# NeRF-3DTalker/NeRF-3DTalker-code

Measured on AMD Instinct MI355X. Metric: rendered frames/sec @512^2 x 64 samples/ray, higher is better.
Workload: dtype bf16; 1 GPU; cfg2-R: 16 heads/GPU/step, 64x64 rays x 64 samples -> fused MLP+composite -> neural renderer -> 512x512 RGB (+ background image); rays_per_frame=4096, samples_per_ray=64, parallelism=frames sharded over 1 rank(s), no data-path collective, ranks_seen_by_backend=1

## Files before the change

### include/n3dt.h

```cpp
#ifndef N3DT_API_H_
#define N3DT_API_H_

#include <stddef.h>
#include <stdint.h>

#ifdef __cplusplus
extern "C" {
#endif

#define N3DT_ABI_VERSION 5

#define N3DT_F32 0
#define N3DT_BF16 1
#define N3DT_F16 2
#define N3DT_BF16X3 3

#define N3DT_OK 0
#define N3DT_EINVAL (-1)
#define N3DT_EWORKSPACE (-2)
#define N3DT_EHIP (-3)

#define N3DT_PE_DIM 63
#define N3DT_MLP_LAYERS 12

typedef struct N3dtGeom {
    int32_t batch;
    int32_t n_rays;
    int32_t n_samples;
    int32_t hidden;
    int32_t feat_nc;
    int32_t shape_dim;
    int32_t appea_dim;
    int32_t audio_dim;
    int32_t featmap_size;
    int32_t n_blocks;
    float world_z1;
    float world_z2;
    int64_t xy_stride_b, xy_stride_c, xy_stride_r;
    int32_t z_planes_given;
    int32_t bg_is_hwc;
    int32_t vd_dim;
} N3dtGeom;

typedef struct N3dtMlpParams {
    const float* weight[N3DT_MLP_LAYERS];
    const float* bias[N3DT_MLP_LAYERS];
} N3dtMlpParams;

#define N3DT_MAX_BLOCKS 8
typedef struct N3dtRenderParams {
    const float* to_rgb_w[N3DT_MAX_BLOCKS + 1];
    const float* to_rgb_b[N3DT_MAX_BLOCKS + 1];
    const float* psu1_w[N3DT_MAX_BLOCKS];
    const float* psu1_b[N3DT_MAX_BLOCKS];
    const float* psu2_w[N3DT_MAX_BLOCKS];
    const float* psu2_b[N3DT_MAX_BLOCKS];
    const float* feat_w[N3DT_MAX_BLOCKS];
    const float* feat_b[N3DT_MAX_BLOCKS];
} N3dtRenderParams;

typedef struct N3dtMlpGrads {
    float* weight[N3DT_MLP_LAYERS];
    float* bias[N3DT_MLP_LAYERS];
} N3dtMlpGrads;

typedef struct N3dtRenderGrads {
    float* to_rgb_w[N3DT_MAX_BLOCKS + 1];
    float* to_rgb_b[N3DT_MAX_BLOCKS + 1];
    float* psu1_w[N3DT_MAX_BLOCKS];
    float* psu1_b[N3DT_MAX_BLOCKS];
    float* psu2_w[N3DT_MAX_BLOCKS];
    float* psu2_b[N3DT_MAX_BLOCKS];
    float* feat_w[N3DT_MAX_BLOCKS];
    float* feat_b[N3DT_MAX_BLOCKS];
} N3dtRenderGrads;

int n3dt_abi_version(void);
const char* n3dt_last_error(void);

size_t n3dt_mlp_packed_bytes(const N3dtGeom* g, int precision);
int n3dt_mlp_pack(const N3dtGeom* g, int precision, const N3dtMlpParams* p, void* packed, void* stream);

size_t n3dt_render_workspace_bytes(const N3dtGeom* g, int precision);
int n3dt_render_fwd(const N3dtGeom* g, int precision, const void* packed_mlp, const N3dtMlpParams* p,
                    const float* xy, const float* R, const float* T, const float* Kinv,
                    const float* shape, const float* appea, const float* audio, const float* t_rand,
                    const float* bg_featmap, const float* ray_bias,
                    float* fg_feat, float* bg_alpha, float* depth, float* weight, float* merge_feat,
                    void* workspace, size_t workspace_bytes, void* stream);

int n3dt_render_fwd16(const N3dtGeom* g, int precision, const void* packed_mlp, const N3dtMlpParams* p,
                      const float* xy, const float* R, const float* T, const float* Kinv,
                      const float* shape, const float* appea, const float* audio, const float* t_rand,
                      const float* bg_featmap, const float* ray_bias,
                      float* fg_feat, float* bg_alpha, float* depth, float* weight, float* merge_feat,
                      void* merge_feat16, float* rgb0, const float* rgb0_w, const float* rgb0_b,
                      void* workspace, size_t workspace_bytes, void* stream);

int n3dt_ray_vd_bias(const N3dtGeom* g, const float* w_vd, int64_t ld_w, const float* xy, const float* R, const float* Kinv,
                     float* ray_bias, void* stream);

int n3dt_fine_sample(const N3dtGeom* g, int n_fine, const float* weight, const float* T, const float* t_rand, const float* u,
                     float* z_planes, void* stream);

int n3dt_sample_points(const N3dtGeom* g, const float* xy, const float* R, const float* T, const float* Kinv, const float* t_rand,
                       float* pts, float* zvals, float* z_dists, float* ray_d, float* ray_l, void* stream);
int n3dt_embed(int batch, size_t m, const float* pts, float* pe, void* stream);
int n3dt_embed_freqs(int batch, size_t m, int n_freqs, const float* pts, float* pe, void* stream);
size_t n3dt_mlp_points_workspace_bytes(const N3dtGeom* g, size_t m);
int n3dt_mlp_points(const N3dtGeom* g, size_t m, const N3dtMlpParams* p, const float* audio, const float* embed_vps,
                    const float* embed_vds, float* rgb, float* density, void* workspace, size_t workspace_bytes, void* stream);
int n3dt_composite(int batch, int n_rays, int n_samples, int channels, const float* rgb, const float* density, const float* z_dists,
                   const float* zvals, float* feat, float* bg_alpha, float* depth, float* weight, void* stream);
int n3dt_x16_pack_probe(int precision, int form, size_t n, const float* in, uint16_t* out, void* stream);
int n3dt_x16_pe_probe(int precision, int form, size_t n, const float* points, uint16_t* out, void* stream);

size_t n3dt_neural_render_workspace_bytes(const N3dtGeom* g, int nb);
int n3dt_neural_render_fwd(const N3dtGeom* g, int nb, int precision, const N3dtRenderParams* p, const float* featmap,
                           float* img, void* workspace, size_t workspace_bytes, void* stream);

int n3dt_neural_render_pack(const N3dtGeom* g, int nb, int precision, const N3dtRenderParams* p, void* workspace,
                            size_t workspace_bytes, void* stream);
int n3dt_neural_render_fwd_reuse(const N3dtGeom* g, int nb, int precision, const N3dtRenderParams* p, const float* featmap,
                                 float* img, void* workspace, size_t workspace_bytes, void* stream);
int n3dt_feat_to_rgb0(int nb, int n_pix, const float* featmap, const float* w, const float* b, float* rgb0, void* stream);
int n3dt_neural_render_fwd16_reuse(const N3dtGeom* g, int nb, int precision, const N3dtRenderParams* p, const void* featmap16,
                                   const float* rgb0, float* img, void* workspace, size_t workspace_bytes, void* stream);

size_t n3dt_render_train_saved_bytes(const N3dtGeom* g);
size_t n3dt_render_train_workspace_bytes(const N3dtGeom* g);
int n3dt_render_train_fwd(const N3dtGeom* g, int precision, const void* packed_mlp, const N3dtMlpParams* p,
                          const float* xy, const float* R, const float* T, const float* Kinv,
                          const float* shape, const float* appea, const float* audio, const float* t_rand,
                          const float* bg_featmap, const float* ray_bias, float* fg_feat, float* bg_alpha, float* depth, float* merge_feat,
                          void* saved, size_t saved_bytes, void* workspace, size_t workspace_bytes, void* stream);
int n3dt_render_bwd(const N3dtGeom* g, int precision, const N3dtMlpParams* p, const N3dtMlpGrads* grads,
                    const float* shape, const float* appea, const float* audio, const float* bg_featmap,
                    const float* d_merge_feat, const float* d_fg_feat, const float* d_bg_alpha,
                    const void* saved, size_t saved_bytes,
                    float* d_bg_featmap, float* d_shape, float* d_appea, float* d_audio, float* d_ray_bias,
                    const float* xy, const float* R, const float* T, const float* Kinv, const float* t_rand,
                    float* d_R, float* d_T,
                    void* workspace, size_t workspace_bytes, void* stream);
int n3dt_render_bwd_cam(const N3dtGeom* g, int precision, const N3dtMlpParams* p, const N3dtMlpGrads* grads,
                        const float* shape, const float* appea, const float* audio, const float* bg_featmap,
                        const float* d_merge_feat, const float* d_fg_feat, const float* d_bg_alpha,
                        const void* saved, size_t saved_bytes,
                        float* d_bg_featmap, float* d_shape, float* d_appea, float* d_audio, float* d_ray_bias,
                        const float* xy, const float* R, const float* T, const float* Kinv, const float* t_rand,
                        float* d_R, float* d_T, float* d_Kinv, float* d_xy,
                        void* workspace, size_t workspace_bytes, void* stream);

size_t n3dt_neural_render_train_saved_bytes(const N3dtGeom* g, int nb);
size_t n3dt_neural_render_train_workspace_bytes(const N3dtGeom* g, int nb);
int n3dt_neural_render_train_fwd(const N3dtGeom* g, int nb, int precision, const N3dtRenderParams* p, const float* featmap, float* img,
                                 void* saved, size_t saved_bytes, void* workspace, size_t workspace_bytes, void* stream);
int n3dt_neural_render_bwd(const N3dtGeom* g, int nb, int precision, const N3dtRenderParams* p, const N3dtRenderGrads* grads,
                           const float* featmap, const float* d_img, const void* saved, size_t saved_bytes,
                           float* d_featmap, void* workspace, size_t workspace_bytes, void* stream);

int n3dt_img_to_uint8(int n_images, int pixels, const float* img, unsigned char* out, void* stream);

size_t n3dt_eval_metrics_workspace_bytes(int n_images, int height, int width);
int n3dt_eval_metrics(int n_images, int height, int width, const float* pred, const float* gt, double* ssim, double* psnr,
                      void* workspace, size_t workspace_bytes, void* stream);

#define N3DT_LPIPS_LAYERS 5
#define N3DT_LPIPS_REFERENCE 0
#define N3DT_LPIPS_STANDARD 1
typedef struct N3dtLpipsParams {
    const float* weight[N3DT_LPIPS_LAYERS];
    const float* bias[N3DT_LPIPS_LAYERS];
    const float* lin[N3DT_LPIPS_LAYERS];
} N3dtLpipsParams;
size_t n3dt_lpips_packed_bytes(void);
int n3dt_lpips_pack(const N3dtLpipsParams* p, void* packed, void* stream);
size_t n3dt_lpips_workspace_bytes(int batch, int height, int width);
int n3dt_lpips(int batch, int height, int width, int input_mode, const void* packed, const float* pred, const float* gt, double* out,
               double* layers, void* workspace, size_t workspace_bytes, void* stream);

size_t n3dt_mel_workspace_bytes(void);
int n3dt_mel_spectrogram(int64_t n_samples, const float* wav, int64_t wav_offset, const float* prev_sample, int64_t total_samples,
                         int64_t first_frame, int n_frames, const float* basis, const double* table, void* out, int64_t out_ld,
                         int out_is_f64, void* workspace, size_t workspace_bytes, void* stream);
int n3dt_mel_windows(int64_t T, const void* mel, int64_t mel_ld, int mel_is_f64, int n_windows, const int32_t* start, float* out,
                     void* stream);

#define N3DT_SYNCNET_BLOCKS 31
typedef struct N3dtSyncnetParams {
    const float* weight[N3DT_SYNCNET_BLOCKS];
    const float* bias[N3DT_SYNCNET_BLOCKS];
    const float* bn_weight[N3DT_SYNCNET_BLOCKS];
    const float* bn_bias[N3DT_SYNCNET_BLOCKS];
    const float* bn_mean[N3DT_SYNCNET_BLOCKS];
    const float* bn_var[N3DT_SYNCNET_BLOCKS];
} N3dtSyncnetParams;
size_t n3dt_syncnet_packed_bytes(void);
int n3dt_syncnet_pack(const N3dtSyncnetParams* p, void* packed, void* stream);
size_t n3dt_syncnet_workspace_bytes(int n);
int n3dt_syncnet_face_windows(int n, int height, int width, const float* frames, const int32_t* boxes, int n_boxes, float* face_windows,
                              void* stream);
int n3dt_syncnet_fwd(int n, const void* packed, const float* mel_windows, const float* face_windows, const float* frames,
                     const int32_t* boxes, int n_boxes, int height, int width, float* audio_emb, float* face_emb, double* cos,
                     void* workspace, size_t workspace_bytes, void* stream);
int n3dt_syncnet_block(int block, int n, const void* packed, const float* in, float* out, void* workspace, size_t workspace_bytes,
                       void* stream);

int n3dt_loss_fwd(int batch, int pixels, const float* merge_img, const float* bg_img, const float* gt, const float* mask,
                  float bg_value, float* acc, float* terms, void* stream);
int n3dt_loss_bwd(int batch, int pixels, const float* merge_img, const float* bg_img, const float* gt, const float* mask,
                  float bg_value, const float* acc, const float* g, const float* g_total, float* d_merge, float* d_bg, void* stream);

#define N3DT_VGG_CONVS 10
typedef struct N3dtVggParams {
    const float* weight[N3DT_VGG_CONVS];
    const float* bias[N3DT_VGG_CONVS];
} N3dtVggParams;
size_t n3dt_vgg_packed_bytes(int precision);
int n3dt_vgg_pack(int precision, const N3dtVggParams* p, void* packed, void* stream);
size_t n3dt_vgg_saved_bytes(int batch, int precision);
size_t n3dt_vgg_workspace_bytes(int batch, int img_size, int precision);
int n3dt_vgg_loss_fwd(int batch, int img_size, int precision, const void* packed, const float* merge_img, const float* gt,
                      const float* mask, float bg_value, float* terms, void* saved, size_t saved_bytes, void* ws, size_t ws_bytes,
                      void* stream);
int n3dt_vgg_loss_bwd(int batch, int img_size, int precision, const void* packed, const float* merge_img, const float* g_total,
                      const void* saved, size_t saved_bytes, float* d_merge, void* ws, size_t ws_bytes, void* stream);

#define N3DT_A2S_IN 1280
#define N3DT_A2S_HIDDEN 640
#define N3DT_A2S_OUT 64
#define N3DT_A2S_MAX_T 256
#define N3DT_A2S_GRAD_FLOATS 20726784
typedef struct N3dtA2sParams {
    const float* w_ih[4];
    const float* w_hh[4];
    const float* b_ih[4];
    const float* b_hh[4];
    const float* lin_w[3];
    const float* lin_b[3];
} N3dtA2sParams;
size_t n3dt_a2s_saved_bytes(int T);
size_t n3dt_a2s_workspace_bytes(int T);
int n3dt_a2s_fwd(int T, const N3dtA2sParams* p, const float* mel, const float* mask1, const float* mask2, const float* mask3,
                 float* out, void* saved, size_t saved_bytes, void* ws, size_t ws_bytes, void* stream);
int n3dt_a2s_bwd(int T, const N3dtA2sParams* p, const float* g_out, const void* saved, size_t saved_bytes, float* grad_arena,
                 void* ws, size_t ws_bytes, void* stream);

#define N3DT_ADAM_MAX_GROUPS 64
#define N3DT_ADAM_MAX_GRID 1024
#define N3DT_ADAM_COUNTER_INTS 4
typedef struct N3dtAdamTensor {
    float* param;
    const float* grad;
    float* exp_avg;
    float* exp_avg_sq;
    int64_t numel;
    int32_t group;
    int32_t active;
} N3dtAdamTensor;
typedef struct N3dtAdamChunk {
    int64_t start;
    int32_t tensor;
    int32_t length;
} N3dtAdamChunk;
typedef struct N3dtAdamGroup {
    double lr, beta1, beta2, eps, weight_decay;
    int32_t maximize;
    int32_t reserved;
} N3dtAdamGroup;
size_t n3dt_flat_adam_record_bytes(int which);
int n3dt_flat_adam_step(const void* tensor_table, const void* chunk_table, int n_chunks, const void* group_table, int n_groups,
                        void* step_counter, void* stream);
#include "n3dt_flat_adam_guard.h"

int n3dt_chw_to_hwc(int C, int n, const float* src, float* dst, void* stream);

#define N3DT_STAGE_MAX 12
typedef struct N3dtStageCopy {
    const float* src[N3DT_STAGE_MAX];
    float* dst[N3DT_STAGE_MAX];
    int64_t count[N3DT_STAGE_MAX];
    int64_t view_dims[3], view_strides[3];
    int32_t n;
} N3dtStageCopy;
int n3dt_stage_inputs(const N3dtStageCopy* st, void* stream);

int n3dt_graph_begin(void* stream);
int n3dt_graph_end(void* stream, void** graph_out);
int n3dt_graph_launch(void* graph, void* stream);
int n3dt_graph_destroy(void* graph);

int n3dt_prof_enable(int max_records);
int n3dt_prof_collect(float* ms_out, int capacity, int* n_out);

#ifdef __cplusplus
}
#endif
#endif
```

### nerf-3dtalker-code_amd/csrc/n3dt_api.hip

```cpp
#include <hip/hip_runtime.h>
#include <stdio.h>
#include <stdlib.h>
#include <string.h>

#include <mutex>

#include "../../include/n3dt.h"
#include "n3dt_layout.h"
#include "eval_metrics_core.h"
#include "lpips_core.h"
#include "mel_core.h"
#include "syncnet_core.h"

extern "C" {
void n3dt_launch_pack(const N3dtGeom*, int, const N3dtMlpParams*, void*, hipStream_t);
void n3dt_launch_fold(const N3dtGeom*, const N3dtMlpParams*, const float*, const float*, const float*, float*, int, hipStream_t);
void n3dt_launch_ray_head(const N3dtGeom*, int, int, const float*, const float*, const float*, const float*, int, float*, float*,
                          float*, float*, float*, hipStream_t);
void n3dt_launch_ray_head_mfma(const N3dtGeom*, int, int, const float*, const float*, const float*, const float*, int, float*, float*,
                               float*, float*, float*, float*, hipStream_t);
void n3dt_launch_ray_head_mfma16(const N3dtGeom*, int, int, const float*, const float*, const float*, const float*, int, float*, float*,
                                 float*, float*, float*, void*, int, float*, const float*, const float*, hipStream_t);
void n3dt_launch_chw_to_hwc(int, int, const float*, float*, hipStream_t);
void n3dt_launch_rayfold(const N3dtGeom*, const float*, const float*, hipStream_t);
void n3dt_launch_ray_vd_bias(const N3dtGeom*, const float*, long, const float*, const float*, const float*, float*, hipStream_t);
void n3dt_launch_embed_freqs(int, size_t, int, const float*, float*, hipStream_t);
void n3dt_launch_sample_points(const N3dtGeom*, const float*, const float*, const float*, const float*, const float*, float*, float*,
                               float*, float*, float*, hipStream_t);
void n3dt_launch_embed(int, size_t, const float*, float*, hipStream_t);
size_t n3dt_seam_mlp_ws_floats(const N3dtGeom*, size_t);
void n3dt_launch_mlp_points(const N3dtGeom*, size_t, const N3dtMlpParams*, const float*, const float*, const float*, float*, float*, float*,
                            hipStream_t);
void n3dt_launch_composite(int, int, int, int, const float*, const float*, const float*, const float*, float*, float*, float*, float*,
                           hipStream_t);
void n3dt_launch_x16_pack_probe(int, int, size_t, const float*, unsigned short*, hipStream_t);
void n3dt_launch_x16_pe_probe(int, int, size_t, const float*, unsigned short*, hipStream_t);
void n3dt_launch_fine_sample(const N3dtGeom*, int, const float*, const float*, const float*, const float*, float*, hipStream_t);
void n3dt_launch_nerf_fwd_f32(const N3dtGeom*, const N3dtMlpParams*, const void*, const float*, const float*, const float*,
                              const float*, const float*, const float*, float*, float*, hipStream_t);
void n3dt_launch_nerf_fwd_x16(const N3dtGeom*, int, const void*, const float*, const float*, const float*, const float*,
                              const float*, const float*, float*, float*, hipStream_t);
void n3dt_launch_nerf_fwd_x16s(const N3dtGeom*, const void*, const float*, const float*, const float*, const float*, const float*,
                               const float*, float*, float*, hipStream_t);
size_t n3dt_nr_workspace_floats(const N3dtGeom*, int);
size_t n3dt_train_saved_floats(const N3dtGeom*);
size_t n3dt_train_ws_floats(const N3dtGeom*);
void n3dt_launch_train_fwd(const N3dtGeom*, const N3dtMlpParams*, const float*, const float*, const float*, const float*, const float*,
                           const float*, const float*, const float*, const float*, const float*, float*, float*, float*, float*, float*,
                           float*, const float* , hipStream_t);
void n3dt_launch_train_bwd(const N3dtGeom*, const N3dtMlpParams*, const N3dtMlpGrads*, const float*, const float*, const float*,
                           const float*, const float*, const float*, const float*, const float*, float*, float*, float*, float*,
                           const float*, const float*, const float*, const float*, const float*, float*, float*, float* ,
                           float* , float*, float* , hipStream_t);
size_t n3dt_train16_saved_bytes(const N3dtGeom*);
size_t n3dt_train16_ws_bytes(const N3dtGeom*);
void n3dt_launch_train16_fwd(const N3dtGeom*, const N3dtMlpParams*, const void*, const float*, const float*, const float*, const float*,
                             const float*, const float*, const float*, const float*, const float*, const float*, float*, float*, float*,
                             float*, void*, void*, const float* , hipStream_t);
void n3dt_launch_train16_bwd(const N3dtGeom*, const N3dtMlpParams*, const N3dtMlpGrads*, const float*, const float*, const float*,
                             const float*, const float*, const float*, const float*, const void*, float*, float*, float*, float*,
                             const float*, const float*, const float*, const float*, const float*, float*, float*, float* ,
                             float* , void*, float* , hipStream_t);
void n3dt_launch_img_to_uint8(int, int, const float*, unsigned char*, hipStream_t);
void n3dt_launch_loss_fwd(int, int, const float*, const float*, const float*, const float*, float, float*, float*, hipStream_t);
void n3dt_launch_loss_bwd(int, int, const float*, const float*, const float*, const float*, float, const float*, const float*, const float*, float*,
                          float*, hipStream_t);
size_t n3dt_nr_train_saved_floats(const N3dtGeom*, int);
size_t n3dt_nr_train_ws_floats(const N3dtGeom*, int);
void n3dt_launch_nr_train_fwd(const N3dtGeom*, int, const N3dtRenderParams*, const float*, float*, float*, float*, int, hipStream_t);
void n3dt_launch_nr_bwd(const N3dtGeom*, int, const N3dtRenderParams*, const N3dtRenderGrads*, const float*, const float*, const float*,
                        float*, float*, int, hipStream_t);
void n3dt_launch_neural_render(const N3dtGeom*, int, int, const N3dtRenderParams*, const float*, float*, float*, int, hipStream_t);
void n3dt_launch_feat_to_rgb0(int, int, const float*, const float*, const float*, float*, hipStream_t);
void n3dt_launch_neural_render16(const N3dtGeom*, int, int, const N3dtRenderParams*, const void*, const float*, float*, float*, hipStream_t);
void n3dt_launch_stage(const N3dtStageCopy*, hipStream_t);
size_t n3dt_vgg_packed_layout_bytes(int);
size_t n3dt_vgg_saved_floats(int);
size_t n3dt_vgg_ws_floats(int);
void n3dt_launch_vgg_pack(int, const N3dtVggParams*, void*, hipStream_t);
void n3dt_launch_vgg_fwd(int, int, int, const void*, const float*, const float*, const float*, float, float*, void*, void*, hipStream_t);
void n3dt_launch_vgg_bwd(int, int, int, const void*, const float*, const float*, const void*, float*, void*, hipStream_t);
size_t n3dt_a2s_saved_floats(int);
size_t n3dt_a2s_ws_floats(int);
void n3dt_launch_a2s_fwd(int, const N3dtA2sParams*, const float*, const float* const[3], float*, void*, void*, hipStream_t);
void n3dt_launch_a2s_bwd(int, const N3dtA2sParams*, const float*, const void*, float*, void*, hipStream_t);
void n3dt_launch_flat_adam(const void*, const void*, int, const void*, int, void*, hipStream_t);
void n3dt_launch_flat_adam_guarded(const void*, const void*, int, const void*, int, void*, void*, void*, hipStream_t);
size_t n3dt_eval_metrics_ws_bytes(int, int, int);
void n3dt_launch_eval_metrics(int, int, int, const float*, const float*, double*, double*, void*, hipStream_t);
size_t n3dt_lpips_packed_layout_bytes(void);
size_t n3dt_lpips_ws_bytes(int, int, int);
void n3dt_launch_lpips_pack(const N3dtLpipsParams*, void*, hipStream_t);
void n3dt_launch_lpips(int, int, int, int, const void*, const float*, const float*, double*, double*, void*, hipStream_t);
size_t n3dt_mel_ws_bytes(void);
void n3dt_launch_mel_spectrogram(const MelSignal*, long long, int, const float*, const double*, void*, long long, int, void*, hipStream_t);
void n3dt_launch_mel_windows(const void*, long long, long long, int, const int*, int, float*, hipStream_t);
size_t n3dt_syncnet_packed_layout_bytes(void);
size_t n3dt_syncnet_ws_bytes(int);
float* n3dt_syncnet_ws_faces(int, void*);
void n3dt_launch_syncnet_pack(const N3dtSyncnetParams*, void*, hipStream_t);
void n3dt_launch_syncnet_faces(int, int, int, const float*, const int*, int, float*, hipStream_t);
void n3dt_launch_syncnet_fwd(int, const void*, const float*, const float*, float*, float*, double*, void*, hipStream_t);
void n3dt_launch_syncnet_block(int, int, const void*, const float*, float*, void*, hipStream_t);
}

static thread_local char g_err[256] = "";

static int fail(int code, const char* msg) {
    snprintf(g_err, sizeof(g_err), "%s", msg);
    return code;
}

static int check_hip(const char* where) {
    hipError_t e = hipGetLastError();
    if (e != hipSuccess) {
        snprintf(g_err, sizeof(g_err), "%s: %s", where, hipGetErrorString(e));
        return N3DT_EHIP;
    }
    return N3DT_OK;
}

static int check_geom(const N3dtGeom* g, int precision) {
    if (!g) return fail(N3DT_EINVAL, "geometry is NULL");
    if (precision != N3DT_F32 && precision != N3DT_BF16 && precision != N3DT_F16 && precision != N3DT_BF16X3)
        return fail(N3DT_EINVAL, "unknown precision");
    if (g->batch < 1 || g->n_rays < 1 || g->n_samples < 1) return fail(N3DT_EINVAL, "batch, n_rays and n_samples must be >= 1");
    if (g->n_samples > 1024) return fail(N3DT_EINVAL, "n_samples > 1024 is not supported");
    if (g->hidden != 384) return fail(N3DT_EINVAL, "only mlp_hidden_nchannels == 384 is built");
    if (g->feat_nc != 256) return fail(N3DT_EINVAL, "only featmap_nc == 256 is built");
    if (g->shape_dim < 1 || g->appea_dim < 1 || g->audio_dim < 0) return fail(N3DT_EINVAL, "bad latent widths");
    if (g->shape_dim + g->audio_dim > 512 || g->appea_dim > 512) return fail(N3DT_EINVAL, "latent width > 512");
    if (g->vd_dim != 0 && g->vd_dim != 27) return fail(N3DT_EINVAL, "vd_dim must be 0 or 27 (include_vd: 3 + 6 * 4 channels)");
    return N3DT_OK;
}
static int check_ray_bias(const N3dtGeom* g, const void* ray_bias, const char* who) {
    if ((g->vd_dim > 0) != (ray_bias != nullptr)) {
        snprintf(g_err, sizeof(g_err), "%s: the per-ray bias must be given iff vd_dim > 0", who);
        return N3DT_EINVAL;
    }
    return N3DT_OK;
}

static inline int block_samples(int precision) { return precision == N3DT_F32 ? 16 : 32; }
static inline size_t align256(size_t b) { return (b + 255) & ~(size_t)255; }

struct RenderCarve {
    size_t fold, part, wlocal, bghwc, total;
    int bpr, bs;
};

static RenderCarve render_carve(const N3dtGeom* g, int precision) {
    RenderCarve c;
    c.bs = block_samples(precision);
    c.bpr = (g->n_samples + c.bs - 1) / c.bs;
    const size_t blocks = (size_t)g->batch * g->n_rays * c.bpr;
    c.fold = 0;
    c.part = align256(n3dt_fold_region_floats(g->batch, g->n_rays, g->vd_dim) * sizeof(float));
    c.wlocal = c.part + align256(blocks * (192 + 4) * sizeof(float));
    c.bghwc = c.wlocal + align256(blocks * c.bs * sizeof(float));
    c.total = c.bghwc + align256((size_t)g->n_rays * g->feat_nc * sizeof(float));
    return c;
}

static std::mutex g_prof_mu;
static hipEvent_t* g_prof_ev = nullptr;
static int g_prof_cap = 0, g_prof_n = 0;

static void prof_free_locked(int created) {
    for (int i = 0; i < created; ++i) (void)hipEventDestroy(g_prof_ev[i]);
    delete[] g_prof_ev;
    g_prof_ev = nullptr;
    g_prof_cap = g_prof_n = 0;
}

extern "C" int n3dt_prof_enable(int max_records) {
    std::lock_guard<std::mutex> lock(g_prof_mu);
    prof_free_locked(2 * g_prof_cap);
    if (max_records <= 0) return N3DT_OK;
    g_prof_ev = new hipEvent_t[2 * (size_t)max_records];
    for (int i = 0; i < 2 * max_records; ++i)
        if (hipEventCreate(&g_prof_ev[i]) != hipSuccess) {
            prof_free_locked(i);
            return fail(N3DT_EHIP, "n3dt_prof_enable: hipEventCreate failed");
        }
    g_prof_cap = max_records;
    return N3DT_OK;
}

extern "C" int n3dt_prof_span_begin(hipStream_t s) {
    if (g_prof_cap <= 0) return -1;
    std::lock_guard<std::mutex> lock(g_prof_mu);
    if (g_prof_n >= g_prof_cap) return -1;
    const int slot = g_prof_n++;
    (void)hipEventRecord(g_prof_ev[2 * slot], s);
    return slot;
}
extern "C" void n3dt_prof_span_end(int slot, hipStream_t s) {
    if (slot < 0) return;
    std::lock_guard<std::mutex> lock(g_prof_mu);
    if (slot < g_prof_cap) (void)hipEventRecord(g_prof_ev[2 * slot + 1], s);
}

extern "C" int n3dt_prof_collect(float* ms_out, int capacity, int* n_out) {
    if (!ms_out || !n_out) return fail(N3DT_EINVAL, "n3dt_prof_collect: NULL argument");
    std::lock_guard<std::mutex> lock(g_prof_mu);
    int n = g_prof_n < capacity ? g_prof_n : capacity;
    for (int i = 0; i < n; ++i) {
        if (hipEventSynchronize(g_prof_ev[2 * i + 1]) != hipSuccess) return fail(N3DT_EHIP, "n3dt_prof_collect: sync failed");
        if (hipEventElapsedTime(&ms_out[i], g_prof_ev[2 * i], g_prof_ev[2 * i + 1]) != hipSuccess)
            return fail(N3DT_EHIP, "n3dt_prof_collect: elapsed failed");
    }
    *n_out = n;
    g_prof_n = 0;
    return N3DT_OK;
}

extern "C" int n3dt_abi_version(void) { return N3DT_ABI_VERSION; }
extern "C" const char* n3dt_last_error(void) { return g_err; }

extern "C" size_t n3dt_mlp_packed_bytes(const N3dtGeom* g, int precision) {
    if (check_geom(g, precision) != N3DT_OK) return 0;
    return n3dt_packed_tail_offset(precision) + n3dt_packed_tail_floats() * sizeof(float);
}

extern "C" int n3dt_mlp_pack(const N3dtGeom* g, int precision, const N3dtMlpParams* p, void* packed, void* stream) {
    int rc = check_geom(g, precision);
    if (rc) return rc;
    if (!p || !packed) return fail(N3DT_EINVAL, "n3dt_mlp_pack: NULL argument");
    for (int l = 0; l < N3DT_MLP_LAYERS; ++l)
        if (!p->weight[l] || !p->bias[l]) return fail(N3DT_EINVAL, "n3dt_mlp_pack: NULL parameter pointer");
    n3dt_launch_pack(g, precision, p, packed, (hipStream_t)stream);
    return check_hip("n3dt_mlp_pack");
}

extern "C" size_t n3dt_render_workspace_bytes(const N3dtGeom* g, int precision) {
    if (check_geom(g, precision) != N3DT_OK) return 0;
    return render_carve(g, precision).total;
}

static int render_fwd_common(const N3dtGeom* g, int precision, const void* packed_mlp, const N3dtMlpParams* p, const float* xy,
                             const float* R, const float* T, const float* Kinv, const float* shape, const float* appea,
                             const float* audio, const float* t_rand, const float* bg_featmap, const float* ray_bias, float* fg_feat,
                             float* bg_alpha, float* depth, float* weight, float* merge_feat, void* merge_feat16, float* rgb0,
                             const float* rgb0_w, const float* rgb0_b, void* workspace, size_t workspace_bytes, void* stream) {
    int rc = check_geom(g, precision);
    if (rc) return rc;
    if ((rc = check_ray_bias(g, ray_bias, "n3dt_render_fwd")) != N3DT_OK) return rc;
    if (!packed_mlp || !p || !xy || !R || !T || !Kinv || !shape || !appea || !workspace)
        return fail(N3DT_EINVAL, "n3dt_render_fwd: NULL argument");
    if (!fg_feat && !merge_feat && !merge_feat16) return fail(N3DT_EINVAL, "n3dt_render_fwd: neither fg_feat nor merge_feat requested");
    if (g->audio_dim > 0 && !audio) return fail(N3DT_EINVAL, "n3dt_render_fwd: audio is NULL but audio_dim > 0");
    if ((merge_feat || merge_feat16 || rgb0) && !bg_featmap) return fail(N3DT_EINVAL, "n3dt_render_fwd: merge_feat needs bg_featmap");
    if ((merge_feat16 || rgb0) && precision == N3DT_F32)
        return fail(N3DT_EINVAL, "n3dt_render_fwd16: the 16-bit map and rgb0 are outputs of the 16-bit precisions");
    if (rgb0 && (!rgb0_w || !rgb0_b)) return fail(N3DT_EINVAL, "n3dt_render_fwd16: rgb0 needs rgb0_w and rgb0_b");
    if (g->z_planes_given && !t_rand) return fail(N3DT_EINVAL, "n3dt_render_fwd: z_planes_given but no planes passed as t_rand");
    const RenderCarve c = render_carve(g, precision);
    if (workspace_bytes < c.total) return fail(N3DT_EWORKSPACE, "n3dt_render_fwd: workspace too small");
    hipStream_t s = (hipStream_t)stream;
    unsigned char* ws = (unsigned char*)workspace;
    float* fold = (float*)(ws + c.fold);
    float* part = (float*)(ws + c.part);
    float* wlocal = (float*)(ws + c.wlocal);
    n3dt_launch_fold(g, p, shape, appea, audio, fold, precision != N3DT_F32, s);
    if (ray_bias) n3dt_launch_rayfold(g, fold, ray_bias, s);
    const int span = n3dt_prof_span_begin(s);
    if (precision == N3DT_F32)
        n3dt_launch_nerf_fwd_f32(g, p, packed_mlp, fold, xy, R, T, Kinv, t_rand, part, weight ? wlocal : nullptr, s);
    else if (precision == N3DT_BF16X3)
        n3dt_launch_nerf_fwd_x16s(g, packed_mlp, fold, xy, R, T, Kinv, t_rand, part, weight ? wlocal : nullptr, s);
    else
        n3dt_launch_nerf_fwd_x16(g, precision, packed_mlp, fold, xy, R, T, Kinv, t_rand, part, weight ? wlocal : nullptr, s);
    n3dt_prof_span_end(span, s);
    const float* tail = (const float*)((const unsigned char*)packed_mlp + n3dt_packed_tail_offset(precision));
    const float* bghwc = bg_featmap;
    const bool merged = merge_feat || merge_feat16 || rgb0;
    if (merged && !g->bg_is_hwc) {
        n3dt_launch_chw_to_hwc(g->feat_nc, g->n_rays, bg_featmap, (float*)(ws + c.bghwc), s);
        bghwc = (const float*)(ws + c.bghwc);
    }
    if (precision == N3DT_F32)
        n3dt_launch_ray_head(g, c.bpr, c.bs, part, wlocal, tail, bghwc, 1, fg_feat, bg_alpha, depth, weight, merge_feat, s);
    else if (merge_feat16 || rgb0)
        n3dt_launch_ray_head_mfma16(g, c.bpr, c.bs, part, wlocal, tail, bghwc, 1, fg_feat, bg_alpha, depth, weight, merge_feat, merge_feat16,
                                    precision == N3DT_BF16 ? N3DT_BF16 : N3DT_F16, rgb0, rgb0_w, rgb0_b, s);
    else
        n3dt_launch_ray_head_mfma(g, c.bpr, c.bs, part, wlocal, tail, bghwc, 1, fg_feat, bg_alpha, depth, weight, merge_feat, nullptr, s);
    return check_hip("n3dt_render_fwd");
}

extern "C" int n3dt_render_fwd(const N3dtGeom* g, int precision, const void* packed_mlp, const N3dtMlpParams* p, const float* xy,
                               const float* R, const float* T, const float* Kinv, const float* shape, const float* appea,
                               const float* audio, const float* t_rand, const float* bg_featmap, const float* ray_bias, float* fg_feat,
                               float* bg_alpha, float* depth, float* weight, float* merge_feat, void* workspace,
                               size_t workspace_bytes, void* stream) {
    return render_fwd_common(g, precision, packed_mlp, p, xy, R, T, Kinv, shape, appea, audio, t_rand, bg_featmap, ray_bias, fg_feat, bg_alpha,
                             depth, weight, merge_feat, nullptr, nullptr, nullptr, nullptr, workspace, workspace_bytes, stream);
}

extern "C" int n3dt_render_fwd16(const N3dtGeom* g, int precision, const void* packed_mlp, const N3dtMlpParams* p, const float* xy,
                                 const float* R, const float* T, const float* Kinv, const float* shape, const float* appea,
                                 const float* audio, const float* t_rand, const float* bg_featmap, const float* ray_bias, float* fg_feat,
                                 float* bg_alpha, float* depth, float* weight, float* merge_feat, void* merge_feat16, float* rgb0,
                                 const float* rgb0_w, const float* rgb0_b, void* workspace, size_t workspace_bytes, void* stream) {
    return render_fwd_common(g, precision, packed_mlp, p, xy, R, T, Kinv, shape, appea, audio, t_rand, bg_featmap, ray_bias, fg_feat, bg_alpha,
                             depth, weight, merge_feat, merge_feat16, rgb0, rgb0_w, rgb0_b, workspace, workspace_bytes, stream);
}

extern "C" int n3dt_sample_points(const N3dtGeom* g, const float* xy, const float* R, const float* T, const float* Kinv,
                                  const float* t_rand, float* pts, float* zvals, float* z_dists, float* ray_d, float* ray_l, void* stream) {
    int rc = check_geom(g, N3DT_F32);
    if (rc) return rc;
    if (!xy || !R || !T || !Kinv) return fail(N3DT_EINVAL, "n3dt_sample_points: NULL argument");
    if (g->z_planes_given && !t_rand) return fail(N3DT_EINVAL, "n3dt_sample_points: z_planes_given but no planes passed as t_rand");
    n3dt_launch_sample_points(g, xy, R, T, Kinv, t_rand, pts, zvals, z_dists, ray_d, ray_l, (hipStream_t)stream);
    return check_hip("n3dt_sample_points");
}

extern "C" int n3dt_embed(int batch, size_t m, const float* pts, float* pe, void* stream) {
    if (batch < 1 || m < 1 || !pts || !pe) return fail(N3DT_EINVAL, "n3dt_embed: bad argument");
    n3dt_launch_embed(batch, m, pts, pe, (hipStream_t)stream);
    return check_hip("n3dt_embed");
}

extern "C" int n3dt_embed_freqs(int batch, size_t m, int n_freqs, const float* pts, float* pe, void* stream) {
    if (batch < 1 || m < 1 || n_freqs < 1 || n_freqs > 16 || !pts || !pe) return fail(N3DT_EINVAL, "n3dt_embed_freqs: bad argument");
    n3dt_launch_embed_freqs(batch, m, n_freqs, pts, pe, (hipStream_t)stream);
    return check_hip("n3dt_embed_freqs");
}

extern "C" int n3dt_ray_vd_bias(const N3dtGeom* g, const float* w_vd, int64_t ld_w, const float* xy, const float* R, const float* Kinv,
                                float* ray_bias, void* stream) {
    int rc = check_geom(g, N3DT_F32);
    if (rc) return rc;
    if (g->vd_dim != 27) return fail(N3DT_EINVAL, "n3dt_ray_vd_bias: vd_dim must be 27");
    if (!w_vd || ld_w < 27 || !xy || !R || !Kinv || !ray_bias) return fail(N3DT_EINVAL, "n3dt_ray_vd_bias: bad argument");
    n3dt_launch_ray_vd_bias(g, w_vd, (long)ld_w, xy, R, Kinv, ray_bias, (hipStream_t)stream);
    return check_hip("n3dt_ray_vd_bias");
}

extern "C" size_t n3dt_mlp_points_workspace_bytes(const N3dtGeom* g, size_t m) {
    if (check_geom(g, N3DT_F32) != N3DT_OK || m < 1) return 0;
    return n3dt_seam_mlp_ws_floats(g, m) * sizeof(float);
}

extern "C" int n3dt_mlp_points(const N3dtGeom* g, size_t m, const N3dtMlpParams* p, const float* audio, const float* embed_vps,
                               const float* embed_vds, float* rgb, float* density, void* workspace, size_t workspace_bytes, void* stream) {
    int rc = check_geom(g, N3DT_F32);
    if (rc) return rc;
    if (m < 1 || !p || !embed_vps || !embed_vds || !rgb || !density || !workspace) return fail(N3DT_EINVAL, "n3dt_mlp_points: NULL argument");
    if (g->audio_dim > 0 && !audio) return fail(N3DT_EINVAL, "n3dt_mlp_points: audio is NULL but audio_dim > 0");
    if ((size_t)g->batch * m > (size_t)1 << 30) return fail(N3DT_EINVAL, "n3dt_mlp_points: more than 2^30 points");
    if (workspace_bytes < n3dt_mlp_points_workspace_bytes(g, m)) return fail(N3DT_EWORKSPACE, "n3dt_mlp_points: workspace too small");
    for (int l = 0; l < N3DT_MLP_LAYERS; ++l)
        if (!p->weight[l] || !p->bias[l]) return fail(N3DT_EINVAL, "n3dt_mlp_points: NULL parameter pointer");
    n3dt_launch_mlp_points(g, m, p, audio, embed_vps, embed_vds, rgb, density, (float*)workspace, (hipStream_t)stream);
    return check_hip("n3dt_mlp_points");
}

extern "C" int n3dt_composite(int batch, int n_rays, int n_samples, int channels, const float* rgb, const float* density,
                              const float* z_dists, const float* zvals, float* feat, float* bg_alpha, float* depth, float* weight,
                              void* stream) {
    if (batch < 1 || n_rays < 1 || n_samples < 1 || channels < 1 || !rgb || !density || !z_dists || !zvals || !feat)
        return fail(N3DT_EINVAL, "n3dt_composite: bad argument");
    if (n_samples > 4096) return fail(N3DT_EINVAL, "n3dt_composite: more than 4096 samples per ray");
    n3dt_launch_composite(batch, n_rays, n_samples, channels, rgb, density, z_dists, zvals, feat, bg_alpha, depth, weight,
                          (hipStream_t)stream);
    return check_hip("n3dt_composite");
}

extern "C" int n3dt_x16_pack_probe(int precision, int form, size_t n, const float* in, uint16_t* out, void* stream) {
    if (precision != N3DT_BF16 && precision != N3DT_F16) return fail(N3DT_EINVAL, "n3dt_x16_pack_probe: precision must be N3DT_BF16 or N3DT_F16");
    if (form != 0 && form != 1) return fail(N3DT_EINVAL, "n3dt_x16_pack_probe: form must be 0 (pack) or 1 (element-wise cast)");
    if (n < 512 || n % 512 != 0 || n / 512 > 0x7fffffffu) return fail(N3DT_EINVAL, "n3dt_x16_pack_probe: n must be a multiple of 512, at most 2^40");
    if (!in || !out) return fail(N3DT_EINVAL, "n3dt_x16_pack_probe: NULL argument");
    n3dt_launch_x16_pack_probe(precision, form, n, in, out, (hipStream_t)stream);
    return check_hip("n3dt_x16_pack_probe");
}

extern "C" int n3dt_x16_pe_probe(int precision, int form, size_t n, const float* points, uint16_t* out, void* stream) {
    if (precision != N3DT_BF16 && precision != N3DT_F16) return fail(N3DT_EINVAL, "n3dt_x16_pe_probe: precision must be N3DT_BF16 or N3DT_F16");
    if (form != 0 && form != 1) return fail(N3DT_EINVAL, "n3dt_x16_pe_probe: form must be 0 (by octave half) or 1 (per channel)");
    if (n < 32 || n % 32 != 0 || n / 32 > 0x7fffffffu) return fail(N3DT_EINVAL, "n3dt_x16_pe_probe: n must be a multiple of 32, at most 2^36");
    if (!points || !out) return fail(N3DT_EINVAL, "n3dt_x16_pe_probe: NULL argument");
    n3dt_launch_x16_pe_probe(precision, form, n, points, out, (hipStream_t)stream);
    return check_hip("n3dt_x16_pe_probe");
}

extern "C" int n3dt_fine_sample(const N3dtGeom* g, int n_fine, const float* weight, const float* T, const float* t_rand, const float* u,
                                float* z_planes, void* stream) {
    int rc = check_geom(g, N3DT_F32);
    if (rc) return rc;
    if (!weight || !T || !z_planes) return fail(N3DT_EINVAL, "n3dt_fine_sample: NULL argument");
    if (g->z_planes_given && !t_rand) return fail(N3DT_EINVAL, "n3dt_fine_sample: z_planes_given but no coarse planes passed as t_rand");
    if (g->n_samples < 3) return fail(N3DT_EINVAL, "n3dt_fine_sample: needs at least 3 coarse samples");
    if (n_fine < 0 || g->n_samples + n_fine + 1 > 2048) return fail(N3DT_EINVAL, "n3dt_fine_sample: more than 2048 planes per ray");
    n3dt_launch_fine_sample(g, n_fine, weight, T, t_rand, u, z_planes, (hipStream_t)stream);
    return check_hip("n3dt_fine_sample");
}

extern "C" size_t n3dt_neural_render_workspace_bytes(const N3dtGeom* g, int nb) {
    if (!g || nb < 1 || g->n_blocks < 1 || g->n_blocks > N3DT_MAX_BLOCKS || g->featmap_size < 2) return 0;
    return n3dt_nr_workspace_floats(g, nb) * sizeof(float);
}

static int neural_render_common(const N3dtGeom* g, int nb, int precision, const N3dtRenderParams* p, const float* featmap, float* img,
                                void* workspace, size_t workspace_bytes, int pack_mode, void* stream, const char* who,
                                const void* featmap16 = nullptr, const float* rgb0 = nullptr) {
    if (!g || !p || !workspace || (pack_mode != 2 && ((!featmap && !featmap16) || !img))) return fail(N3DT_EINVAL, "neural render: NULL argument");
    if (featmap16 && (!rgb0 || precision == N3DT_F32)) return fail(N3DT_EINVAL, "neural render: a 16-bit map needs rgb0 and a 16-bit precision");
    if (precision == N3DT_BF16X3) precision = N3DT_F16;
    if (precision != N3DT_F32 && precision != N3DT_BF16 && precision != N3DT_F16) return fail(N3DT_EINVAL, "unknown precision");
    if (nb < 1) return fail(N3DT_EINVAL, "neural render: nb < 1");
    if (g->n_blocks < 1 || g->n_blocks > N3DT_MAX_BLOCKS) return fail(N3DT_EINVAL, "n_blocks must be in 1..8");
    if (g->feat_nc != 256) return fail(N3DT_EINVAL, "only featmap_nc == 256 is built");
    if (g->featmap_size < 2) return fail(N3DT_EINVAL, "featmap_size < 2 (reflect border needs 2 pixels)");
    {
        const size_t side = (size_t)g->featmap_size << g->n_blocks, elems = (size_t)nb * side * side * 32;
        if (elems >= ((size_t)1 << 31)) return fail(N3DT_EINVAL, "neural render: nb x output pixels x 32 channels must stay below 2^31 (split the batch)");
    }
    if (workspace_bytes < n3dt_neural_render_workspace_bytes(g, nb)) return fail(N3DT_EWORKSPACE, "neural render workspace too small");
    for (int i = 0; i <= g->n_blocks; ++i)
        if (!p->to_rgb_w[i] || !p->to_rgb_b[i]) return fail(N3DT_EINVAL, "NULL feat_2_rgb parameter");
    for (int i = 0; i < g->n_blocks; ++i)
        if (!p->psu1_w[i] || !p->psu1_b[i] || !p->psu2_w[i] || !p->psu2_b[i] || !p->feat_w[i] || !p->feat_b[i])
            return fail(N3DT_EINVAL, "NULL neural-render block parameter");
    if (featmap16)
        n3dt_launch_neural_render16(g, nb, precision, p, featmap16, rgb0, img, (float*)workspace, (hipStream_t)stream);
    else
        n3dt_launch_neural_render(g, nb, precision, p, featmap, img, (float*)workspace, pack_mode, (hipStream_t)stream);
    return check_hip(who);
}

extern "C" int n3dt_neural_render_fwd(const N3dtGeom* g, int nb, int precision, const N3dtRenderParams* p, const float* featmap,
                                      float* img, void* workspace, size_t workspace_bytes, void* stream) {
    return neural_render_common(g, nb, precision, p, featmap, img, workspace, workspace_bytes, 0, stream, "n3dt_neural_render_fwd");
}

extern "C" int n3dt_neural_render_pack(const N3dtGeom* g, int nb, int precision, const N3dtRenderParams* p, void* workspace,
                                       size_t workspace_bytes, void* stream) {
    return neural_render_common(g, nb, precision, p, nullptr, nullptr, workspace, workspace_bytes, 2, stream, "n3dt_neural_render_pack");
}

extern "C" int n3dt_neural_render_fwd_reuse(const N3dtGeom* g, int nb, int precision, const N3dtRenderParams* p, const float* featmap,
                                            float* img, void* workspace, size_t workspace_bytes, void* stream) {
    return neural_render_common(g, nb, precision, p, featmap, img, workspace, workspace_bytes, 1, stream, "n3dt_neural_render_fwd_reuse");
}

extern "C" int n3dt_feat_to_rgb0(int nb, int n_pix, const float* featmap, const float* w, const float* b, float* rgb0, void* stream) {
    if (nb < 1 || n_pix < 1 || !featmap || !w || !b || !rgb0) return fail(N3DT_EINVAL, "n3dt_feat_to_rgb0: bad argument");
    if ((size_t)nb * n_pix >= ((size_t)1 << 27)) return fail(N3DT_EINVAL, "n3dt_feat_to_rgb0: more than 2^27 pixels");
    n3dt_launch_feat_to_rgb0(nb, n_pix, featmap, w, b, rgb0, (hipStream_t)stream);
    return check_hip("n3dt_feat_to_rgb0");
}

extern "C" int n3dt_neural_render_fwd16_reuse(const N3dtGeom* g, int nb, int precision, const N3dtRenderParams* p, const void* featmap16,
                                              const float* rgb0, float* img, void* workspace, size_t workspace_bytes, void* stream) {
    if (!featmap16) return fail(N3DT_EINVAL, "n3dt_neural_render_fwd16_reuse: NULL argument");
    return neural_render_common(g, nb, precision, p, nullptr, img, workspace, workspace_bytes, 1, stream, "n3dt_neural_render_fwd16_reuse",
                                featmap16, rgb0);
}

static int check_vgg(const char* who, int batch, int img_size, int precision) {
    char m[160];
    if (precision != N3DT_F32 && precision != N3DT_BF16) {
        snprintf(m, sizeof(m), "%s: unsupported precision %d (N3DT_F32 or N3DT_BF16)", who, precision);
        return fail(N3DT_EINVAL, m);
    }
    if (batch < 1 || batch > 64) {
        snprintf(m, sizeof(m), "%s: batch %d outside 1..64", who, batch);
        return fail(N3DT_EINVAL, m);
    }
    if (img_size < 16 || img_size > 2048) {
        snprintf(m, sizeof(m), "%s: img_size %d outside 16..2048", who, img_size);
        return fail(N3DT_EINVAL, m);
    }
    return N3DT_OK;
}

extern "C" size_t n3dt_vgg_packed_bytes(int precision) {
    if (check_vgg("n3dt_vgg_packed_bytes", 1, 224, precision)) return 0;
    return n3dt_vgg_packed_layout_bytes(precision);
}

extern "C" size_t n3dt_vgg_saved_bytes(int batch, int precision) {
    if (check_vgg("n3dt_vgg_saved_bytes", batch, 224, precision)) return 0;
    return n3dt_vgg_saved_floats(batch) * sizeof(float);
}

extern "C" size_t n3dt_vgg_workspace_bytes(int batch, int img_size, int precision) {
    if (check_vgg("n3dt_vgg_workspace_bytes", batch, img_size, precision)) return 0;
    return n3dt_vgg_ws_floats(batch) * sizeof(float);
}

extern "C" int n3dt_vgg_pack(int precision, const N3dtVggParams* p, void* packed, void* stream) {
    int rc = check_vgg("n3dt_vgg_pack", 1, 224, precision);
    if (rc) return rc;
    if (!p || !packed) return fail(N3DT_EINVAL, "n3dt_vgg_pack: NULL argument");
    for (int l = 0; l < N3DT_VGG_CONVS; ++l)
        if (!p->weight[l] || !p->bias[l]) return fail(N3DT_EINVAL, "n3dt_vgg_pack: NULL parameter pointer");
    n3dt_launch_vgg_pack(precision, p, packed, (hipStream_t)stream);
    return check_hip("n3dt_vgg_pack");
}

extern "C" int n3dt_vgg_loss_fwd(int batch, int img_size, int precision, const void* packed, const float* merge_img, const float* gt,
                                 const float* mask, float bg_value, float* terms, void* saved, size_t saved_bytes, void* ws, size_t ws_bytes,
                                 void* stream) {
    int rc = check_vgg("n3dt_vgg_loss_fwd", batch, img_size, precision);
    if (rc) return rc;
    if (!packed || !merge_img || !gt || !terms || !saved || !ws) return fail(N3DT_EINVAL, "n3dt_vgg_loss_fwd: NULL argument");
    if (saved_bytes < n3dt_vgg_saved_floats(batch) * sizeof(float)) return fail(N3DT_EWORKSPACE, "n3dt_vgg_loss_fwd: saved buffer too small");
    if (ws_bytes < n3dt_vgg_ws_floats(batch) * sizeof(float)) return fail(N3DT_EWORKSPACE, "n3dt_vgg_loss_fwd: workspace too small");
    n3dt_launch_vgg_fwd(batch, img_size, precision, packed, merge_img, gt, mask, bg_value, terms, saved, ws, (hipStream_t)stream);
    return check_hip("n3dt_vgg_loss_fwd");
}

extern "C" int n3dt_vgg_loss_bwd(int batch, int img_size, int precision, const void* packed, const float* merge_img, const float* g_total,
                                 const void* saved, size_t saved_bytes, float* d_merge, void* ws, size_t ws_bytes, void* stream) {
    int rc = check_vgg("n3dt_vgg_loss_bwd", batch, img_size, precision);
    if (rc) return rc;
    if (!packed || !merge_img || !g_total || !saved || !d_merge || !ws) return fail(N3DT_EINVAL, "n3dt_vgg_loss_bwd: NULL argument");
    if (saved_bytes < n3dt_vgg_saved_floats(batch) * sizeof(float)) return fail(N3DT_EWORKSPACE, "n3dt_vgg_loss_bwd: saved buffer too small");
    if (ws_bytes < n3dt_vgg_ws_floats(batch) * sizeof(float)) return fail(N3DT_EWORKSPACE, "n3dt_vgg_loss_bwd: workspace too small");
    n3dt_launch_vgg_bwd(batch, img_size, precision, packed, merge_img, g_total, saved, d_merge, ws, (hipStream_t)stream);
    return check_hip("n3dt_vgg_loss_bwd");
}

static int a2s_fail(const char* who, const char* what) {
    char m[200];
    snprintf(m, sizeof(m), "%s: %s", who, what);
    return fail(N3DT_EINVAL, m);
}

static int check_a2s_T(const char* who, int T) {
    if (T < 1 || T > N3DT_A2S_MAX_T) {
        char m[160];
        snprintf(m, sizeof(m), "%s: T = %d outside 1..%d", who, T, N3DT_A2S_MAX_T);
        return fail(N3DT_EINVAL, m);
    }
    return N3DT_OK;
}

static bool a2s_aligned(const void* q) { return (((size_t)q) & 15) == 0; }

static int check_a2s_params(const char* who, const N3dtA2sParams* p) {
    if (!p) return a2s_fail(who, "params is NULL");
    static const char* names[4] = {"w_ih", "w_hh", "b_ih", "b_hh"};
    const float* const* lstm[4] = {p->w_ih, p->w_hh, p->b_ih, p->b_hh};
    char m[96];
    for (int a = 0; a < 4; ++a)
        for (int k = 0; k < 4; ++k) {
            if (!lstm[a][k] || !a2s_aligned(lstm[a][k])) {
                snprintf(m, sizeof(m), "params->%s[%d] is NULL or not 16-byte aligned", names[a], k);
                return a2s_fail(who, m);
            }
        }
    for (int k = 0; k < 3; ++k) {
        if (!p->lin_w[k] || !a2s_aligned(p->lin_w[k])) {
            snprintf(m, sizeof(m), "params->lin_w[%d] is NULL or not 16-byte aligned", k);
            return a2s_fail(who, m);
        }
        if (!p->lin_b[k] || !a2s_aligned(p->lin_b[k])) {
            snprintf(m, sizeof(m), "params->lin_b[%d] is NULL or not 16-byte aligned", k);
            return a2s_fail(who, m);
        }
    }
    return N3DT_OK;
}

static int check_a2s_buf(const char* who, const char* name, const void* q, size_t have, size_t need) {
    char m[160];
    if (!q || !a2s_aligned(q)) {
        snprintf(m, sizeof(m), "%s is NULL or not 16-byte aligned", name);
        return a2s_fail(who, m);
    }
    if (have < need) {
        snprintf(m, sizeof(m), "%s_bytes = %zu, %zu needed", name, have, need);
        return a2s_fail(who, m);
    }
    return N3DT_OK;
}

extern "C" size_t n3dt_a2s_saved_bytes(int T) {
    if (check_a2s_T("n3dt_a2s_saved_bytes", T)) return 0;
    return n3dt_a2s_saved_floats(T) * sizeof(float);
}

extern "C" size_t n3dt_a2s_workspace_bytes(int T) {
    if (check_a2s_T("n3dt_a2s_workspace_bytes", T)) return 0;
    return n3dt_a2s_ws_floats(T) * sizeof(float);
}

extern "C" int n3dt_a2s_fwd(int T, const N3dtA2sParams* p, const float* mel, const float* mask1, const float* mask2, const float* mask3,
                            float* out, void* saved, size_t saved_bytes, void* ws, size_t ws_bytes, void* stream) {
    static const char* who = "n3dt_a2s_fwd";
    int rc = check_a2s_T(who, T);
    if (!rc) rc = check_a2s_params(who, p);
    if (rc) return rc;
    if (!mel || !a2s_aligned(mel)) return a2s_fail(who, "mel is NULL or not 16-byte aligned");
    if (!out) return a2s_fail(who, "out is NULL");
    const float* masks[3] = {mask1, mask2, mask3};
    if ((mask1 != nullptr) != (mask2 != nullptr) || (mask1 != nullptr) != (mask3 != nullptr))
        return a2s_fail(who, "mask1, mask2 and mask3 must be all given or all NULL");
    if ((rc = check_a2s_buf(who, "saved", saved, saved_bytes, n3dt_a2s_saved_floats(T) * sizeof(float)))) return rc;
    if ((rc = check_a2s_buf(who, "ws", ws, ws_bytes, n3dt_a2s_ws_floats(T) * sizeof(float)))) return rc;
    n3dt_launch_a2s_fwd(T, p, mel, masks, out, saved, ws, (hipStream_t)stream);
    return check_hip(who);
}

extern "C" int n3dt_a2s_bwd(int T, const N3dtA2sParams* p, const float* g_out, const void* saved, size_t saved_bytes, float* grad_arena,
                            void* ws, size_t ws_bytes, void* stream) {
    static const char* who = "n3dt_a2s_bwd";
    int rc = check_a2s_T(who, T);
    if (!rc) rc = check_a2s_params(who, p);
    if (rc) return rc;
    if (!g_out) return a2s_fail(who, "g_out is NULL");
    if (!grad_arena || !a2s_aligned(grad_arena)) return a2s_fail(who, "grad_arena is NULL or not 16-byte aligned");
    if ((rc = check_a2s_buf(who, "saved", saved, saved_bytes, n3dt_a2s_saved_floats(T) * sizeof(float)))) return rc;
    if ((rc = check_a2s_buf(who, "ws", ws, ws_bytes, n3dt_a2s_ws_floats(T) * sizeof(float)))) return rc;
    n3dt_launch_a2s_bwd(T, p, g_out, saved, grad_arena, ws, (hipStream_t)stream);
    return check_hip(who);
}

extern "C" size_t n3dt_flat_adam_record_bytes(int which) {
    return which == 0 ? sizeof(N3dtAdamTensor) : which == 1 ? sizeof(N3dtAdamChunk) : which == 2 ? sizeof(N3dtAdamGroup) : 0;
}

extern "C" int n3dt_flat_adam_step(const void* tensor_table, const void* chunk_table, int n_chunks, const void* group_table,
                                   int n_groups, void* step_counter, void* stream) {
    if (!tensor_table || !chunk_table || !group_table || !step_counter) return fail(N3DT_EINVAL, "n3dt_flat_adam_step: NULL table");
    if (n_chunks <= 0) return fail(N3DT_EINVAL, "n3dt_flat_adam_step: n_chunks must be >= 1");
    if (n_groups < 1 || n_groups > N3DT_ADAM_MAX_GROUPS) return fail(N3DT_EINVAL, "n3dt_flat_adam_step: n_groups outside 1..64");
    if ((((size_t)tensor_table) | ((size_t)chunk_table) | ((size_t)group_table)) & 7 || ((size_t)step_counter) & 3)
        return fail(N3DT_EINVAL, "n3dt_flat_adam_step: tables must be 8-byte aligned, the step counter 4-byte aligned");
    n3dt_launch_flat_adam(tensor_table, chunk_table, n_chunks, group_table, n_groups, step_counter, (hipStream_t)stream);
    return check_hip("n3dt_flat_adam_step");
}

extern "C" size_t n3dt_flat_adam_guard_bytes(void) { return sizeof(N3dtAdamGuard); }

extern "C" int n3dt_flat_adam_guarded_step(const void* tensor_table, const void* chunk_table, int n_chunks, const void* group_table,
                                           int n_groups, void* step_counter, void* partials, void* guard, void* stream) {
    static const char* who = "n3dt_flat_adam_guarded_step";
    char msg[160];
    const char* what = nullptr;
    if (!tensor_table || !chunk_table || !group_table || !step_counter) what = "NULL table";
    else if (!partials || !guard) what = "NULL partials or guard record";
    else if (n_chunks <= 0) what = "n_chunks must be >= 1";
    else if (n_groups < 1 || n_groups > N3DT_ADAM_MAX_GROUPS) what = "n_groups outside 1..64";
    else if ((((size_t)tensor_table) | ((size_t)chunk_table) | ((size_t)group_table)) & 7 || ((size_t)step_counter) & 3)
        what = "tables must be 8-byte aligned, the step counter 4-byte aligned";
    else if (((size_t)partials) & 7 || ((size_t)guard) & 3) what = "partials must be 8-byte aligned, the guard record 4-byte aligned";
    if (what) {
        snprintf(msg, sizeof(msg), "%s: %s", who, what);
        return fail(N3DT_EINVAL, msg);
    }
    n3dt_launch_flat_adam_guarded(tensor_table, chunk_table, n_chunks, group_table, n_groups, step_counter, partials, guard,
                                  (hipStream_t)stream);
    return check_hip(who);
}

static const char* eval_metrics_geometry(int n_images, int height, int width) {
    if (n_images < 1) return "n_images must be >= 1";
    if (height < EVM_WIN || width < EVM_WIN) return "height and width must be >= 7 (one 7x7 window)";
    if ((long long)height * (long long)width >= EVM_MAX_HW) return "height * width must stay below 2^31";
    return nullptr;
}

extern "C" size_t n3dt_eval_metrics_workspace_bytes(int n_images, int height, int width) {
    const char* what = eval_metrics_geometry(n_images, height, width);
    if (what) {
        snprintf(g_err, sizeof(g_err), "n3dt_eval_metrics_workspace_bytes: %s", what);
        return 0;
    }
    return n3dt_eval_metrics_ws_bytes(n_images, height, width);
}

extern "C" int n3dt_eval_metrics(int n_images, int height, int width, const float* pred, const float* gt, double* ssim, double* psnr,
                                 void* workspace, size_t workspace_bytes, void* stream) {
    static const char* who = "n3dt_eval_metrics";
    char msg[160];
    const char* what = eval_metrics_geometry(n_images, height, width);
    if (!what) {
        if (!pred || !gt || !ssim || !psnr || !workspace) what = "NULL pointer";
        else if ((((size_t)ssim) | ((size_t)psnr) | ((size_t)workspace)) & 7) what = "ssim, psnr and the workspace must be 8-byte aligned";
        else if ((((size_t)pred) | ((size_t)gt)) & 3) what = "pred and gt must be 4-byte aligned";
        else if (workspace_bytes < n3dt_eval_metrics_ws_bytes(n_images, height, width)) what = "workspace too small";
    }
    if (what) {
// ... 425 lines not shown
```

### nerf-3dtalker-code_amd/csrc/n3dt_device.h

```cpp
#pragma once
#include <hip/hip_runtime.h>
#include <stdint.h>

#include "../../include/n3dt.h"

#define N3DT_HID 384
#define N3DT_C 256
#define N3DT_G 192
#define N3DT_PE_ROWS 64
#define N3DT_PART_STRIDE (N3DT_G + 4)

typedef float f32x4 __attribute__((ext_vector_type(4)));
typedef float f32x16 __attribute__((ext_vector_type(16)));
typedef short s16x8 __attribute__((ext_vector_type(8)));
typedef _Float16 f16x8 __attribute__((ext_vector_type(8)));

struct N3dtFrameCam {
    float R[9], K[9], T[3];
};

__device__ __forceinline__ float n3dt_linspace01(int i, int steps) {
    float step = 1.0f / (float)(steps - 1);
    int half = steps / 2;
    return (i < half) ? step * (float)i : 1.0f - step * (float)(steps - 1 - i);
}

__device__ __forceinline__ void n3dt_ray_setup(const float* __restrict__ R, const float* __restrict__ K, float x, float y,
                                               float d[3], float& l) {
    float c[3], w[3];
#pragma unroll
    for (int i = 0; i < 3; ++i) c[i] = K[i * 3 + 0] * x + K[i * 3 + 1] * y + K[i * 3 + 2] * 1.0f;
#pragma unroll
    for (int i = 0; i < 3; ++i) w[i] = R[i * 3 + 0] * c[0] + R[i * 3 + 1] * c[1] + R[i * 3 + 2] * c[2];
    float n = sqrtf(w[0] * w[0] + w[1] * w[1] + w[2] * w[2]);
    d[0] = w[0] / n;
    d[1] = w[1] / n;
    d[2] = w[2] / n;
    l = -1.0f / d[2];
}

__device__ __forceinline__ float n3dt_edge_z(float rz1, float rz2, int j, int Ns, const float* __restrict__ tr) {
    float t = n3dt_linspace01(j, Ns + 1);
    float zv = rz1 * (1.0f - t) + rz2 * t;
    if (!tr) return zv;
    float lower, upper;
    if (j == 0) {
        lower = zv;
    } else {
        float tp = n3dt_linspace01(j - 1, Ns + 1);
        float zp = rz1 * (1.0f - tp) + rz2 * tp;
        lower = 0.5f * (zv + zp);
    }
    if (j == Ns) {
        upper = zv;
    } else {
        float tn = n3dt_linspace01(j + 1, Ns + 1);
        float zn = rz1 * (1.0f - tn) + rz2 * tn;
        upper = 0.5f * (zn + zv);
    }
    return lower + (upper - lower) * tr[j];
}

__device__ __forceinline__ void n3dt_sample_point(const N3dtGeom& g, const float* __restrict__ xy, const float* __restrict__ R,
                                                  const float* __restrict__ T, const float* __restrict__ Kinv,
                                                  const float* __restrict__ t_rand, int b, int ray, int s, float p[3],
                                                  float& dist, float& zval) {
    const float* Rb = R + b * 9;
    const float* Kb = Kinv + b * 9;
    const float* Tb = T + b * 3;
    float x = xy[(int64_t)b * g.xy_stride_b + 0 * g.xy_stride_c + (int64_t)ray * g.xy_stride_r];
    float y = xy[(int64_t)b * g.xy_stride_b + 1 * g.xy_stride_c + (int64_t)ray * g.xy_stride_r];
    float d[3], l;
    n3dt_ray_setup(Rb, Kb, x, y, d, l);
    float rz1 = Tb[2] - g.world_z1, rz2 = Tb[2] - g.world_z2;
    const int Ns = g.n_samples;
    if (s < Ns) {
        const float* tr = t_rand ? t_rand + ((int64_t)b * g.n_rays + ray) * (Ns + 1) : nullptr;
        float z_lo, z_hi;
        if (g.z_planes_given) {
            z_lo = tr[s];
            z_hi = tr[s + 1];
        } else {
            z_lo = n3dt_edge_z(rz1, rz2, s, Ns, tr);
            z_hi = n3dt_edge_z(rz1, rz2, s + 1, Ns, tr);
        }
        dist = (z_hi - z_lo) * l;
        zval = z_lo;
#pragma unroll
        for (int i = 0; i < 3; ++i) p[i] = Tb[i] + (d[i] * l) * z_lo;
    } else {
        dist = 0.0f;
        zval = 0.0f;
        p[0] = p[1] = p[2] = 0.0f;
    }
}

__device__ __forceinline__ float n3dt_pe_row_accurate(const float p[3], int row) {
    if (row < 3) return row == 0 ? p[0] : (row == 1 ? p[1] : p[2]);
    if (row >= N3DT_PE_DIM) return 0.0f;
    int k = (row - 3) / 6, w = (row - 3) % 6;
    int dim = w % 3;
    float v = dim == 0 ? p[0] : (dim == 1 ? p[1] : p[2]);
    float a = v * (float)(1 << k);
    return w < 3 ? sinf(a) : cosf(a);
}

struct N3dtDiv {
    unsigned d;
    int sh;
};
__device__ __forceinline__ N3dtDiv n3dt_div(const unsigned d) {
    N3dtDiv v;
    v.d = d;
    v.sh = (d != 0 && (d & (d - 1)) == 0) ? 31 - __builtin_clz(d) : -1;
    return v;
}
__device__ __forceinline__ size_t n3dt_quot(const size_t x, const N3dtDiv v) { return v.sh >= 0 ? x >> v.sh : x / v.d; }
__device__ __forceinline__ int n3dt_rem(const size_t x, const N3dtDiv v) { return v.sh >= 0 ? (int)(x & (v.d - 1)) : (int)(x % v.d); }

__device__ __forceinline__ void n3dt_up_blur_w3(const int o, const int n, float (&w3)[3]) {
    if (n >= 3) {
        const bool ev = (o & 1) == 0;
        const bool first = o == 0, second = o == 1, last = o == 2 * n - 1, last2 = o == 2 * n - 2;
        w3[0] = (first || second) ? 0.0f : (last ? 0.125f : (ev ? 0.3125f : 0.0625f));
        w3[1] = (first || last) ? 0.875f : ((second || last2) ? 0.6875f : 0.625f);
        w3[2] = (last || last2) ? 0.0f : (first ? 0.125f : (ev ? 0.0625f : 0.3125f));
        return;
    }
    const int base = o >> 1;
    w3[0] = w3[1] = w3[2] = 0.0f;
#pragma unroll
    for (int d = -1; d <= 1; ++d) {
        int i = o + d;
        i = i < 0 ? -i : (i >= 2 * n ? 4 * n - 2 - i : i);
        const float kd = d == 0 ? 0.5f : 0.25f;
        const int m = i >> 1;
        int a0, a1;
        float f0, f1;
        if ((i & 1) == 0) {
            a0 = max(m - 1, 0); f0 = 0.25f;
            a1 = m; f1 = 0.75f;
        } else {
            a0 = m; f0 = 0.75f;
            a1 = min(m + 1, n - 1); f1 = 0.25f;
        }
        const int s0 = a0 - base + 1, s1 = a1 - base + 1;
        w3[0] += (s0 == 0 ? kd * f0 : 0.0f) + (s1 == 0 ? kd * f1 : 0.0f);
        w3[1] += (s0 == 1 ? kd * f0 : 0.0f) + (s1 == 1 ? kd * f1 : 0.0f);
        w3[2] += (s0 == 2 ? kd * f0 : 0.0f) + (s1 == 2 ? kd * f1 : 0.0f);
    }
}

template <int WIDTH>
__device__ __forceinline__ float n3dt_exclusive_prod(float x, int lane_in_group) {
    float incl = x;
#pragma unroll
    for (int off = 1; off < WIDTH; off <<= 1) {
        float o = __shfl_up(incl, off, WIDTH);
        if (lane_in_group >= off) incl *= o;
    }
    float excl = __shfl_up(incl, 1, WIDTH);
    return lane_in_group == 0 ? 1.0f : excl;
}
```

### nerf-3dtalker-code_amd/csrc/nerf_aux.hip

```cpp
#include "n3dt_device.h"
#include "n3dt_layout.h"

__device__ __forceinline__ float logical_weight(const N3dtMlpParams& p, int stage, int row, int col, int S, int A, int U) {
    const int in0 = N3DT_PE_DIM + S + U, in5 = N3DT_PE_DIM + S + N3DT_HID, inr = N3DT_HID + A;
    switch (stage) {
        case 0: return col < N3DT_PE_DIM ? p.weight[0][(size_t)row * in0 + col] : 0.0f;
        case 5:
            if (col < N3DT_PE_DIM) return p.weight[5][(size_t)row * in5 + col];
            if (col == N3DT_PE_DIM) return 0.0f;
            return p.weight[5][(size_t)row * in5 + N3DT_PE_DIM + S + (col - 64)];
        case 8: return row == 0 ? p.weight[8][col] : 0.0f;
        case 10: return p.weight[10][(size_t)row * inr + col];
        default: return p.weight[stage][(size_t)row * N3DT_HID + col];
    }
}

__global__ __launch_bounds__(256) void small_gemm_kernel(int M, int N, int K, const float* __restrict__ A, long sam, long sak,
                                                                 const float* __restrict__ Bm, long sbn, long sbk,
                                                                 float* __restrict__ C, long ldc, int accumulate) {
    __shared__ float As[32][33], Bs[32][33];
    const int t = threadIdx.x, tx = t & 15, ty = t >> 4;
    const int m0 = blockIdx.y * 32, n0 = blockIdx.x * 32;
    float acc[2][2] = {{0.f, 0.f}, {0.f, 0.f}};
    float ra[4], rb[4];
    auto fetch = [&](const int k0) {
#pragma unroll
        for (int u = 0; u < 4; ++u) {
            const int i = t + 256 * u;
            const int a_r = sak == 1 ? i >> 5 : i & 31, a_k = sak == 1 ? i & 31 : i >> 5;
            const int b_r = sbk == 1 ? i >> 5 : i & 31, b_k = sbk == 1 ? i & 31 : i >> 5;
            ra[u] = (m0 + a_r < M && k0 + a_k < K) ? A[(long)(m0 + a_r) * sam + (long)(k0 + a_k) * sak] : 0.0f;
            rb[u] = (n0 + b_r < N && k0 + b_k < K) ? Bm[(long)(n0 + b_r) * sbn + (long)(k0 + b_k) * sbk] : 0.0f;
        }
    };
    fetch(0);
    for (int k0 = 0; k0 < K; k0 += 32) {
#pragma unroll
        for (int u = 0; u < 4; ++u) {
            const int i = t + 256 * u;
            const int a_r = sak == 1 ? i >> 5 : i & 31, a_k = sak == 1 ? i & 31 : i >> 5;
            const int b_r = sbk == 1 ? i >> 5 : i & 31, b_k = sbk == 1 ? i & 31 : i >> 5;
            As[a_k][a_r] = ra[u];
            Bs[b_k][b_r] = rb[u];
        }
        __syncthreads();
        if (k0 + 32 < K) fetch(k0 + 32);
#pragma unroll
        for (int k = 0; k < 32; ++k) {
            const float a0 = As[k][ty], a1 = As[k][ty + 16], b0 = Bs[k][tx], b1 = Bs[k][tx + 16];
            acc[0][0] = fmaf(a0, b0, acc[0][0]);
            acc[0][1] = fmaf(a0, b1, acc[0][1]);
            acc[1][0] = fmaf(a1, b0, acc[1][0]);
            acc[1][1] = fmaf(a1, b1, acc[1][1]);
        }
        __syncthreads();
    }
#pragma unroll
    for (int i = 0; i < 2; ++i)
#pragma unroll
        for (int j = 0; j < 2; ++j) {
            const int m = m0 + ty + 16 * i, n = n0 + tx + 16 * j;
            if (m < M && n < N) C[(long)m * ldc + n] = (accumulate ? C[(long)m * ldc + n] : 0.0f) + acc[i][j];
        }
}
extern "C" void n3dt_launch_small_gemm(int M, int N, int K, const float* A, long sam, long sak, const float* B, long sbn, long sbk,
                                       float* C, long ldc, int accumulate, hipStream_t s) {
    hipLaunchKernelGGL(small_gemm_kernel, dim3((N + 31) / 32, (M + 31) / 32), dim3(256), 0, s, M, N, K, A, sam, sak, B, sbn, sbk, C, ldc,
                       accumulate);
}

__device__ __forceinline__ unsigned short f32_to_bf16_rne(float f) {
    __bf16 h = (__bf16)f;
    return __builtin_bit_cast(unsigned short, h);
}

__global__ void pack_mlp_kernel(N3dtMlpParams p, int precision, int S, int A, int U, const float* __restrict__ wm,
                                unsigned char* __restrict__ out) {
    const int stage = blockIdx.y;
    const bool merged = precision != N3DT_F32 && stage == 9;
    if (precision != N3DT_F32 && stage == 10) return;
    N3dtStage st = n3dt_stage(stage);
    if (merged) st = n3dt_stage(10);
    const size_t n = (size_t)st.N * st.K;
    const size_t base = n3dt_stage_offset(stage);
    for (size_t e = (size_t)blockIdx.x * blockDim.x + threadIdx.x; e < n; e += (size_t)gridDim.x * blockDim.x) {
        int row, col;
        if (precision == N3DT_F32) {
            int j = e & 3, lane = (e >> 2) & 63;
            size_t t = e >> 8;
            int k4 = (int)(t % (st.K / 16)), ot = (int)(t / (st.K / 16));
            row = ot * 16 + (lane & 15);
            col = 16 * k4 + 4 * j + (lane >> 4);
        } else {
            int j = e & 7, lane = (e >> 3) & 63;
            size_t t = e >> 9;
            int ks = (int)(t % (st.K / 16)), ot = (int)(t / (st.K / 16));
            row = ot * 32 + (lane & 31);
            col = 32 * (ks >> 1) + 16 * (ks & 1) + 8 * (j >> 2) + 4 * (lane >> 5) + (j & 3);
        }
        float v;
        if (merged) {
            v = wm[(size_t)row * N3DT_HID + col];
        } else {
            v = logical_weight(p, stage, row, col, S, A, U);
        }
        if (precision == N3DT_F32) {
            reinterpret_cast<float*>(out)[base + e] = v;
        } else if (precision == N3DT_BF16) {
            reinterpret_cast<unsigned short*>(out)[base + e] = f32_to_bf16_rne(v);
        } else if (precision == N3DT_BF16X3) {
            const size_t P = (base + e) >> 9, in = (base + e) & 511;
            const __bf16 hi = (__bf16)v;
            const __bf16 lo = (__bf16)(v - (float)hi);
            reinterpret_cast<unsigned short*>(out)[(2 * P) * 512 + in] = __builtin_bit_cast(unsigned short, hi);
            reinterpret_cast<unsigned short*>(out)[(2 * P + 1) * 512 + in] = __builtin_bit_cast(unsigned short, lo);
        } else {
            _Float16 hv = (_Float16)v;
            reinterpret_cast<unsigned short*>(out)[base + e] = __builtin_bit_cast(unsigned short, hv);
        }
    }
}

__global__ void pack_tail_kernel(N3dtMlpParams p, float* __restrict__ tail) {
    int i = blockIdx.x * blockDim.x + threadIdx.x;
    if (i < N3DT_G * N3DT_C) {
        int j = i / N3DT_C, c = i % N3DT_C;
        tail[i] = p.weight[11][(size_t)c * N3DT_G + j];
    } else if (i < N3DT_G * N3DT_C + N3DT_C) {
        tail[i] = p.bias[11][i - N3DT_G * N3DT_C];
    } else if (i < N3DT_G * N3DT_C + N3DT_C + 12 * 8 * 2 * 64) {
        const int t = i - (N3DT_G * N3DT_C + N3DT_C);
        const int lane = t & 63, piece = t >> 6, part = piece & 1, tile = (piece >> 1) & 7, ks = piece >> 4;
        const int col = 32 * tile + (lane & 31), k0 = 16 * ks + 8 * (lane >> 5);
        unsigned short* dst = reinterpret_cast<unsigned short*>(tail + n3dt_tail_w2_frags_offset()) + (size_t)piece * 512 + lane * 8;
        for (int j = 0; j < 8; ++j) {
            const float v = p.weight[11][(size_t)col * N3DT_G + k0 + j];
            const __bf16 hi = (__bf16)v;
            const __bf16 out = part == 0 ? hi : (__bf16)(v - (float)hi);
            dst[j] = __builtin_bit_cast(unsigned short, out);
        }
    }
}

extern "C" void n3dt_launch_pack(const N3dtGeom* g, int precision, const N3dtMlpParams* p, void* packed, hipStream_t stream) {
    float* tail = reinterpret_cast<float*>(reinterpret_cast<unsigned char*>(packed) + n3dt_packed_tail_offset(precision));
    float* wm = tail + N3DT_G * N3DT_C + N3DT_C;
    if (precision != N3DT_F32)
        n3dt_launch_small_gemm(192, 384, 384, p->weight[10], 384 + g->appea_dim, 1, p->weight[9], 1, 384, wm, 384, 0, stream);
    hipLaunchKernelGGL(pack_mlp_kernel, dim3(64, N3DT_NSTAGE), dim3(256), 0, stream, *p, precision, g->shape_dim, g->appea_dim, g->audio_dim,
                       wm, reinterpret_cast<unsigned char*>(packed));
    const int n = N3DT_G * N3DT_C + N3DT_C + 12 * 8 * 2 * 64;
    hipLaunchKernelGGL(pack_tail_kernel, dim3((n + 255) / 256), dim3(256), 0, stream, *p, tail);
}

#define FOLD_ROWGROUPS 24
__global__ __launch_bounds__(256) void fold_latents_kernel(N3dtMlpParams p, int S, int A, int U, int merged, const float* __restrict__ shape,
                                                           const float* __restrict__ appea, const float* __restrict__ audio,
                                                           float* __restrict__ fold) {
    const int b = blockIdx.x, stage = blockIdx.y;
    const int lane = threadIdx.x & 63, wave = threadIdx.x >> 6;
    __shared__ float code[512 + N3DT_HID];
    const int in0 = N3DT_PE_DIM + S + U, in5 = N3DT_PE_DIM + S + N3DT_HID, inr = N3DT_HID + A;
    const N3dtStage st = n3dt_stage(stage);
    float* out = fold + (size_t)b * N3DT_FOLD_STRIDE + n3dt_bias_offset(stage);
    int n_code = 0, col0 = 0, ld = 0;
    if (stage == 0) { n_code = S + U; col0 = N3DT_PE_DIM; ld = in0; }
    else if (stage == 5) { n_code = S; col0 = N3DT_PE_DIM; ld = in5; }
    else if (stage == 10) {
        n_code = merged ? N3DT_HID + A : A;
        col0 = merged ? 0 : N3DT_HID;
        ld = inr;
    }
    for (int i = threadIdx.x; i < n_code; i += blockDim.x) {
        float v;
        if (stage == 10) {
            const int j = merged ? i - N3DT_HID : i;
            v = j < 0 ? p.bias[9][i] : appea[(size_t)b * A + j];
        } else {
            v = i < S ? shape[(size_t)b * S + i] : audio[(size_t)b * U + (i - S)];
        }
        code[i] = v;
    }
    __syncthreads();
    if (stage == 8) {
        for (int o = blockIdx.z * 4 + wave; o < st.N; o += 4 * FOLD_ROWGROUPS)
            if (lane == 0) out[o] = o == 0 ? p.bias[8][0] : 0.0f;
        return;
    }
    constexpr int FOLD_UNR = 4;
    constexpr int RSTEP = 4 * FOLD_ROWGROUPS;
    for (int o0 = blockIdx.z * 4 + wave; o0 < st.N; o0 += RSTEP * FOLD_UNR) {
        float acc[FOLD_UNR];
#pragma unroll
        for (int u = 0; u < FOLD_UNR; ++u) acc[u] = 0.0f;
        if (n_code > 0) {
            const float* w[FOLD_UNR];
#pragma unroll
            for (int u = 0; u < FOLD_UNR; ++u) w[u] = p.weight[st.layer] + (size_t)min(o0 + RSTEP * u, st.N - 1) * ld + col0;
            for (int i = lane; i < n_code; i += 64) {
                const float cv = code[i];
#pragma unroll
                for (int u = 0; u < FOLD_UNR; ++u) acc[u] = fmaf(w[u][i], cv, acc[u]);
            }
#pragma unroll
            for (int off = 32; off > 0; off >>= 1)
#pragma unroll
                for (int u = 0; u < FOLD_UNR; ++u) acc[u] += __shfl_xor(acc[u], off, 64);
        }
#pragma unroll
        for (int u = 0; u < FOLD_UNR; ++u) {
            const int o = o0 + RSTEP * u;
            if (lane == 0 && o < st.N) out[o] = p.bias[st.layer][o] + acc[u];
        }
    }
}

extern "C" void n3dt_launch_fold(const N3dtGeom* g, const N3dtMlpParams* p, const float* shape, const float* appea,
                                 const float* audio, float* fold, int merged_rgb, hipStream_t stream) {
    hipLaunchKernelGGL(fold_latents_kernel, dim3(g->batch, N3DT_NSTAGE, FOLD_ROWGROUPS), dim3(256), 0, stream, *p, g->shape_dim,
                       g->appea_dim, g->audio_dim, merged_rgb, shape, appea, audio, fold);
}

__global__ __launch_bounds__(256) void rayfold_kernel(int n_rays, long total, const float* __restrict__ fold, const float* __restrict__ ray_bias,
                                                      float* __restrict__ rayfold) {
    const long i = (long)blockIdx.x * blockDim.x + threadIdx.x;
    if (i >= total * 48) return;
    const long ray = i / 48;
    const int o = (int)(i % 48) * 4;
    const f32x4 f = *reinterpret_cast<const f32x4*>(fold + (size_t)(ray / n_rays) * N3DT_FOLD_STRIDE + n3dt_bias_offset(10) + o);
    const f32x4 r = *reinterpret_cast<const f32x4*>(ray_bias + (size_t)ray * N3DT_RAYFOLD_STRIDE + o);
    *reinterpret_cast<f32x4*>(rayfold + (size_t)ray * N3DT_RAYFOLD_STRIDE + o) = f32x4{f[0] + r[0], f[1] + r[1], f[2] + r[2], f[3] + r[3]};
}
extern "C" void n3dt_launch_rayfold(const N3dtGeom* g, const float* fold, const float* ray_bias, hipStream_t s) {
    const long total = (long)g->batch * g->n_rays;
    float* rayfold = const_cast<float*>(fold) + n3dt_rayfold_offset(g->batch);
    hipLaunchKernelGGL(rayfold_kernel, dim3((unsigned)((total * 48 + 255) / 256)), dim3(256), 0, s, g->n_rays, total, fold, ray_bias, rayfold);
}

__global__ __launch_bounds__(256) void ray_vd_bias_kernel(N3dtGeom g, const float* __restrict__ w_vd, long ld_w, const float* __restrict__ xy,
                                                          const float* __restrict__ R, const float* __restrict__ Kinv,
                                                          float* __restrict__ ray_bias) {
    __shared__ float wl[192 * 27];
    for (int i = threadIdx.x; i < 192 * 27; i += blockDim.x) wl[i] = w_vd[(size_t)(i / 27) * ld_w + i % 27];
    __syncthreads();
    const int lane = threadIdx.x & 63, wave = threadIdx.x >> 6;
    const long total = (long)g.batch * g.n_rays;
    for (long rayg = (long)blockIdx.x * 4 + wave; rayg < total; rayg += (long)gridDim.x * 4) {
        const int b = (int)(rayg / g.n_rays), ray = (int)(rayg % g.n_rays);
        const float x = xy[(int64_t)b * g.xy_stride_b + 0 * g.xy_stride_c + (int64_t)ray * g.xy_stride_r];
        const float y = xy[(int64_t)b * g.xy_stride_b + 1 * g.xy_stride_c + (int64_t)ray * g.xy_stride_r];
        float d[3], l;
        n3dt_ray_setup(R + b * 9, Kinv + b * 9, x, y, d, l);
        float pe[27];
        pe[0] = d[0]; pe[1] = d[1]; pe[2] = d[2];
#pragma unroll
        for (int k = 0; k < 4; ++k)
#pragma unroll
            for (int i = 0; i < 3; ++i) {
                const float a = d[i] * (float)(1 << k);
                pe[3 + 6 * k + i] = sinf(a);
                pe[3 + 6 * k + 3 + i] = cosf(a);
            }
#pragma unroll
        for (int u = 0; u < 3; ++u) {
            const int o = lane + 64 * u;
            float acc = 0.0f;
#pragma unroll
            for (int j = 0; j < 27; ++j) acc = fmaf(wl[o * 27 + j], pe[j], acc);
            ray_bias[(size_t)rayg * N3DT_RAYFOLD_STRIDE + o] = acc;
        }
    }
}
extern "C" void n3dt_launch_ray_vd_bias(const N3dtGeom* g, const float* w_vd, long ld_w, const float* xy, const float* R, const float* Kinv,
                                        float* ray_bias, hipStream_t s) {
    const long total = (long)g->batch * g->n_rays;
    long grid = (total + 3) / 4;
    if (grid > 2048) grid = 2048;
    hipLaunchKernelGGL(ray_vd_bias_kernel, dim3((unsigned)grid), dim3(256), 0, s, *g, w_vd, ld_w, xy, R, Kinv, ray_bias);
}

#define HEAD_RAYS 8
#define HEAD_MAX_BPR 64
__global__ __launch_bounds__(256) void ray_head_kernel(N3dtGeom g, int bpr, int bs, const float* __restrict__ part,
                                                       const float* __restrict__ wlocal, const float* __restrict__ tail,
                                                       const float* __restrict__ bg_featmap, int bg_hwc, float* __restrict__ fg_feat,
                                                       float* __restrict__ bg_alpha, float* __restrict__ depth,
                                                       float* __restrict__ weight, float* __restrict__ merge_feat,
                                                       float* __restrict__ rayrec) {
    __shared__ float G[HEAD_RAYS][N3DT_G];
    __shared__ float pref[HEAD_RAYS][HEAD_MAX_BPR];
    __shared__ float wsum_s[HEAD_RAYS], dsum_s[HEAD_RAYS];
    const long nrays_total = (long)g.batch * g.n_rays;
    const long ray0 = (long)blockIdx.x * HEAD_RAYS;
    const int t = threadIdx.x;
    if (t < HEAD_RAYS) {
        long rg = ray0 + t;
        float Trun = 1.0f, ws = 0.0f, ds = 0.0f;
        if (rg < nrays_total) {
            for (int k = 0; k < bpr; ++k) {
                const float* po = part + ((size_t)rg * bpr + k) * N3DT_PART_STRIDE + N3DT_G;
                pref[t][k] = Trun;
                ws += Trun * po[0];
                ds += Trun * po[1];
                Trun *= po[2];
            }
        }
        wsum_s[t] = ws;
        dsum_s[t] = ds;
    }
    __syncthreads();
    for (int i = t; i < HEAD_RAYS * N3DT_G; i += 256) {
        int r = i / N3DT_G, j = i % N3DT_G;
        long rg = ray0 + r;
        float acc = 0.0f;
        if (rg < nrays_total)
            for (int k = 0; k < bpr; ++k) acc += pref[r][k] * part[((size_t)rg * bpr + k) * N3DT_PART_STRIDE + j];
        G[r][j] = acc;
        if (rayrec && rg < nrays_total) rayrec[(size_t)rg * N3DT_PART_STRIDE + j] = acc;
    }
    __syncthreads();
    if (rayrec && t < HEAD_RAYS && ray0 + t < nrays_total) {
        float* rec = rayrec + (size_t)(ray0 + t) * N3DT_PART_STRIDE + N3DT_G;
        rec[0] = wsum_s[t];
        rec[1] = dsum_s[t];
        rec[2] = 0.0f;
        rec[3] = 0.0f;
    }
    const float* W2T = tail;
    const float b2 = tail[N3DT_G * N3DT_C + t];
    float acc[HEAD_RAYS];
#pragma unroll
    for (int r = 0; r < HEAD_RAYS; ++r) acc[r] = 0.0f;
    for (int j = 0; j < N3DT_G; ++j) {
        float wv = W2T[j * N3DT_C + t];
#pragma unroll
        for (int r = 0; r < HEAD_RAYS; ++r) acc[r] = fmaf(wv, G[r][j], acc[r]);
    }
#pragma unroll
    for (int r = 0; r < HEAD_RAYS; ++r) {
        long rg = ray0 + r;
        if (rg >= nrays_total) break;
        float fg = acc[r] + b2 * wsum_s[r];
        float ba = 1.0f - wsum_s[r];
        if (fg_feat) fg_feat[(size_t)rg * N3DT_C + t] = fg;
        if (merge_feat) {
            int ray = (int)(rg % g.n_rays);
            merge_feat[(size_t)rg * N3DT_C + t] = fg + ba * (bg_hwc ? bg_featmap[(size_t)ray * N3DT_C + t] : bg_featmap[(size_t)t * g.n_rays + ray]);
        }
        if (t == 0) {
            if (bg_alpha) bg_alpha[rg] = ba;
            if (depth) depth[rg] = dsum_s[r];
        }
    }
    if (weight) {
        for (int i = t; i < HEAD_RAYS * g.n_samples; i += 256) {
            int r = i / g.n_samples, s = i % g.n_samples;
            long rg = ray0 + r;
            if (rg < nrays_total) {
                int k = s / bs;
                weight[(size_t)rg * g.n_samples + s] = pref[r][k] * wlocal[((size_t)rg * bpr + k) * bs + (s % bs)];
            }
        }
    }
}

typedef __bf16 rh_bf16x8 __attribute__((ext_vector_type(8)));
#define RH_RAYS 32
template <bool MAP16, int PREC16 = N3DT_BF16>
__global__ __launch_bounds__(256, 4) void ray_head_mfma_kernel(N3dtGeom g, int bpr, int bs, const float* __restrict__ part,
                                                            const float* __restrict__ wlocal, const float* __restrict__ tail,
                                                            const float* __restrict__ bg_featmap, int bg_hwc,
                                                            float* __restrict__ fg_feat, float* __restrict__ bg_alpha,
                                                            float* __restrict__ depth, float* __restrict__ weight,
                                                            float* __restrict__ merge_feat, float* __restrict__ rayrec,
                                                            unsigned short* __restrict__ merge16, float* __restrict__ rgb0, const float* __restrict__ rgb_w,
                                                            const float* __restrict__ rgb_b) {
    __shared__ __attribute__((aligned(16))) float G[RH_RAYS][N3DT_G + 4];
    __shared__ float pref[RH_RAYS][HEAD_MAX_BPR];
    __shared__ float wsum_s[RH_RAYS], dsum_s[RH_RAYS];
    __shared__ float rgb_s[4][RH_RAYS][3];
    const long nrays_total = (long)g.batch * g.n_rays;
    const long ray0 = (long)blockIdx.x * RH_RAYS;
    const int t = threadIdx.x, lane = t & 63, wave = t >> 6;
    if (MAP16) rayrec = nullptr;
    if (t < RH_RAYS) {
        const long rg = ray0 + t;
        float Trun = 1.0f, ws = 0.0f, ds = 0.0f;
        if (rg < nrays_total) {
            for (int k = 0; k < bpr; ++k) {
                const float* po = part + ((size_t)rg * bpr + k) * N3DT_PART_STRIDE + N3DT_G;
                pref[t][k] = Trun;
                ws += Trun * po[0];
                ds += Trun * po[1];
                Trun *= po[2];
            }
        }
        wsum_s[t] = ws;
        dsum_s[t] = ds;
    }
    __syncthreads();
    static_assert(N3DT_G % 4 == 0 && (N3DT_PART_STRIDE * 4) % 16 == 0 && RH_RAYS * (N3DT_G / 4) % 256 == 0, "whole quads");
    constexpr int QPR = N3DT_G / 4, NQ = RH_RAYS * QPR / 256;
    if (bpr <= 2) {
        f32x4 v[NQ][2];
        float pf[NQ][2];
#pragma unroll
        for (int u = 0; u < NQ; ++u) {
            const int i = t + 256 * u, r = i / QPR, q = i % QPR;
            const long rg = min(ray0 + r, nrays_total - 1);
            const float* p0 = part + (size_t)rg * bpr * N3DT_PART_STRIDE + 4 * q;
            v[u][0] = *reinterpret_cast<const f32x4*>(p0);
            v[u][1] = *reinterpret_cast<const f32x4*>(p0 + (bpr == 2 ? N3DT_PART_STRIDE : 0));
            pf[u][0] = pref[r][0];
            pf[u][1] = bpr == 2 ? pref[r][1] : 0.0f;
        }
#pragma unroll
        for (int u = 0; u < NQ; ++u) {
            const int i = t + 256 * u, r = i / QPR, q = i % QPR;
            f32x4 a;
#pragma unroll
            for (int e = 0; e < 4; ++e) a[e] = pf[u][0] * v[u][0][e] + pf[u][1] * v[u][1][e];
            const bool in = ray0 + r < nrays_total;
            if (!in) a = f32x4{0.0f, 0.0f, 0.0f, 0.0f};
            *reinterpret_cast<f32x4*>(&G[r][4 * q]) = a;
            if (rayrec && in) *reinterpret_cast<f32x4*>(rayrec + (size_t)(ray0 + r) * N3DT_PART_STRIDE + 4 * q) = a;
        }
    } else {
        for (int i = t; i < RH_RAYS * N3DT_G; i += 256) {
            const int r = i / N3DT_G, j = i % N3DT_G;
            const long rg = ray0 + r;
            float acc = 0.0f;
            if (rg < nrays_total)
                for (int k = 0; k < bpr; ++k) acc += pref[r][k] * part[((size_t)rg * bpr + k) * N3DT_PART_STRIDE + j];
            G[r][j] = acc;
            if (rayrec && rg < nrays_total) rayrec[(size_t)rg * N3DT_PART_STRIDE + j] = acc;
        }
    }
    __syncthreads();
    if (rayrec && t < RH_RAYS && ray0 + t < nrays_total) {
        float* rec = rayrec + (size_t)(ray0 + t) * N3DT_PART_STRIDE + N3DT_G;
        rec[0] = wsum_s[t];
        rec[1] = dsum_s[t];
        rec[2] = 0.0f;
        rec[3] = 0.0f;
    }
    const int r31 = lane & 31, h = lane >> 5;
    f32x16 acc[2];
#pragma unroll
    for (int i = 0; i < 2; ++i)
#pragma unroll
        for (int r = 0; r < 16; ++r) acc[i][r] = 0.0f;
    const rh_bf16x8* w2frags = reinterpret_cast<const rh_bf16x8*>(tail + n3dt_tail_w2_frags_offset());
#pragma unroll 2
    for (int ks = 0; ks < N3DT_G / 16; ++ks) {
        const int k0 = 16 * ks + 8 * h;
        rh_bf16x8 a_hi, a_lo;
        const f32x4 g0 = *reinterpret_cast<const f32x4*>(&G[r31][k0]), g1 = *reinterpret_cast<const f32x4*>(&G[r31][k0 + 4]);
#pragma unroll
        for (int j = 0; j < 8; ++j) {
            const float v = j < 4 ? g0[j] : g1[j - 4];
            const __bf16 hi = (__bf16)v;
            a_hi[j] = hi;
            a_lo[j] = (__bf16)(v - (float)hi);
        }
#pragma unroll
        for (int i = 0; i < 2; ++i) {
            const rh_bf16x8* fr = w2frags + ((size_t)(ks * 8 + 2 * wave + i) * 2) * 64 + lane;
            const rh_bf16x8 b_hi = fr[0], b_lo = fr[64];
            acc[i] = __builtin_amdgcn_mfma_f32_32x32x16_bf16(a_hi, b_hi, acc[i], 0, 0, 0);
            acc[i] = __builtin_amdgcn_mfma_f32_32x32x16_bf16(a_hi, b_lo, acc[i], 0, 0, 0);
            acc[i] = __builtin_amdgcn_mfma_f32_32x32x16_bf16(a_lo, b_hi, acc[i], 0, 0, 0);
        }
    }
    float pr[MAP16 ? 16 : 1][3];
    if constexpr (!MAP16) {
#pragma unroll
        for (int i = 0; i < 2; ++i) {
            const int c = 64 * wave + 32 * i + r31;
            const float b2 = tail[N3DT_G * N3DT_C + c];
            float bgv[16];
#pragma unroll
            for (int r = 0; r < 16; ++r) {
                const int rr = (r & 3) + 8 * (r >> 2) + 4 * h;
                const long rg = min(ray0 + rr, nrays_total - 1);
                const int ray = (int)(rg % g.n_rays);
                bgv[r] = merge_feat ? (bg_hwc ? bg_featmap[(size_t)ray * N3DT_C + c] : bg_featmap[(size_t)c * g.n_rays + ray]) : 0.0f;
            }
#pragma unroll
            for (int r = 0; r < 16; ++r) {
                const int rr = (r & 3) + 8 * (r >> 2) + 4 * h;
                const long rg = ray0 + rr;
                if (rg >= nrays_total) continue;
                const float fg = acc[i][r] + b2 * wsum_s[rr];
                if (fg_feat) fg_feat[(size_t)rg * N3DT_C + c] = fg;
                if (merge_feat) merge_feat[(size_t)rg * N3DT_C + c] = fg + (1.0f - wsum_s[rr]) * bgv[r];
            }
        }
    } else {
#pragma unroll
        for (int i = 0; i < 2; ++i) {
            const int c = 64 * wave + 32 * i + r31;
            const float b2 = tail[N3DT_G * N3DT_C + c];
            float w3[3] = {0.0f, 0.0f, 0.0f};
            if (rgb0) {
#pragma unroll
                for (int k = 0; k < 3; ++k) w3[k] = rgb_w[k * N3DT_C + c];
            }
#pragma unroll
            for (int r0 = 0; r0 < 16; r0 += 8) {
                float bgv[8];
#pragma unroll
                for (int r = r0; r < r0 + 8; ++r) {
                    const int rr = (r & 3) + 8 * (r >> 2) + 4 * h;
                    const long rg = min(ray0 + rr, nrays_total - 1);
                    const int ray = (int)(rg % g.n_rays);
                    bgv[r - r0] = bg_featmap[(size_t)ray * N3DT_C + c];
                }
#pragma unroll
                for (int r = r0; r < r0 + 8; ++r) {
                    const int rr = (r & 3) + 8 * (r >> 2) + 4 * h;
                    const long rg = ray0 + rr;
                    const float mg = (acc[i][r] + b2 * wsum_s[rr]) + (1.0f - wsum_s[rr]) * bgv[r - r0];
#pragma unroll
// ... 225 lines not shown
```

### nerf-3dtalker-code_amd/csrc/nerf_fwd_x16.hip

```cpp
#include "x16_core.h"


#ifndef X16_SAVE_DEPTH
#define X16_SAVE_DEPTH 3
#endif
#ifndef X16_FWD_ISSUE
#define X16_FWD_ISSUE 0, 1, 2
#endif
template <int PREC>
struct X16SaveStage {
    unsigned char* tile0;
    unsigned* gate0;
};

enum { X16_BIAS_GLOBAL_MFMA = 0, X16_BIAS_LDS_MFMA = 1, X16_BIAS_LDS_C = 2 };
#define X16_BIAS_SLOT 1536
struct X16BiasLds {
    unsigned char* slots;
    unsigned addr;
    __device__ __forceinline__ void stage_in(const float* table, const int n, const int slot, const int lane, const int at = 0) const {
#pragma unroll
        for (int i = 0; i < 6; ++i)
            if (64 * i < n)
                __builtin_amdgcn_global_load_lds((const GLOBAL_AS void*)(table + 64 * i + lane),
                                                 (LDS_AS void*)(slots + slot * X16_BIAS_SLOT + 4 * at + 256 * i), 4, 0, 0);
    }
    __device__ __forceinline__ unsigned at(const int slot, const int at = 0) const { return addr + slot * X16_BIAS_SLOT + 4 * at; }
};
struct X16TileInit {
    f32x4 q[2][4];
    template <int SET, int OFF>
    __device__ __forceinline__ void issue(const unsigned table) {
        asm volatile("ds_read_b128 %0, %4 offset:%5\n\tds_read_b128 %1, %4 offset:%6\n\t"
                     "ds_read_b128 %2, %4 offset:%7\n\tds_read_b128 %3, %4 offset:%8"
                     : "=&v"(q[SET][0]), "=&v"(q[SET][1]), "=&v"(q[SET][2]), "=&v"(q[SET][3])
                     : "v"(table), "i"(OFF), "i"(OFF + 32), "i"(OFF + 64), "i"(OFF + 96)
                     : "memory");
    }
    template <int SET>
    __device__ __forceinline__ void landed() {
        asm volatile("" : "+v"(q[SET][0]), "+v"(q[SET][1]), "+v"(q[SET][2]), "+v"(q[SET][3]));
    }
    template <int SET>
    __device__ __forceinline__ void settle() {
        asm volatile("s_waitcnt lgkmcnt(0)" : "+v"(q[SET][0]), "+v"(q[SET][1]), "+v"(q[SET][2]), "+v"(q[SET][3]));
    }
    template <int SET>
    __device__ __forceinline__ f32x16 get() const {
        f32x16 v;
#pragma unroll
        for (int r = 0; r < 16; ++r) v[r] = q[SET][r >> 2][r & 3];
        return v;
    }
};
constexpr int X16_TILE_INIT_READS = 4;

template <int PREC, int WAVES, int KS, int KPE, int NT, int MODE, bool SAVE, int BIAS, int PAR, bool NEXT, class WS>
__device__ __forceinline__ void x16_stage(WS& ws, X16TileInit& ti, const float* __restrict__ bias, const unsigned bias_lds, const unsigned next_lds,
                                          const typename X16<PREC>::frag (&pe_reg)[4], const unsigned char* pe_lds,
                                          const typename X16<PREC>::frag (&hin)[24], typename X16<PREC>::frag (&hout)[24],
                                          float& aux, float* const po, const bool live, const int lane,
                                          const X16SaveStage<PREC>* sv = nullptr, const short relu_lo = 0) {
    typedef typename X16<PREC>::frag frag;
    static_assert(KS >= WS::depth, "a tile's bias reads are covered by the wait of its own k-step DEPTH - 1");
    const int h = lane >> 5, c = lane & 31;
    float red[32];
    unsigned gate_word = 0;
    constexpr bool PACKS = (MODE == MODE_HIDDEN || MODE == MODE_LINEAR);
    f32x16 acc;
    constexpr bool CINIT = BIAS == X16_BIAS_LDS_C, LB = BIAS == X16_BIAS_LDS_MFMA;
    [[maybe_unused]] const frag ones = X16<PREC>::ones_frag();
    [[maybe_unused]] float bias_cur = 0.0f, bias_nxt = 0.0f;
    if constexpr (LB) {
        x16_bias_read<0>(bias_cur, bias_lds);
        asm volatile("s_waitcnt lgkmcnt(0)" : "+v"(bias_cur));
    } else if constexpr (!CINIT) {
        bias_cur = bias[c];
    }
    auto finish_half = [&](const int t, const int half) {
        float v[8];
#pragma unroll
        for (int r = 0; r < 8; ++r) v[r] = acc[8 * half + r];
        frag f = X16<PREC>::pack(v);
        if (MODE == MODE_HIDDEN) f = X16<PREC>::relu(f, relu_lo);
        hout[2 * t + half] = f;
    };
    static_for<0, NT>([&](auto ot_c) {
        constexpr int ot = decltype(ot_c)::value;
        constexpr int cs = (PAR + ot) & 1, ns = cs ^ 1;
        constexpr bool FETCH = CINIT && ot + 1 < NT;
        X16_T(const unsigned long long s0 = x16_now();)
        if constexpr (CINIT) {
            if constexpr (ot == 0) ti.template settle<cs>();
            if constexpr (FETCH) ti.template issue<ns, (ot + 1) * 128>(bias_lds);
            acc = ti.template get<cs>();
        } else {
            const frag bf = X16<PREC>::bias_frag(bias_cur, h == 0);
            if constexpr (LB) {
                if constexpr (ot + 1 < NT) x16_bias_read<(ot + 1) * 128>(bias_nxt, bias_lds);
            } else {
                if (ot + 1 < NT) bias_cur = bias[(ot + 1) * 32 + c];
            }
            f32x16 zero;
#pragma unroll
            for (int r = 0; r < 16; ++r) zero[r] = 0.0f;
            acc = X16<PREC>::mfma(bf, ones, zero);
        }
        X16_T(const unsigned long long s1 = x16_now(); const unsigned long long rv0 = ws.t_rv;)
        static_for<0, KS>([&](auto ks_c) {
            constexpr int ks = decltype(ks_c)::value;
            const frag a_cur = ws.template next<MODE == MODE_COMPOSITE, NT * KS, ot * KS + ks,
                                                (FETCH && ks < WS::depth - 1) ? X16_TILE_INIT_READS : 0>();
            frag b;
            if (ks < KPE) {
                if (pe_lds) b = *reinterpret_cast<const frag*>(pe_lds + ks * X16_PIECE);
                else b = pe_reg[ks < 4 ? ks : 0];
            } else {
                b = hin[ks >= KPE ? ks - KPE : 0];
            }
            acc = X16<PREC>::mfma(a_cur, b, acc);
        });
        if constexpr (FETCH) ti.template landed<ns>();
        else if constexpr (CINIT && NEXT && ot + 1 == NT) ti.template issue<ns, 0>(next_lds);
        if constexpr (LB && ot + 1 < NT) {
            asm volatile("" : "+v"(bias_nxt), "+v"(acc));
            bias_cur = bias_nxt;
        }
        X16_T(const unsigned long long s2 = x16_now();)
        if (PACKS) {
            finish_half(ot, 0);
            finish_half(ot, 1);
        }
        if constexpr (SAVE && PACKS) {
#ifndef X16_DIAG_NOIMG
            x16_image_store<PREC>(hout[2 * ot], hout[2 * ot + 1], sv->tile0 + ot * 2 * X16_PIECE);
            ws.note_stores(2);
#endif
#ifndef X16_DIAG_NOGATE
            unsigned m = 0;
#pragma unroll
            for (int half = 0; half < 2; ++half) {
                const s16x8 hv = __builtin_bit_cast(s16x8, hout[2 * ot + half]);
#pragma unroll
                for (int j = 0; j < 8; ++j) m |= (hv[j] != 0 ? 1u : 0u) << (8 * half + j);
            }
            if constexpr (ot & 1) {
                __builtin_nontemporal_store(gate_word | (m << 16), sv->gate0 + (ot >> 1) * 64);
                ws.note_stores(1);
            } else {
                gate_word = m;
            }
#endif
        }
        if (MODE == MODE_DENSITY) {
            aux = acc[0];
        } else if (MODE == MODE_COMPOSITE) {
#pragma unroll
            for (int r = 0; r < 16; ++r) red[(ot & 1) * 16 + r] = fmaxf(acc[r], 0.0f) * aux;
            if constexpr (SAVE) {
#pragma unroll
                for (int half = 0; half < 2; ++half) {
                    float v[8];
#pragma unroll
                    for (int r = 0; r < 8; ++r) v[r] = fmaxf(acc[8 * half + r], 0.0f);
                    __builtin_nontemporal_store(X16<PREC>::pack(v), reinterpret_cast<frag*>(sv->tile0 + (2 * ot + half) * X16_PIECE));
                }
                ws.note_stores(2);
            }
            if (ot & 1) {
                float s = butterfly32(red, c);
                const int v = ((c & 1) << 4) | ((c & 2) << 2) | (c & 4) | ((c & 8) >> 2) | ((c & 16) >> 4);
                const int reg = v & 15, tile = (ot - 1) + (v >> 4);
                if (live) po[tile * 32 + (reg & 3) + 8 * (reg >> 2) + 4 * h] = s;
            }
        }
        X16_T(const unsigned long long s3 = x16_now(); ws.t_bias += s1 - s0; ws.t_mfma += (s2 - s1) - (ws.t_rv - rv0); ws.t_epi += s3 - s2;
              if (ws.tl && ws.tile_no >= 20 && ws.tile_no < 33 && (threadIdx.x & 63) == 0) {
                  ws.tl[4 + 2 * (ws.tile_no - 20)] = (float)(s1 & 0xFFFFFF);
                  ws.tl[5 + 2 * (ws.tile_no - 20)] = (float)(s2 & 0xFFFFFF);
              }
              ++ws.tile_no;)
    });
}

struct X16TrainSave {
    unsigned char* xT;
    unsigned char* gS;
    float* geo;
    unsigned* gates;
};

template <int PREC, int WAVES, bool SAVE = false>
__device__ __forceinline__ void nerf_fwd_x16_body(
    const N3dtGeom& g, const unsigned char* __restrict__ packed, const float* __restrict__ fold, const float* __restrict__ xy,
    const float* __restrict__ R, const float* __restrict__ T, const float* __restrict__ Kinv, const float* __restrict__ t_rand,
    float* __restrict__ part, float* __restrict__ wlocal, int bpr, long total_blocks, unsigned char* lds, const int wave,
    const X16TrainSave tsv = X16TrainSave{nullptr, nullptr, nullptr, nullptr}) {
    typedef typename X16<PREC>::frag frag;
    const int lane = threadIdx.x & 63;
    const int c = lane & 31, h = lane >> 5;
    X16_T(const unsigned long long t_entry = x16_now();)

    typedef WeightStream<PREC, WAVES, X16_NCHUNK, X16_NBUF, SAVE ? X16_SAVE_DEPTH : X16_DEPTH,
                         std::conditional_t<SAVE, X16Issue<>, X16Issue<X16_FWD_ISSUE>>> WS;
    WS ws;
    if constexpr (SAVE) {
        ws.gsrc = packed + (size_t)wave * WS::PPW * X16_PIECE + lane * 16;
    } else {
        ws.gsrc = packed + (size_t)wave * WS::PPW * X16_PIECE;
        ws.voff = lane * 16;
    }
    ws.ring = lds;
    ws.lds_addr0 = (unsigned)(size_t)(LDS_AS unsigned char*)lds + lane * 16;
    ws.wave = wave;
    ws.prologue_issue();
    unsigned char* pe_lds = lds + X16_NBUF * X16_CH * X16_PIECE + (size_t)wave * 4 * X16_PIECE + lane * 16;

    long blk = (long)blockIdx.x * WAVES + wave;
    const bool live = __builtin_amdgcn_readfirstlane((int)(blk < total_blocks)) != 0;
    if (!live) blk = total_blocks - 1;
    float* const po = part + (size_t)blk * N3DT_PART_STRIDE;
    float dist, zval;
    frag pe[4];
    const int sb = (int)(blk % bpr);
    const long ray0 = blk / bpr;
    const int ray = (int)(ray0 % g.n_rays);
    const int frame = (int)(ray0 / g.n_rays);
    {
        float p[3];
        n3dt_sample_point(g, xy, R, T, Kinv, t_rand, frame, ray, sb * X16_BS + c, p, dist, zval);
        pe_encode<PREC>(p, h, pe_lds, pe);
    }
    const float* fb = fold + (size_t)__builtin_amdgcn_readfirstlane(frame) * N3DT_FOLD_STRIDE;
    const float* b10 = fb + n3dt_bias_offset(10);
    if (g.vd_dim > 0) b10 = fold + n3dt_rayfold_offset(g.batch) + (size_t)__builtin_amdgcn_readfirstlane((int)ray0) * N3DT_RAYFOLD_STRIDE;
    X16SaveStage<PREC> svs;
    unsigned char* xT_blk = nullptr;
    const long rec = live ? blk : total_blocks;
    if constexpr (SAVE) {
        xT_blk = tsv.xT + (size_t)rec * X16_XT_TILES * 2 * X16_PIECE + x16_image_lane_offset(lane);
        pe_settle(pe);
        x16_image_store<PREC>(pe[0], pe[1], xT_blk);
        x16_image_store<PREC>(pe[2], pe[3], xT_blk + 2 * X16_PIECE);
    }
    auto sv_hidden = [&](const int l) -> const X16SaveStage<PREC>* {
        if constexpr (SAVE) {
            svs.tile0 = xT_blk + (size_t)(2 + 12 * l) * 2 * X16_PIECE;
            svs.gate0 = tsv.gates + ((size_t)rec * 8 + l) * 6 * 64 + lane;
            return &svs;
        } else {
            return nullptr;
        }
    };
    constexpr int BIAS = SAVE ? X16_BIAS_LDS_MFMA : X16_BIAS_LDS_C;
    constexpr int BIAS_DEN = BIAS == X16_BIAS_LDS_C ? X16_BIAS_LDS_C : X16_BIAS_GLOBAL_MFMA;
    X16BiasLds bl{nullptr, 0u};
    constexpr int DEN_AT = 192;
    bl.slots = lds + X16_NBUF * X16_CH * X16_PIECE + (size_t)WAVES * 4 * X16_PIECE + (size_t)wave * 2 * X16_BIAS_SLOT;
    bl.addr = (unsigned)(size_t)(LDS_AS unsigned char*)bl.slots + (BIAS == X16_BIAS_LDS_C ? 16 * h : 4 * c);
    bl.stage_in(fb + n3dt_bias_offset(0), 384, 0, lane);
    auto bias_slot = [&](const int k) -> unsigned {
        if (k < 7) {
            bl.stage_in(fb + n3dt_bias_offset(k + 1), 384, (k + 1) & 1, lane);
        } else {
            bl.stage_in(b10, 192, 0, lane);
            if constexpr (BIAS_DEN == X16_BIAS_LDS_C) bl.stage_in(fb + n3dt_bias_offset(8), 64, 0, lane, DEN_AT);
        }
        return bl.at(k & 1);
    };
    if constexpr (!SAVE) pe_settle(pe);
    ws.prologue_wait();
    X16_T(const unsigned long long t_head = x16_now() - t_entry;)
    X16_T(if (wlocal && live) ws.tl = wlocal + (size_t)blk * X16_BS;)
    X16TileInit ti;
    if constexpr (BIAS == X16_BIAS_LDS_C) ti.template issue<0, 0>(bl.at(0));

    frag ha[24], hb[24];
    float aux;
    x16_stage<PREC, WAVES, 4, 4, 12, MODE_HIDDEN, SAVE, BIAS, 0, true>(ws, ti, fb + n3dt_bias_offset(0), bias_slot(0), bl.at(1), pe, nullptr, ha, ha, aux, po, live, lane, sv_hidden(0));
    x16_stage<PREC, WAVES, 24, 0, 12, MODE_HIDDEN, SAVE, BIAS, 0, true>(ws, ti, fb + n3dt_bias_offset(1), bias_slot(1), bl.at(0), pe, nullptr, ha, hb, aux, po, live, lane, sv_hidden(1));
    x16_stage<PREC, WAVES, 24, 0, 12, MODE_HIDDEN, SAVE, BIAS, 0, true>(ws, ti, fb + n3dt_bias_offset(2), bias_slot(2), bl.at(1), pe, nullptr, hb, ha, aux, po, live, lane, sv_hidden(2));
    x16_stage<PREC, WAVES, 24, 0, 12, MODE_HIDDEN, SAVE, BIAS, 0, true>(ws, ti, fb + n3dt_bias_offset(3), bias_slot(3), bl.at(0), pe, nullptr, ha, hb, aux, po, live, lane, sv_hidden(3));
    x16_stage<PREC, WAVES, 24, 0, 12, MODE_HIDDEN, SAVE, BIAS, 0, true>(ws, ti, fb + n3dt_bias_offset(4), bias_slot(4), bl.at(1), pe, nullptr, hb, ha, aux, po, live, lane, sv_hidden(4));
    x16_stage<PREC, WAVES, 28, 4, 12, MODE_HIDDEN, SAVE, BIAS, 0, true>(ws, ti, fb + n3dt_bias_offset(5), bias_slot(5), bl.at(0), pe, pe_lds, ha, hb, aux, po, live, lane, sv_hidden(5));
    x16_stage<PREC, WAVES, 24, 0, 12, MODE_HIDDEN, SAVE, BIAS, 0, true>(ws, ti, fb + n3dt_bias_offset(6), bias_slot(6), bl.at(1), pe, nullptr, hb, ha, aux, po, live, lane, sv_hidden(6));
    x16_stage<PREC, WAVES, 24, 0, 12, MODE_HIDDEN, SAVE, BIAS, 0, true>(ws, ti, fb + n3dt_bias_offset(7), bias_slot(7), bl.at(0, DEN_AT), pe, nullptr, ha, hb, aux, po, live, lane, sv_hidden(7));
    x16_stage<PREC, WAVES, 24, 0, 1, MODE_DENSITY, false, BIAS_DEN, 0, true>(ws, ti, fb + n3dt_bias_offset(8), bl.at(0, DEN_AT), bl.at(0), pe, nullptr, hb, ha, aux, po, live, lane);
    {
        float sp = __shfl(aux, c, 64);
        if constexpr (SAVE) {
            if (live && h == 0) {
                tsv.geo[(size_t)blk * 64 + c] = sp;
                tsv.geo[(size_t)blk * 64 + 32 + c] = dist;
            }
        }
        float sigma = fmaxf(sp, 0.0f);
        float alpha = 1.0f - expf(-sigma * dist);
        float x = 1.0f - alpha + 1e-10f;
        float Tl = n3dt_exclusive_prod<32>(x, c);
        float w = alpha * Tl;
        float s0 = w, s1 = w * zval;
#pragma unroll
        for (int off = 16; off > 0; off >>= 1) {
            s0 += __shfl_xor(s0, off, 32);
            s1 += __shfl_xor(s1, off, 32);
        }
        float tprod = __shfl(Tl * x, 31, 32);
        if (live && lane == 0) {
            po[N3DT_G + 0] = s0;
            po[N3DT_G + 1] = s1;
            po[N3DT_G + 2] = tprod;
            po[N3DT_G + 3] = 0.0f;
        }
#ifndef X16_STAMP
        if (live && wlocal && h == 0) wlocal[(size_t)blk * X16_BS + c] = w;
#endif
        aux = w;
    }
    if constexpr (SAVE) {
        svs.tile0 = tsv.gS + (size_t)rec * 12 * X16_PIECE + lane * 16;
        svs.gate0 = nullptr;
    }
    x16_stage<PREC, WAVES, 24, 0, 6, MODE_COMPOSITE, SAVE, BIAS, 1, false>(ws, ti, b10, bl.at(0), 0u, pe, nullptr, hb, ha, aux, po, live, lane,
                                                                               SAVE ? &svs : nullptr);
#ifdef X16_STAMP
    if (wlocal && lane == 0 && live) {
        float* dbg = wlocal + (size_t)blk * X16_BS;
        dbg[0] = (float)ws.t_bias;
        dbg[1] = (float)ws.t_mfma;
        dbg[2] = (float)ws.t_epi;
        dbg[3] = (float)ws.t_rv;
        dbg[30] = (float)t_head;
    }
#endif
}

template <int PREC, int WAVES>
__global__ __launch_bounds__(WAVES * 64, 1) void nerf_fwd_x16_kernel(
    N3dtGeom g, const unsigned char* __restrict__ packed, const float* __restrict__ fold, const float* __restrict__ xy,
    const float* __restrict__ R, const float* __restrict__ T, const float* __restrict__ Kinv, const float* __restrict__ t_rand,
    float* __restrict__ part, float* __restrict__ wlocal, int bpr, long total_blocks) {
    extern __shared__ __attribute__((aligned(16))) unsigned char lds[];
    const int wave = __builtin_amdgcn_readfirstlane(threadIdx.x >> 6);
    nerf_fwd_x16_body<PREC, WAVES>(g, packed, fold, xy, R, T, Kinv, t_rand, part, wlocal, bpr, total_blocks, lds, wave);
}

template <int WAVES>
__global__ __launch_bounds__(WAVES * 64, 1) void nerf_fwd_x16_train_kernel(
    N3dtGeom g, const unsigned char* __restrict__ packed, const float* __restrict__ fold, const float* __restrict__ xy,
    const float* __restrict__ R, const float* __restrict__ T, const float* __restrict__ Kinv, const float* __restrict__ t_rand,
    float* __restrict__ part, float* __restrict__ wlocal, int bpr, long total_blocks, X16TrainSave tsv) {
    extern __shared__ __attribute__((aligned(16))) unsigned char lds[];
    const int wave = __builtin_amdgcn_readfirstlane(threadIdx.x >> 6);
    nerf_fwd_x16_body<N3DT_BF16, WAVES, true>(g, packed, fold, xy, R, T, Kinv, t_rand, part, wlocal, bpr, total_blocks, lds, wave,
                                                        tsv);
}

#ifndef X16_TRAIN_WAVES
#define X16_TRAIN_WAVES 8
#endif
extern "C" void n3dt_launch_nerf_fwd_x16_train(const N3dtGeom* g, const void* packed, const float* fold, const float* xy, const float* R,
                                               const float* T, const float* Kinv, const float* t_rand, float* part, float* wlocal,
                                               void* xT, void* gS, float* geo, void* gates, hipStream_t stream) {
    constexpr int WAVES = X16_TRAIN_WAVES;
    const int bpr = (g->n_samples + X16_BS - 1) / X16_BS;
    const long total = (long)g->batch * g->n_rays * bpr;
    const int grid = (int)((total + WAVES - 1) / WAVES);
    const size_t lds_bytes = X16_NBUF * X16_CH * X16_PIECE + (size_t)WAVES * 4 * X16_PIECE + (size_t)WAVES * 2 * X16_BIAS_SLOT;
    auto kern = nerf_fwd_x16_train_kernel<WAVES>;
    (void)hipFuncSetAttribute(reinterpret_cast<const void*>(kern), hipFuncAttributeMaxDynamicSharedMemorySize, (int)lds_bytes);
    X16TrainSave tsv{reinterpret_cast<unsigned char*>(xT), reinterpret_cast<unsigned char*>(gS), geo, reinterpret_cast<unsigned*>(gates)};
    hipLaunchKernelGGL(kern, dim3(grid), dim3(WAVES * 64), lds_bytes, stream, *g, reinterpret_cast<const unsigned char*>(packed), fold, xy,
                       R, T, Kinv, t_rand, part, wlocal, bpr, total, tsv);
}

template <int PREC>
static void launch_x16(const N3dtGeom* g, const void* packed, const float* fold, const float* xy, const float* R, const float* T,
                       const float* Kinv, const float* t_rand, float* part, float* wlocal, hipStream_t stream) {
    constexpr int WAVES = 8;
    const int bpr = (g->n_samples + X16_BS - 1) / X16_BS;
    const long total = (long)g->batch * g->n_rays * bpr;
    const int grid = (int)((total + WAVES - 1) / WAVES);
    const size_t lds_bytes = X16_NBUF * X16_CH * X16_PIECE + (size_t)WAVES * 4 * X16_PIECE + (size_t)WAVES * 2 * X16_BIAS_SLOT;
    auto kern = nerf_fwd_x16_kernel<PREC, WAVES>;
    (void)hipFuncSetAttribute(reinterpret_cast<const void*>(kern), hipFuncAttributeMaxDynamicSharedMemorySize, (int)lds_bytes);
    hipLaunchKernelGGL(kern, dim3(grid), dim3(WAVES * 64), lds_bytes, stream, *g, reinterpret_cast<const unsigned char*>(packed),
                       fold, xy, R, T, Kinv, t_rand, part, wlocal, bpr, total);
}

extern "C" void n3dt_launch_nerf_fwd_x16(const N3dtGeom* g, int precision, const void* packed, const float* fold, const float* xy,
                                         const float* R, const float* T, const float* Kinv, const float* t_rand, float* part,
                                         float* wlocal, hipStream_t stream) {
    if (precision == N3DT_BF16) launch_x16<N3DT_BF16>(g, packed, fold, xy, R, T, Kinv, t_rand, part, wlocal, stream);
    else launch_x16<N3DT_F16>(g, packed, fold, xy, R, T, Kinv, t_rand, part, wlocal, stream);
}
```

### nerf-3dtalker-code_amd/csrc/seams.hip

```cpp
#include "gemm32.h"
#include "n3dt_device.h"
#include "x16_core.h"

__global__ void seam_sample_kernel(N3dtGeom g, const float* __restrict__ xy, const float* __restrict__ R, const float* __restrict__ T,
                                   const float* __restrict__ Kinv, const float* __restrict__ t_rand, float* __restrict__ pts,
                                   float* __restrict__ zvals, float* __restrict__ z_dists, float* __restrict__ ray_d,
                                   float* __restrict__ ray_l) {
    const size_t total = (size_t)g.batch * g.n_rays * g.n_samples;
    const size_t i = (size_t)blockIdx.x * blockDim.x + threadIdx.x;
    if (i >= total) return;
    const int s = (int)(i % g.n_samples);
    const size_t rg = i / g.n_samples;
    const int ray = (int)(rg % g.n_rays), b = (int)(rg / g.n_rays);
    float p[3], dist, zval;
    n3dt_sample_point(g, xy, R, T, Kinv, t_rand, b, ray, s, p, dist, zval);
    const size_t M = (size_t)g.n_rays * g.n_samples, m = (size_t)ray * g.n_samples + s;
    if (pts)
#pragma unroll
        for (int d = 0; d < 3; ++d) pts[((size_t)b * 3 + d) * M + m] = p[d];
    if (zvals) zvals[(size_t)b * M + m] = zval;
    if (z_dists) z_dists[(size_t)b * M + m] = dist;
    if (s == 0 && (ray_d || ray_l)) {
        const float x = xy[(int64_t)b * g.xy_stride_b + (int64_t)ray * g.xy_stride_r];
        const float y = xy[(int64_t)b * g.xy_stride_b + g.xy_stride_c + (int64_t)ray * g.xy_stride_r];
        float d[3], l;
        n3dt_ray_setup(R + b * 9, Kinv + b * 9, x, y, d, l);
        if (ray_d)
#pragma unroll
            for (int k = 0; k < 3; ++k) ray_d[((size_t)b * 3 + k) * g.n_rays + ray] = d[k];
        if (ray_l) ray_l[(size_t)b * g.n_rays + ray] = l;
    }
}

extern "C" void n3dt_launch_sample_points(const N3dtGeom* g, const float* xy, const float* R, const float* T, const float* Kinv,
                                          const float* t_rand, float* pts, float* zvals, float* z_dists, float* ray_d, float* ray_l,
                                          hipStream_t s) {
    const size_t total = (size_t)g->batch * g->n_rays * g->n_samples;
    hipLaunchKernelGGL(seam_sample_kernel, dim3((unsigned)((total + 255) / 256)), dim3(256), 0, s, *g, xy, R, T, Kinv, t_rand, pts, zvals,
                       z_dists, ray_d, ray_l);
}

__global__ void seam_embed_kernel(int B, size_t M, const float* __restrict__ pts, float* __restrict__ pe) {
    const size_t i = (size_t)blockIdx.x * blockDim.x + threadIdx.x;
    if (i >= (size_t)B * M) return;
    const size_t b = i / M, m = i % M;
    const float p[3] = {pts[(b * 3 + 0) * M + m], pts[(b * 3 + 1) * M + m], pts[(b * 3 + 2) * M + m]};
    for (int r = 0; r < N3DT_PE_DIM; ++r) pe[(b * N3DT_PE_DIM + r) * M + m] = n3dt_pe_row_accurate(p, r);
}

extern "C" void n3dt_launch_embed(int B, size_t M, const float* pts, float* pe, hipStream_t s) {
    hipLaunchKernelGGL(seam_embed_kernel, dim3((unsigned)(((size_t)B * M + 255) / 256)), dim3(256), 0, s, B, M, pts, pe);
}

__global__ void seam_embed_freqs_kernel(int B, size_t M, int n_freqs, const float* __restrict__ pts, float* __restrict__ pe) {
    const size_t i = (size_t)blockIdx.x * blockDim.x + threadIdx.x;
    if (i >= (size_t)B * M) return;
    const size_t b = i / M, m = i % M;
    const int rows = 3 + 6 * n_freqs;
    const float p[3] = {pts[(b * 3 + 0) * M + m], pts[(b * 3 + 1) * M + m], pts[(b * 3 + 2) * M + m]};
    for (int r = 0; r < 3; ++r) pe[(b * rows + r) * M + m] = p[r];
    for (int k = 0; k < n_freqs; ++k)
        for (int d = 0; d < 3; ++d) {
            const float a = p[d] * (float)(1 << k);
            pe[(b * rows + 3 + 6 * k + d) * M + m] = sinf(a);
            pe[(b * rows + 3 + 6 * k + 3 + d) * M + m] = cosf(a);
        }
}
extern "C" void n3dt_launch_embed_freqs(int B, size_t M, int n_freqs, const float* pts, float* pe, hipStream_t s) {
    hipLaunchKernelGGL(seam_embed_freqs_kernel, dim3((unsigned)(((size_t)B * M + 255) / 256)), dim3(256), 0, s, B, M, n_freqs, pts, pe);
}

__global__ void seam_to_rows_kernel(int B, int C, size_t M, const float* __restrict__ src, float* __restrict__ dst, long ld, int col0) {
    __shared__ float tile[32][33];
    const int b = blockIdx.z, c0 = blockIdx.y * 32;
    const size_t m0 = (size_t)blockIdx.x * 32;
    const int tx = threadIdx.x & 31, ty = threadIdx.x >> 5;
    for (int i = ty; i < 32; i += 8) {
        const int c = c0 + i;
        const size_t m = m0 + tx;
        tile[i][tx] = (c < C && m < M) ? src[((size_t)b * C + c) * M + m] : 0.0f;
    }
    __syncthreads();
    for (int i = ty; i < 32; i += 8) {
        const size_t m = m0 + i;
        const int c = c0 + tx;
        if (c < C && m < M) dst[((size_t)b * M + m) * ld + col0 + c] = tile[tx][i];
    }
}
__global__ void seam_to_planes_kernel(int B, int C, size_t M, const float* __restrict__ src, long ld, float* __restrict__ dst, int relu) {
    __shared__ float tile[32][33];
    const int b = blockIdx.z, c0 = blockIdx.y * 32;
    const size_t m0 = (size_t)blockIdx.x * 32;
    const int tx = threadIdx.x & 31, ty = threadIdx.x >> 5;
    for (int i = ty; i < 32; i += 8) {
        const size_t m = m0 + i;
        const int c = c0 + tx;
        tile[i][tx] = (c < C && m < M) ? src[((size_t)b * M + m) * ld + c] : 0.0f;
    }
    __syncthreads();
    for (int i = ty; i < 32; i += 8) {
        const int c = c0 + i;
        const size_t m = m0 + tx;
        if (c < C && m < M) {
            const float v = tile[tx][i];
            dst[((size_t)b * C + c) * M + m] = relu ? fmaxf(v, 0.0f) : v;
        }
    }
}

struct SeamMlpWs {
    size_t in0, cat5, h[2], rin, g, out, total;
    long ld0, ld5, ldr;
};
static SeamMlpWs seam_mlp_layout(const N3dtGeom* g, size_t P) {
    SeamMlpWs w;
    auto al = [](size_t n) { return (n + 63) & ~(size_t)63; };
    const int vp = N3DT_PE_DIM + g->shape_dim;
    w.ld0 = (vp + g->audio_dim + 3) & ~3;
    w.ld5 = (vp + 384 + 3) & ~3;
    w.ldr = (384 + g->appea_dim + 3) & ~3;
    size_t o = 0;
    w.in0 = o; o += al(P * w.ld0);
    w.cat5 = o; o += al(P * w.ld5);
    w.h[0] = o; o += al(P * 384);
    w.h[1] = o; o += al(P * 384);
    w.rin = o; o += al(P * w.ldr);
    w.g = o; o += al(P * 192);
    w.out = o; o += al(P * 256);
    w.total = o;
    return w;
}
extern "C" size_t n3dt_seam_mlp_ws_floats(const N3dtGeom* g, size_t M) { return seam_mlp_layout(g, (size_t)g->batch * M).total; }

static Gemm32 smk(long M, int N, int K, const float* A, long lda, const float* Bw, long ldb, const float* bias, int relu, float* C, long ldc) {
    Gemm32 q;
    q.M = (int)M; q.N = N; q.K = K;
    q.A = A; q.lda = lda; q.a_kmajor = 0;
    q.B = Bw; q.ldb = ldb; q.b_kmajor = 0;
    q.C = C; q.ldc = ldc;
    q.bias = bias; q.bias_group_rows = 0; q.bias_ld = 0;
    q.act = relu ? G32_ACT_RELU : G32_ACT_NONE;
    q.gate = nullptr; q.ldgate = 0; q.gate_act = G32_ACT_NONE;
    q.accumulate = 0; q.split_k = 1;
    q.a16 = q.b16 = q.c16 = q.gate16 = 0;
    return q;
}

extern "C" void n3dt_launch_mlp_points(const N3dtGeom* g, size_t M, const N3dtMlpParams* p, const float* audio, const float* vps,
                                       const float* vds, float* rgb, float* density, float* ws, hipStream_t s) {
    const int B = g->batch, S = g->shape_dim, A = g->appea_dim, U = g->audio_dim, vp = N3DT_PE_DIM + S;
    const size_t P = (size_t)B * M;
    const SeamMlpWs wl = seam_mlp_layout(g, P);
    auto rows = [&](int C, const float* src, float* dst, long ld, int col0) {
        hipLaunchKernelGGL(seam_to_rows_kernel, dim3((unsigned)((M + 31) / 32), (C + 31) / 32, B), dim3(256), 0, s, B, C, M, src, dst, ld, col0);
    };
    float* in0 = ws + wl.in0;
    float* cat5 = ws + wl.cat5;
    float* rin = ws + wl.rin;
    rows(vp, vps, in0, wl.ld0, 0);
    if (U > 0) rows(U, audio, in0, wl.ld0, vp);
    rows(vp, vps, cat5, wl.ld5, 0);
    rows(A, vds, rin, wl.ldr, 384);
    const float* x = in0;
    long ldx = wl.ld0;
    int kx = vp + U;
    for (int i = 0; i < 8; ++i) {
        float* y = i == 4 ? cat5 + vp : ws + wl.h[i & 1];
        const long ldy = i == 4 ? wl.ld5 : 384;
        n3dt_gemm32(smk((long)P, 384, kx, x, ldx, p->weight[i], kx, p->bias[i], 1, y, ldy), s);
        if (i == 4) { x = cat5; ldx = wl.ld5; kx = vp + 384; }
        else { x = y; ldx = 384; kx = 384; }
    }
    n3dt_gemm32(smk((long)P, 1, 384, x, 384, p->weight[8], 384, p->bias[8], 1, density, 1), s);
    n3dt_gemm32(smk((long)P, 384, 384, x, 384, p->weight[9], 384, p->bias[9], 0, rin, wl.ldr), s);
    n3dt_gemm32(smk((long)P, 192, 384 + A, rin, wl.ldr, p->weight[10], 384 + A, p->bias[10], 1, ws + wl.g, 192), s);
    n3dt_gemm32(smk((long)P, 256, 192, ws + wl.g, 192, p->weight[11], 192, p->bias[11], 0, ws + wl.out, 256), s);
    hipLaunchKernelGGL(seam_to_planes_kernel, dim3((unsigned)((M + 31) / 32), 8, B), dim3(256), 0, s, B, 256, M, ws + wl.out, 256L, rgb, 0);
}

__global__ void seam_composite_kernel(int B, int Nr, int Ns, int C, const float* __restrict__ rgb, const float* __restrict__ density,
                                      const float* __restrict__ z_dists, const float* __restrict__ zvals, float* __restrict__ feat,
                                      float* __restrict__ bg_alpha, float* __restrict__ depth, float* __restrict__ weight) {
    extern __shared__ float w_lds[];
    const long rg = (long)blockIdx.x * 4 + (threadIdx.x >> 6);
    const int lane = threadIdx.x & 63;
    if (rg >= (long)B * Nr) return;
    const int b = (int)(rg / Nr), ray = (int)(rg % Nr);
    float* wl = w_lds + (size_t)(threadIdx.x >> 6) * Ns;
    const size_t base = ((size_t)b * Nr + ray) * Ns;
    float Trun = 1.0f, wsum = 0.0f, dsum = 0.0f;
    for (int s0 = 0; s0 < Ns; s0 += 64) {
        const int s = s0 + lane;
        float alpha = 0.0f, z = 0.0f;
        if (s < Ns) {
            alpha = 1.0f - expf(-density[base + s] * z_dists[base + s]);
            z = zvals[base + s];
        }
        const float x = 1.0f - alpha + 1e-10f;
        float incl = x;
#pragma unroll
        for (int off = 1; off < 64; off <<= 1) {
            const float o = __shfl_up(incl, off, 64);
            if (lane >= off) incl *= o;
        }
        float excl = __shfl_up(incl, 1, 64);
        if (lane == 0) excl = 1.0f;
        const float w = alpha * Trun * excl;
        if (s < Ns) {
            wl[s] = w;
            if (weight) weight[base + s] = w;
        }
        float a = w, d = w * z;
#pragma unroll
        for (int off = 32; off > 0; off >>= 1) {
            a += __shfl_xor(a, off, 64);
            d += __shfl_xor(d, off, 64);
        }
        wsum += a;
        dsum += d;
        Trun *= __shfl(incl, 63, 64);
    }
    if (lane == 0) {
        if (bg_alpha) bg_alpha[(size_t)b * Nr + ray] = 1.0f - wsum;
        if (depth) depth[(size_t)b * Nr + ray] = dsum;
    }
    for (int c = lane; c < C; c += 64) {
        const float* col = rgb + (((size_t)b * C + c) * Nr + ray) * Ns;
        float acc = 0.0f;
        for (int s = 0; s < Ns; ++s) acc = fmaf(wl[s], col[s], acc);
        feat[((size_t)b * C + c) * Nr + ray] = acc;
    }
}

extern "C" void n3dt_launch_composite(int B, int Nr, int Ns, int C, const float* rgb, const float* density, const float* z_dists,
                                      const float* zvals, float* feat, float* bg_alpha, float* depth, float* weight, hipStream_t s) {
    const long rays = (long)B * Nr;
    hipLaunchKernelGGL(seam_composite_kernel, dim3((unsigned)((rays + 3) / 4)), dim3(256), sizeof(float) * 4 * Ns, s, B, Nr, Ns, C, rgb,
                       density, z_dists, zvals, feat, bg_alpha, depth, weight);
}

template <int PREC, int FORM>
__global__ void __launch_bounds__(64) x16_pack_probe_kernel(size_t n, const float* __restrict__ in, unsigned short* __restrict__ out) {
    typedef typename X16<PREC>::frag frag;
    typedef typename std::conditional<PREC == N3DT_BF16, __bf16, _Float16>::type elem;
    const size_t base = (size_t)blockIdx.x * 512 + (size_t)threadIdx.x * 8;
    if (base + 8 > n) return;
    float v[8];
#pragma unroll
    for (int j = 0; j < 8; ++j) v[j] = in[base + j];
    frag f;
    if constexpr (FORM == 0) {
        f = X16<PREC>::pack(v);
    } else {
#pragma unroll
        for (int j = 0; j < 8; ++j) f[j] = (elem)v[j];
    }
    *reinterpret_cast<frag*>(out + base) = f;
}

template <int PREC, int FORM>
__global__ void __launch_bounds__(64) x16_pe_probe_kernel(size_t n, const float* __restrict__ points, unsigned short* __restrict__ out) {
    typedef typename X16<PREC>::frag frag;
    __shared__ __attribute__((aligned(16))) unsigned char pe_wave[4 * X16_PIECE];
    const int lane = threadIdx.x, c = lane & 31, h = lane >> 5;
    const size_t pt = (size_t)blockIdx.x * 32 + c;
    if ((size_t)blockIdx.x * 32 + 32 > n) return;
    const float p[3] = {points[3 * pt], points[3 * pt + 1], points[3 * pt + 2]};
    frag pe[4];
    if constexpr (FORM == 0) {
        pe_encode<PREC>(p, h, pe_wave + 16 * lane, pe);
        pe_settle(pe);
    } else {
        float rh[3], rl[3];
#pragma unroll
        for (int i = 0; i < 3; ++i) pe_phase(p[i], rh[i], rl[i]);
#pragma unroll
        for (int ks = 0; ks < 4; ++ks) {
            float v[8];
#pragma unroll
            for (int j = 0; j < 8; ++j)
                v[j] = pe_fast(p[0], p[1], p[2], rh[0], rh[1], rh[2], rl[0], rl[1], rl[2], 16 * ks + 8 * (j >> 2) + 4 * h + (j & 3));
            pe[ks] = X16<PREC>::pack(v);
        }
    }
#pragma unroll
    for (int ks = 0; ks < 4; ++ks) *reinterpret_cast<frag*>(out + (((size_t)blockIdx.x * 4 + ks) * 64 + lane) * 8) = pe[ks];
}

extern "C" void n3dt_launch_x16_pe_probe(int precision, int form, size_t n, const float* points, unsigned short* out, hipStream_t s) {
    const dim3 grid((unsigned)(n / 32)), block(64);
    if (precision == N3DT_BF16) {
        if (form == 0) hipLaunchKernelGGL((x16_pe_probe_kernel<N3DT_BF16, 0>), grid, block, 0, s, n, points, out);
        else hipLaunchKernelGGL((x16_pe_probe_kernel<N3DT_BF16, 1>), grid, block, 0, s, n, points, out);
    } else {
        if (form == 0) hipLaunchKernelGGL((x16_pe_probe_kernel<N3DT_F16, 0>), grid, block, 0, s, n, points, out);
        else hipLaunchKernelGGL((x16_pe_probe_kernel<N3DT_F16, 1>), grid, block, 0, s, n, points, out);
    }
}

extern "C" void n3dt_launch_x16_pack_probe(int precision, int form, size_t n, const float* in, unsigned short* out, hipStream_t s) {
    const dim3 grid((unsigned)(n / 512)), block(64);
    if (precision == N3DT_BF16) {
        if (form == 0) hipLaunchKernelGGL((x16_pack_probe_kernel<N3DT_BF16, 0>), grid, block, 0, s, n, in, out);
        else hipLaunchKernelGGL((x16_pack_probe_kernel<N3DT_BF16, 1>), grid, block, 0, s, n, in, out);
    } else {
        if (form == 0) hipLaunchKernelGGL((x16_pack_probe_kernel<N3DT_F16, 0>), grid, block, 0, s, n, in, out);
        else hipLaunchKernelGGL((x16_pack_probe_kernel<N3DT_F16, 1>), grid, block, 0, s, n, in, out);
    }
}
```

### nerf-3dtalker-code_amd/n3dt/_lib.py

```python
import ctypes
import os

_HERE = os.path.dirname(os.path.abspath(__file__))
LIB_PATH = os.environ.get("N3DT_LIB") or os.path.join(os.path.dirname(_HERE), "lib", "libn3dt.so")

F32, BF16, F16, BF16X3 = 0, 1, 2, 3
PRECISIONS = {"fp32": F32, "f32": F32, "bf16": BF16, "fp16": F16, "f16": F16, "bf16x3": BF16X3}
MLP_LAYERS = 12
MAX_BLOCKS = 8

MLP_ORDER = ["FeaExt_module_%d" % i for i in range(8)] + ["density_module", "RGB_layer_0", "RGB_layer_1", "RGB_layer_2"]


class Geom(ctypes.Structure):
    _fields_ = [
        ("batch", ctypes.c_int32), ("n_rays", ctypes.c_int32), ("n_samples", ctypes.c_int32),
        ("hidden", ctypes.c_int32), ("feat_nc", ctypes.c_int32), ("shape_dim", ctypes.c_int32),
        ("appea_dim", ctypes.c_int32), ("audio_dim", ctypes.c_int32), ("featmap_size", ctypes.c_int32),
        ("n_blocks", ctypes.c_int32), ("world_z1", ctypes.c_float), ("world_z2", ctypes.c_float),
        ("xy_stride_b", ctypes.c_int64), ("xy_stride_c", ctypes.c_int64), ("xy_stride_r", ctypes.c_int64),
        ("z_planes_given", ctypes.c_int32), ("bg_is_hwc", ctypes.c_int32), ("vd_dim", ctypes.c_int32),
    ]


VGG_CONVS = 10


class VggParams(ctypes.Structure):
    _fields_ = [("weight", ctypes.c_void_p * VGG_CONVS), ("bias", ctypes.c_void_p * VGG_CONVS)]


LPIPS_LAYERS = 5
LPIPS_INPUT_MODES = {"reference": 0, "standard": 1}


class LpipsParams(ctypes.Structure):
    _fields_ = [("weight", ctypes.c_void_p * LPIPS_LAYERS), ("bias", ctypes.c_void_p * LPIPS_LAYERS), ("lin", ctypes.c_void_p * LPIPS_LAYERS)]


SYNCNET_BLOCKS = 31


class SyncnetParams(ctypes.Structure):
    _fields_ = [(name, ctypes.c_void_p * SYNCNET_BLOCKS) for name in ("weight", "bias", "bn_weight", "bn_bias", "bn_mean", "bn_var")]


class A2sParams(ctypes.Structure):
    _fields_ = [("w_ih", ctypes.c_void_p * 4), ("w_hh", ctypes.c_void_p * 4), ("b_ih", ctypes.c_void_p * 4), ("b_hh", ctypes.c_void_p * 4),
                ("lin_w", ctypes.c_void_p * 3), ("lin_b", ctypes.c_void_p * 3)]


class AdamTensor(ctypes.Structure):
    _fields_ = [("param", ctypes.c_void_p), ("grad", ctypes.c_void_p), ("exp_avg", ctypes.c_void_p), ("exp_avg_sq", ctypes.c_void_p),
                ("numel", ctypes.c_int64), ("group", ctypes.c_int32), ("active", ctypes.c_int32)]


class AdamChunk(ctypes.Structure):
    _fields_ = [("start", ctypes.c_int64), ("tensor", ctypes.c_int32), ("length", ctypes.c_int32)]


class AdamGroup(ctypes.Structure):
    _fields_ = [("lr", ctypes.c_double), ("beta1", ctypes.c_double), ("beta2", ctypes.c_double), ("eps", ctypes.c_double),
                ("weight_decay", ctypes.c_double), ("maximize", ctypes.c_int32), ("reserved", ctypes.c_int32)]


class AdamGuard(ctypes.Structure):
    _fields_ = [("max_grad_norm", ctypes.c_float), ("skip_nonfinite", ctypes.c_int32), ("grad_norm", ctypes.c_float),
                ("clip_coef", ctypes.c_float), ("skip", ctypes.c_int32), ("skipped_steps", ctypes.c_int32),
                ("norm_done", ctypes.c_int32), ("reserved", ctypes.c_int32)]


GUARD_HOST_BYTES = 8
ADAM_MAX_GROUPS = 64
ADAM_COUNTER_INTS = 4

A2S_MAX_T = 256
A2S_GRAD_FLOATS = 20726784


class MlpParams(ctypes.Structure):
    _fields_ = [("weight", ctypes.c_void_p * MLP_LAYERS), ("bias", ctypes.c_void_p * MLP_LAYERS)]


class RenderParams(ctypes.Structure):
    _fields_ = [
        ("to_rgb_w", ctypes.c_void_p * (MAX_BLOCKS + 1)), ("to_rgb_b", ctypes.c_void_p * (MAX_BLOCKS + 1)),
        ("psu1_w", ctypes.c_void_p * MAX_BLOCKS), ("psu1_b", ctypes.c_void_p * MAX_BLOCKS),
        ("psu2_w", ctypes.c_void_p * MAX_BLOCKS), ("psu2_b", ctypes.c_void_p * MAX_BLOCKS),
        ("feat_w", ctypes.c_void_p * MAX_BLOCKS), ("feat_b", ctypes.c_void_p * MAX_BLOCKS),
    ]


EXPORTS = [
    "n3dt_abi_version", "n3dt_last_error", "n3dt_mlp_packed_bytes", "n3dt_mlp_pack",
    "n3dt_render_workspace_bytes", "n3dt_render_fwd", "n3dt_neural_render_workspace_bytes",
    "n3dt_neural_render_fwd", "n3dt_chw_to_hwc", "n3dt_prof_enable", "n3dt_prof_collect",
    "n3dt_render_train_saved_bytes", "n3dt_render_train_workspace_bytes", "n3dt_render_train_fwd", "n3dt_render_bwd",
    "n3dt_render_bwd_cam",
    "n3dt_neural_render_train_saved_bytes", "n3dt_neural_render_train_workspace_bytes",
    "n3dt_neural_render_train_fwd", "n3dt_neural_render_bwd", "n3dt_loss_fwd", "n3dt_loss_bwd", "n3dt_fine_sample",
    "n3dt_img_to_uint8", "n3dt_sample_points", "n3dt_embed", "n3dt_mlp_points_workspace_bytes", "n3dt_mlp_points", "n3dt_composite",
    "n3dt_ray_vd_bias", "n3dt_embed_freqs",
    "n3dt_neural_render_pack", "n3dt_neural_render_fwd_reuse", "n3dt_stage_inputs", "n3dt_graph_begin", "n3dt_graph_end", "n3dt_graph_launch", "n3dt_graph_destroy",
    "n3dt_vgg_packed_bytes", "n3dt_vgg_pack", "n3dt_vgg_saved_bytes", "n3dt_vgg_workspace_bytes", "n3dt_vgg_loss_fwd", "n3dt_vgg_loss_bwd",
    "n3dt_a2s_saved_bytes", "n3dt_a2s_workspace_bytes", "n3dt_a2s_fwd", "n3dt_a2s_bwd",
    "n3dt_flat_adam_record_bytes", "n3dt_flat_adam_step",
    "n3dt_render_fwd16", "n3dt_neural_render_fwd16_reuse", "n3dt_feat_to_rgb0",
    "n3dt_x16_pack_probe", "n3dt_x16_pe_probe",
    "n3dt_eval_metrics_workspace_bytes", "n3dt_eval_metrics",
    "n3dt_lpips_packed_bytes", "n3dt_lpips_pack", "n3dt_lpips_workspace_bytes", "n3dt_lpips",
    "n3dt_mel_workspace_bytes", "n3dt_mel_spectrogram", "n3dt_mel_windows",
    "n3dt_syncnet_packed_bytes", "n3dt_syncnet_pack", "n3dt_syncnet_workspace_bytes", "n3dt_syncnet_face_windows", "n3dt_syncnet_fwd",
    "n3dt_syncnet_block",
]

GUARD_EXPORTS = ["n3dt_flat_adam_guard_bytes", "n3dt_flat_adam_guarded_step"]

STAGE_MAX = 12


class Stage(ctypes.Structure):
    _fields_ = [("src", ctypes.c_void_p * STAGE_MAX), ("dst", ctypes.c_void_p * STAGE_MAX), ("count", ctypes.c_int64 * STAGE_MAX),
                ("view_dims", ctypes.c_int64 * 3), ("view_strides", ctypes.c_int64 * 3), ("n", ctypes.c_int32)]


_LIB = None


class N3dtError(RuntimeError):
    pass


def lib():
    global _LIB
    if _LIB is not None:
        return _LIB
    if not os.path.exists(LIB_PATH):
        raise N3dtError("libn3dt.so not found at %s -- the HIP extension is required (no CPU fallback); "
                        "run `make -C nerf-3dtalker-code_amd`" % LIB_PATH)
    L = ctypes.CDLL(LIB_PATH)
    vp, sz, ci = ctypes.c_void_p, ctypes.c_size_t, ctypes.c_int
    L.n3dt_abi_version.restype = ci
    L.n3dt_last_error.restype = ctypes.c_char_p
    L.n3dt_mlp_packed_bytes.restype = sz
    L.n3dt_mlp_packed_bytes.argtypes = [ctypes.POINTER(Geom), ci]
    L.n3dt_mlp_pack.restype = ci
    L.n3dt_mlp_pack.argtypes = [ctypes.POINTER(Geom), ci, ctypes.POINTER(MlpParams), vp, vp]
    L.n3dt_render_workspace_bytes.restype = sz
    L.n3dt_render_workspace_bytes.argtypes = [ctypes.POINTER(Geom), ci]
    L.n3dt_render_fwd.restype = ci
    L.n3dt_render_fwd.argtypes = [ctypes.POINTER(Geom), ci, vp, ctypes.POINTER(MlpParams)] + [vp] * 15 + [vp, sz, vp]
    L.n3dt_render_fwd16.restype = ci
    L.n3dt_render_fwd16.argtypes = [ctypes.POINTER(Geom), ci, vp, ctypes.POINTER(MlpParams)] + [vp] * 19 + [vp, sz, vp]
    L.n3dt_neural_render_workspace_bytes.restype = sz
    L.n3dt_neural_render_workspace_bytes.argtypes = [ctypes.POINTER(Geom), ci]
    L.n3dt_neural_render_fwd.restype = ci
    L.n3dt_neural_render_fwd.argtypes = [ctypes.POINTER(Geom), ci, ci, ctypes.POINTER(RenderParams), vp, vp, vp, sz, vp]
    L.n3dt_neural_render_fwd_reuse.restype = ci
    L.n3dt_neural_render_fwd_reuse.argtypes = [ctypes.POINTER(Geom), ci, ci, ctypes.POINTER(RenderParams), vp, vp, vp, sz, vp]
    L.n3dt_neural_render_fwd16_reuse.restype = ci
    L.n3dt_neural_render_fwd16_reuse.argtypes = [ctypes.POINTER(Geom), ci, ci, ctypes.POINTER(RenderParams), vp, vp, vp, vp, sz, vp]
    L.n3dt_feat_to_rgb0.restype = ci
    L.n3dt_feat_to_rgb0.argtypes = [ci, ci, vp, vp, vp, vp, vp]
    L.n3dt_neural_render_pack.restype = ci
    L.n3dt_neural_render_pack.argtypes = [ctypes.POINTER(Geom), ci, ci, ctypes.POINTER(RenderParams), vp, sz, vp]
    L.n3dt_chw_to_hwc.restype = ci
    L.n3dt_chw_to_hwc.argtypes = [ci, ci, vp, vp, vp]
    gp, mp, rp = ctypes.POINTER(Geom), ctypes.POINTER(MlpParams), ctypes.POINTER(RenderParams)
    L.n3dt_render_train_saved_bytes.restype = sz
    L.n3dt_render_train_saved_bytes.argtypes = [gp]
    L.n3dt_render_train_workspace_bytes.restype = sz
    L.n3dt_render_train_workspace_bytes.argtypes = [gp]
    L.n3dt_render_train_fwd.restype = ci
    L.n3dt_render_train_fwd.argtypes = [gp, ci, vp, mp] + [vp] * 14 + [vp, sz, vp, sz, vp]
    L.n3dt_render_bwd.restype = ci
    L.n3dt_render_bwd.argtypes = [gp, ci, mp, mp] + [vp] * 7 + [vp, sz] + [vp] * 12 + [vp, sz, vp]
    L.n3dt_render_bwd_cam.restype = ci
    L.n3dt_render_bwd_cam.argtypes = [gp, ci, mp, mp] + [vp] * 7 + [vp, sz] + [vp] * 14 + [vp, sz, vp]
    L.n3dt_neural_render_train_saved_bytes.restype = sz
    L.n3dt_neural_render_train_saved_bytes.argtypes = [gp, ci]
    L.n3dt_neural_render_train_workspace_bytes.restype = sz
    L.n3dt_neural_render_train_workspace_bytes.argtypes = [gp, ci]
    L.n3dt_neural_render_train_fwd.restype = ci
    L.n3dt_neural_render_train_fwd.argtypes = [gp, ci, ci, rp, vp, vp, vp, sz, vp, sz, vp]
    L.n3dt_neural_render_bwd.restype = ci
    L.n3dt_neural_render_bwd.argtypes = [gp, ci, ci, rp, rp, vp, vp, vp, sz, vp, vp, sz, vp]
    L.n3dt_loss_fwd.restype = ci
    L.n3dt_loss_fwd.argtypes = [ci, ci, vp, vp, vp, vp, ctypes.c_float, vp, vp, vp]
    L.n3dt_loss_bwd.restype = ci
    L.n3dt_loss_bwd.argtypes = [ci, ci, vp, vp, vp, vp, ctypes.c_float, vp, vp, vp, vp, vp, vp]
    L.n3dt_prof_enable.restype = ci
    L.n3dt_prof_enable.argtypes = [ci]
    L.n3dt_prof_collect.restype = ci
    L.n3dt_prof_collect.argtypes = [ctypes.POINTER(ctypes.c_float), ci, ctypes.POINTER(ci)]
    L.n3dt_fine_sample.restype = ci
    L.n3dt_fine_sample.argtypes = [gp, ci, vp, vp, vp, vp, vp, vp]
    L.n3dt_img_to_uint8.restype = ci
    L.n3dt_img_to_uint8.argtypes = [ci, ci, vp, vp, vp]
    L.n3dt_sample_points.restype = ci
    L.n3dt_sample_points.argtypes = [gp] + [vp] * 10 + [vp]
    L.n3dt_embed.restype = ci
    L.n3dt_embed.argtypes = [ci, sz, vp, vp, vp]
    L.n3dt_embed_freqs.restype = ci
    L.n3dt_embed_freqs.argtypes = [ci, sz, ci, vp, vp, vp]
    L.n3dt_ray_vd_bias.restype = ci
    L.n3dt_ray_vd_bias.argtypes = [gp, vp, ctypes.c_int64, vp, vp, vp, vp, vp]
    L.n3dt_mlp_points_workspace_bytes.restype = sz
    L.n3dt_mlp_points_workspace_bytes.argtypes = [gp, sz]
    L.n3dt_mlp_points.restype = ci
    L.n3dt_mlp_points.argtypes = [gp, sz, mp] + [vp] * 5 + [vp, sz, vp]
    L.n3dt_composite.restype = ci
    L.n3dt_composite.argtypes = [ci, ci, ci, ci] + [vp] * 8 + [vp]
    L.n3dt_x16_pack_probe.restype = ci
    L.n3dt_x16_pack_probe.argtypes = [ci, ci, sz, vp, vp, vp]
    L.n3dt_x16_pe_probe.restype = ci
    L.n3dt_x16_pe_probe.argtypes = [ci, ci, sz, vp, vp, vp]
    L.n3dt_stage_inputs.restype = ci
    L.n3dt_stage_inputs.argtypes = [ctypes.POINTER(Stage), vp]
    L.n3dt_graph_begin.restype = ci
    L.n3dt_graph_begin.argtypes = [vp]
    L.n3dt_graph_end.restype = ci
    L.n3dt_graph_end.argtypes = [vp, ctypes.POINTER(vp)]
    L.n3dt_graph_launch.restype = ci
    L.n3dt_graph_launch.argtypes = [vp, vp]
    L.n3dt_graph_destroy.restype = ci
    L.n3dt_graph_destroy.argtypes = [vp]
    L.n3dt_vgg_packed_bytes.restype = sz
    L.n3dt_vgg_packed_bytes.argtypes = [ci]
    L.n3dt_vgg_pack.restype = ci
    L.n3dt_vgg_pack.argtypes = [ci, ctypes.POINTER(VggParams), vp, vp]
    L.n3dt_vgg_saved_bytes.restype = sz
    L.n3dt_vgg_saved_bytes.argtypes = [ci, ci]
    L.n3dt_vgg_workspace_bytes.restype = sz
    L.n3dt_vgg_workspace_bytes.argtypes = [ci, ci, ci]
    L.n3dt_vgg_loss_fwd.restype = ci
    L.n3dt_vgg_loss_fwd.argtypes = [ci, ci, ci, vp, vp, vp, vp, ctypes.c_float, vp, vp, sz, vp, sz, vp]
    L.n3dt_vgg_loss_bwd.restype = ci
    L.n3dt_vgg_loss_bwd.argtypes = [ci, ci, ci, vp, vp, vp, vp, sz, vp, vp, sz, vp]
    L.n3dt_a2s_saved_bytes.restype = sz
    L.n3dt_a2s_saved_bytes.argtypes = [ci]
    L.n3dt_a2s_workspace_bytes.restype = sz
    L.n3dt_a2s_workspace_bytes.argtypes = [ci]
    L.n3dt_a2s_fwd.restype = ci
    L.n3dt_a2s_fwd.argtypes = [ci, ctypes.POINTER(A2sParams), vp, vp, vp, vp, vp, vp, sz, vp, sz, vp]
    L.n3dt_a2s_bwd.restype = ci
    L.n3dt_a2s_bwd.argtypes = [ci, ctypes.POINTER(A2sParams), vp, vp, sz, vp, vp, sz, vp]
    L.n3dt_flat_adam_record_bytes.restype = sz
    L.n3dt_flat_adam_record_bytes.argtypes = [ci]
    L.n3dt_flat_adam_step.restype = ci
    L.n3dt_flat_adam_step.argtypes = [vp, vp, ci, vp, ci, vp, vp]
    L.n3dt_eval_metrics_workspace_bytes.restype = sz
    L.n3dt_eval_metrics_workspace_bytes.argtypes = [ci, ci, ci]
    L.n3dt_eval_metrics.restype = ci
    L.n3dt_eval_metrics.argtypes = [ci, ci, ci, vp, vp, vp, vp, vp, sz, vp]
    L.n3dt_lpips_packed_bytes.restype = sz
    L.n3dt_lpips_packed_bytes.argtypes = []
    L.n3dt_lpips_pack.restype = ci
    L.n3dt_lpips_pack.argtypes = [ctypes.POINTER(LpipsParams), vp, vp]
    L.n3dt_lpips_workspace_bytes.restype = sz
    L.n3dt_lpips_workspace_bytes.argtypes = [ci, ci, ci]
    L.n3dt_lpips.restype = ci
    L.n3dt_lpips.argtypes = [ci, ci, ci, ci, vp, vp, vp, vp, vp, vp, sz, vp]
    i64 = ctypes.c_int64
    L.n3dt_mel_workspace_bytes.restype = sz
    L.n3dt_mel_workspace_bytes.argtypes = []
    L.n3dt_mel_spectrogram.restype = ci
    L.n3dt_mel_spectrogram.argtypes = [i64, vp, i64, vp, i64, i64, ci, vp, vp, vp, i64, ci, vp, sz, vp]
    L.n3dt_mel_windows.restype = ci
    L.n3dt_mel_windows.argtypes = [i64, vp, i64, ci, ci, vp, vp, vp]
    L.n3dt_syncnet_packed_bytes.restype = sz
    L.n3dt_syncnet_packed_bytes.argtypes = []
    L.n3dt_syncnet_pack.restype = ci
    L.n3dt_syncnet_pack.argtypes = [ctypes.POINTER(SyncnetParams), vp, vp]
    L.n3dt_syncnet_workspace_bytes.restype = sz
    L.n3dt_syncnet_workspace_bytes.argtypes = [ci]
    L.n3dt_syncnet_face_windows.restype = ci
    L.n3dt_syncnet_face_windows.argtypes = [ci, ci, ci, vp, vp, ci, vp, vp]
    L.n3dt_syncnet_fwd.restype = ci
    L.n3dt_syncnet_fwd.argtypes = [ci, vp, vp, vp, vp, vp, ci, ci, ci, vp, vp, vp, vp, sz, vp]
    L.n3dt_syncnet_block.restype = ci
    L.n3dt_syncnet_block.argtypes = [ci, ci, vp, vp, vp, vp, sz, vp]
    L.n3dt_flat_adam_guard_bytes.restype = sz
    L.n3dt_flat_adam_guard_bytes.argtypes = []
    L.n3dt_flat_adam_guarded_step.restype = ci
    L.n3dt_flat_adam_guarded_step.argtypes = [vp, vp, ci, vp, ci, vp, vp, vp, vp]
    if L.n3dt_abi_version() != 5:
        raise N3dtError("libn3dt.so ABI version mismatch")
    if L.n3dt_flat_adam_guard_bytes() != ctypes.sizeof(AdamGuard):
        raise N3dtError("libn3dt.so: N3dtAdamGuard differs from its ctypes mirror")
    for which, rec in enumerate((AdamTensor, AdamChunk, AdamGroup)):
        if L.n3dt_flat_adam_record_bytes(which) != ctypes.sizeof(rec):
            raise N3dtError("libn3dt.so: FlatAdam table record %d differs from its ctypes mirror" % which)
    _LIB = L
    return L


PROF_ACTIVE = False


def prof_enable(max_records):
    global PROF_ACTIVE
    check(lib().n3dt_prof_enable(int(max_records)), "n3dt_prof_enable")
    PROF_ACTIVE = max_records > 0


def check(rc, what):
    if rc != 0:
        raise N3dtError("%s failed (%d): %s" % (what, rc, lib().n3dt_last_error().decode()))
```

### nerf-3dtalker-code_amd/n3dt/ops.py

```python
import ctypes

import torch

from . import _lib
from ._lib import Geom, MlpParams, RenderParams, check, lib


def _stream():
    return ctypes.c_void_p(torch.cuda.current_stream().cuda_stream)


def _ptr(t):
    if t is None:
        return None
    assert t.is_cuda, "libn3dt works on device memory only (no CPU fallback)"
    return ctypes.c_void_p(t.data_ptr())


def _f32c(t):
    return t.detach().to(dtype=torch.float32).contiguous()


class _Workspace:

    def __init__(self):
        self.buf = {}

    def get(self, key, nbytes, device):
        assert device.type == "cuda", "libn3dt works on device memory only (no CPU fallback)"
        k = (key, device.index, torch.cuda.current_stream(device).cuda_stream)
        b = self.buf.get(k)
        if b is None or b.numel() < nbytes:
            b = torch.empty(max(int(nbytes), 256), dtype=torch.uint8, device=device)
            self.buf[k] = b
        return b


WORKSPACE = _Workspace()


def make_geom(batch, n_rays, n_samples, hidden, feat_nc, shape_dim, appea_dim, audio_dim, featmap_size, n_blocks,
              world_z1, world_z2, xy_strides=(0, 0, 0), z_planes_given=0, bg_is_hwc=0, vd_dim=0):
    g = Geom()
    g.z_planes_given = int(z_planes_given)
    g.bg_is_hwc = int(bg_is_hwc)
    g.vd_dim = int(vd_dim)
    g.batch, g.n_rays, g.n_samples = int(batch), int(n_rays), int(n_samples)
    g.hidden, g.feat_nc = int(hidden), int(feat_nc)
    g.shape_dim, g.appea_dim, g.audio_dim = int(shape_dim), int(appea_dim), int(audio_dim)
    g.featmap_size, g.n_blocks = int(featmap_size), int(n_blocks)
    g.world_z1, g.world_z2 = float(world_z1), float(world_z2)
    g.xy_stride_b, g.xy_stride_c, g.xy_stride_r = [int(s) for s in xy_strides]
    return g


def mlp_params(weights, biases):
    p = MlpParams()
    for i, (w, b) in enumerate(zip(weights, biases)):
        assert w.is_cuda and w.dtype == torch.float32 and w.is_contiguous()
        assert b.is_cuda and b.dtype == torch.float32 and b.is_contiguous()
        p.weight[i] = w.data_ptr()
        p.bias[i] = b.data_ptr()
    return p


def render_params(to_rgb, psu1, psu2, feat):
    p = RenderParams()
    for i, (w, b) in enumerate(to_rgb):
        p.to_rgb_w[i], p.to_rgb_b[i] = w.data_ptr(), b.data_ptr()
    for i, (w, b) in enumerate(psu1):
        p.psu1_w[i], p.psu1_b[i] = w.data_ptr(), b.data_ptr()
    for i, (w, b) in enumerate(psu2):
        p.psu2_w[i], p.psu2_b[i] = w.data_ptr(), b.data_ptr()
    for i, (w, b) in enumerate(feat):
        p.feat_w[i], p.feat_b[i] = w.data_ptr(), b.data_ptr()
    return p


def pack_mlp(geom, precision, params, device, out=None):
    nbytes = lib().n3dt_mlp_packed_bytes(ctypes.byref(geom), precision)
    if nbytes == 0:
        raise _lib.N3dtError("n3dt_mlp_packed_bytes: " + lib().n3dt_last_error().decode())
    packed = out if out is not None and out.numel() >= nbytes else torch.empty(nbytes, dtype=torch.uint8, device=device)
    check(lib().n3dt_mlp_pack(ctypes.byref(geom), precision, ctypes.byref(params), _ptr(packed), _stream()), "n3dt_mlp_pack")
    return packed


def render_workspace_bytes(geom, precision):
    return _bytes_or_raise(lib().n3dt_render_workspace_bytes(ctypes.byref(geom), precision), "n3dt_render_workspace_bytes")


def render_fwd(geom, precision, packed, params, xy, R, T, Kinv, shape, appea, audio, t_rand, bg_featmap,
               want_depth=False, want_weight=False, want_merge=True, merge_out=None, want_fg=True, weight_out=None, ws=None, ray_bias=None,
               merge16_out=None, rgb0_out=None, rgb0_wb=None):
    dev = xy.device
    B, Nr, Ns, C = geom.batch, geom.n_rays, geom.n_samples, geom.feat_nc
    assert want_fg or want_merge
    map16 = merge16_out is not None or rgb0_out is not None
    if map16:
        assert want_merge and (merge16_out is None or (merge16_out.is_contiguous() and merge16_out.element_size() == 2))
        assert rgb0_out is None or (rgb0_wb is not None and rgb0_out.is_contiguous() and rgb0_out.dtype == torch.float32)
    out = {
        "fg_feat": torch.empty(B, Nr, C, dtype=torch.float32, device=dev) if want_fg else None,
        "bg_alpha": torch.empty(B, Nr, dtype=torch.float32, device=dev) if want_fg else None,
        "depth": torch.empty(B, Nr, dtype=torch.float32, device=dev) if want_depth else None,
        "weight": (weight_out if weight_out is not None else torch.empty(B, Nr, Ns, dtype=torch.float32, device=dev))
        if want_weight else None,
        "merge_feat": (merge_out if merge_out is not None else None if map16 else torch.empty(B, Nr, C, dtype=torch.float32, device=dev))
        if want_merge else None,
    }
    ws_bytes = render_workspace_bytes(geom, precision)
    if ws is None:
        ws = WORKSPACE.get("render", ws_bytes, dev)
    assert ws.numel() >= ws_bytes
    if map16:
        out["merge_feat16"], out["rgb0"] = merge16_out, rgb0_out
        rc = lib().n3dt_render_fwd16(
            ctypes.byref(geom), precision, _ptr(packed), ctypes.byref(params), _ptr(xy), _ptr(R), _ptr(T), _ptr(Kinv),
            _ptr(shape), _ptr(appea), _ptr(audio), _ptr(t_rand), _ptr(bg_featmap), _ptr(ray_bias),
            _ptr(out["fg_feat"]), _ptr(out["bg_alpha"]), _ptr(out["depth"]), _ptr(out["weight"]), _ptr(out["merge_feat"]),
            _ptr(merge16_out), _ptr(rgb0_out), _ptr(rgb0_wb[0]) if rgb0_wb else None, _ptr(rgb0_wb[1]) if rgb0_wb else None,
            _ptr(ws), ws_bytes, _stream())
        check(rc, "n3dt_render_fwd16")
        return out
    rc = lib().n3dt_render_fwd(
        ctypes.byref(geom), precision, _ptr(packed), ctypes.byref(params), _ptr(xy), _ptr(R), _ptr(T), _ptr(Kinv),
        _ptr(shape), _ptr(appea), _ptr(audio), _ptr(t_rand), _ptr(bg_featmap) if want_merge else None, _ptr(ray_bias),
        _ptr(out["fg_feat"]), _ptr(out["bg_alpha"]), _ptr(out["depth"]), _ptr(out["weight"]), _ptr(out["merge_feat"]),
        _ptr(ws), ws_bytes, _stream())
    check(rc, "n3dt_render_fwd")
    return out


def fine_sample(geom, n_fine, weight, T, t_rand=None, u=None, out=None):
    B, Nr, Nc = geom.batch, geom.n_rays, geom.n_samples
    z = out if out is not None else torch.empty(B, Nr, Nc + n_fine + 1, dtype=torch.float32, device=weight.device)
    check(lib().n3dt_fine_sample(ctypes.byref(geom), int(n_fine), _ptr(weight), _ptr(T), _ptr(t_rand), _ptr(u), _ptr(z), _stream()),
          "n3dt_fine_sample")
    return z


def img_to_uint8(img):
    img = _f32c(img)
    V, _, P, Q = img.shape
    out = torch.empty(V, P, Q, 3, dtype=torch.uint8, device=img.device)
    check(lib().n3dt_img_to_uint8(V, P * Q, _ptr(img), _ptr(out), _stream()), "n3dt_img_to_uint8")
    return out


def sample_points(geom, xy, R, T, Kinv, t_rand=None):
    B, Nr, Ns, dev = geom.batch, geom.n_rays, geom.n_samples, xy.device
    out = {"pts": torch.empty(B, 3, Nr, Ns, dtype=torch.float32, device=dev),
           "zvals": torch.empty(B, 1, Nr, Ns, dtype=torch.float32, device=dev),
           "z_dists": torch.empty(B, 1, Nr, Ns, dtype=torch.float32, device=dev),
           "ray_d": torch.empty(B, 3, Nr, dtype=torch.float32, device=dev),
           "ray_l": torch.empty(B, 1, Nr, dtype=torch.float32, device=dev)}
    check(lib().n3dt_sample_points(ctypes.byref(geom), _ptr(xy), _ptr(R), _ptr(T), _ptr(Kinv), _ptr(t_rand), _ptr(out["pts"]),
                                   _ptr(out["zvals"]), _ptr(out["z_dists"]), _ptr(out["ray_d"]), _ptr(out["ray_l"]), _stream()),
          "n3dt_sample_points")
    return out


def embed(pts):
    pts = _f32c(pts)
    B = pts.shape[0]
    M = pts[0, 0].numel()
    pe = torch.empty((B, 63) + tuple(pts.shape[2:]), dtype=torch.float32, device=pts.device)
    check(lib().n3dt_embed(B, M, _ptr(pts), _ptr(pe), _stream()), "n3dt_embed")
    return pe


def embed_freqs(pts, n_freqs):
    pts = _f32c(pts)
    B = pts.shape[0]
    M = pts[0, 0].numel()
    pe = torch.empty((B, 3 + 6 * n_freqs) + tuple(pts.shape[2:]), dtype=torch.float32, device=pts.device)
    check(lib().n3dt_embed_freqs(B, M, int(n_freqs), _ptr(pts), _ptr(pe), _stream()), "n3dt_embed_freqs")
    return pe


def x16_pack_probe(x, precision, form=0):
    x = _f32c(x)
    prec = _lib.PRECISIONS[precision] if isinstance(precision, str) else int(precision)
    out = torch.empty(x.shape, dtype=torch.bfloat16 if prec == _lib.BF16 else torch.float16, device=x.device)
    check(lib().n3dt_x16_pack_probe(prec, int(form), x.numel(), _ptr(x), _ptr(out), _stream()), "n3dt_x16_pack_probe")
    return out


def x16_pe_probe(points, precision, form=0):
    points = _f32c(points)
    assert points.dim() == 2 and points.shape[1] == 3, "points must be [n, 3]"
    n = points.shape[0]
    prec = _lib.PRECISIONS[precision] if isinstance(precision, str) else int(precision)
    out = torch.empty((n // 32, 4, 64, 8), dtype=torch.bfloat16 if prec == _lib.BF16 else torch.float16, device=points.device)
    check(lib().n3dt_x16_pe_probe(prec, int(form), n, _ptr(points), _ptr(out), _stream()), "n3dt_x16_pe_probe")
    return out


def ray_vd_bias(geom, w_rgb1, xy, R, Kinv, out=None):
    assert w_rgb1.is_contiguous() and w_rgb1.dim() == 2 and w_rgb1.shape[0] == 192 and w_rgb1.shape[1] >= 384 + 27
    B, Nr = geom.batch, geom.n_rays
    rb = out if out is not None else torch.empty(B, Nr, 192, dtype=torch.float32, device=xy.device)
    w_vd = ctypes.c_void_p(w_rgb1.data_ptr() + 384 * 4)
    check(lib().n3dt_ray_vd_bias(ctypes.byref(geom), w_vd, int(w_rgb1.shape[1]), _ptr(xy), _ptr(R), _ptr(Kinv), _ptr(rb), _stream()),
          "n3dt_ray_vd_bias")
    return rb


def mlp_points(geom, params, audio, embed_vps, embed_vds):
    vps, vds = _f32c(embed_vps), _f32c(embed_vds)
    aud = _f32c(audio) if geom.audio_dim > 0 else None
    B = vps.shape[0]
    M = vps[0, 0].numel()
    tail = tuple(vps.shape[2:])
    rgb = torch.empty((B, geom.feat_nc) + tail, dtype=torch.float32, device=vps.device)
    dens = torch.empty((B, 1) + tail, dtype=torch.float32, device=vps.device)
    wb = _bytes_or_raise(lib().n3dt_mlp_points_workspace_bytes(ctypes.byref(geom), M), "n3dt_mlp_points_workspace_bytes")
    ws = WORKSPACE.get("seam_mlp", wb, vps.device)
    check(lib().n3dt_mlp_points(ctypes.byref(geom), M, ctypes.byref(params), _ptr(aud), _ptr(vps), _ptr(vds), _ptr(rgb), _ptr(dens),
                                _ptr(ws), wb, _stream()), "n3dt_mlp_points")
    return rgb, dens


def composite(rgb, density, z_dists, zvals):
    rgb, density, z_dists, zvals = _f32c(rgb), _f32c(density), _f32c(z_dists), _f32c(zvals)
    B, C, Nr, Ns = rgb.shape
    dev = rgb.device
    feat = torch.empty(B, C, Nr, dtype=torch.float32, device=dev)
    ba = torch.empty(B, 1, Nr, dtype=torch.float32, device=dev)
    dp = torch.empty(B, 1, Nr, dtype=torch.float32, device=dev)
    w = torch.empty(B, 1, Nr, Ns, dtype=torch.float32, device=dev)
    check(lib().n3dt_composite(B, Nr, Ns, C, _ptr(rgb), _ptr(density), _ptr(z_dists), _ptr(zvals), _ptr(feat), _ptr(ba), _ptr(dp), _ptr(w),
                               _stream()), "n3dt_composite")
    return feat, ba, dp, w


def neural_render_workspace_bytes(geom, nb):
    ws_bytes = lib().n3dt_neural_render_workspace_bytes(ctypes.byref(geom), nb)
    if ws_bytes == 0:
        raise _lib.N3dtError("n3dt_neural_render_workspace_bytes: unsupported geometry")
    return ws_bytes


def neural_render_pack(geom, nb, rparams, precision, ws):
    check(lib().n3dt_neural_render_pack(ctypes.byref(geom), nb, precision, ctypes.byref(rparams), _ptr(ws), ws.numel(), _stream()),
          "n3dt_neural_render_pack")


def neural_render_fwd(geom, nb, rparams, featmap, precision=0, img=None, ws=None, reuse_packed=False):
    dev = featmap.device
    P = geom.featmap_size << geom.n_blocks
    if img is None:
        img = torch.empty(nb, 3, P, P, dtype=torch.float32, device=dev)
    ws_bytes = neural_render_workspace_bytes(geom, nb)
    if ws is None:
        ws = WORKSPACE.get("nr", ws_bytes, dev)
    assert ws.numel() >= ws_bytes
    fn = lib().n3dt_neural_render_fwd_reuse if reuse_packed else lib().n3dt_neural_render_fwd
    check(fn(ctypes.byref(geom), nb, precision, ctypes.byref(rparams), _ptr(featmap), _ptr(img), _ptr(ws), ws_bytes, _stream()),
          "n3dt_neural_render_fwd")
    return img


def feat_to_rgb0(featmap, w, b):
    nb, n_pix, C = featmap.shape
    assert C == 256 and featmap.is_contiguous() and featmap.dtype == torch.float32
    out = torch.empty(nb, 3, n_pix, dtype=torch.float32, device=featmap.device)
    check(lib().n3dt_feat_to_rgb0(nb, n_pix, _ptr(featmap), _ptr(w), _ptr(b), _ptr(out), _stream()), "n3dt_feat_to_rgb0")
    return out


def neural_render_fwd16(geom, nb, rparams, featmap16, rgb0, precision, img=None, ws=None):
    P = geom.featmap_size << geom.n_blocks
    if img is None:
        img = torch.empty(nb, 3, P, P, dtype=torch.float32, device=featmap16.device)
    ws_bytes = neural_render_workspace_bytes(geom, nb)
    assert ws is not None and ws.numel() >= ws_bytes and featmap16.element_size() == 2 and featmap16.is_contiguous()
    check(lib().n3dt_neural_render_fwd16_reuse(ctypes.byref(geom), nb, precision, ctypes.byref(rparams), _ptr(featmap16), _ptr(rgb0), _ptr(img),
                                               _ptr(ws), ws_bytes, _stream()), "n3dt_neural_render_fwd16_reuse")
    return img


def chw_to_hwc(src, C, n, dst=None):
    if dst is None:
        dst = torch.empty(n, C, dtype=torch.float32, device=src.device)
    check(lib().n3dt_chw_to_hwc(C, n, _ptr(src), _ptr(dst), _stream()), "n3dt_chw_to_hwc")
    return dst


def stage_inputs(pairs, view=None):
    st = _lib.Stage()
    assert 1 <= len(pairs) <= _lib.STAGE_MAX
    for i, (src, dst) in enumerate(pairs):
        assert src.is_cuda and dst.is_cuda and src.dtype == torch.float32 and dst.dtype == torch.float32 and dst.is_contiguous()
        assert src.numel() == dst.numel() and (i == 0 and view is not None or src.is_contiguous())
        st.src[i], st.dst[i], st.count[i] = src.data_ptr(), dst.data_ptr(), src.numel()
    if view is not None:
        assert view.dim() == 3
        for d in range(3):
            st.view_dims[d], st.view_strides[d] = view.shape[d], view.stride(d)
    st.n = len(pairs)
    check(lib().n3dt_stage_inputs(ctypes.byref(st), _stream()), "n3dt_stage_inputs")


def graph_begin(stream):
    check(lib().n3dt_graph_begin(ctypes.c_void_p(stream.cuda_stream)), "n3dt_graph_begin")


def graph_end(stream):
    h = ctypes.c_void_p()
    check(lib().n3dt_graph_end(ctypes.c_void_p(stream.cuda_stream), ctypes.byref(h)), "n3dt_graph_end")
    return h


def graph_launch(handle):
    check(lib().n3dt_graph_launch(handle, _stream()), "n3dt_graph_launch")


def graph_destroy(handle):
    if handle:
        lib().n3dt_graph_destroy(handle)


def _bytes_or_raise(n, what):
    if n == 0:
        raise _lib.N3dtError(what + ": " + lib().n3dt_last_error().decode())
    return n


def render_train_fwd(geom, packed, params, xy, R, T, Kinv, shape, appea, audio, t_rand, bg_featmap, precision=0, merge_out=None, ray_bias=None):
    dev = xy.device
    B, Nr, C = geom.batch, geom.n_rays, geom.feat_nc
    if merge_out is not None:
        assert merge_out.is_contiguous() and tuple(merge_out.shape) == (B, Nr, C) and merge_out.dtype == torch.float32
    out = {
        "fg_feat": torch.empty(B, Nr, C, dtype=torch.float32, device=dev),
        "bg_alpha": torch.empty(B, Nr, dtype=torch.float32, device=dev),
        "merge_feat": merge_out if merge_out is not None else torch.empty(B, Nr, C, dtype=torch.float32, device=dev),
    }
    sbytes = _bytes_or_raise(lib().n3dt_render_train_saved_bytes(ctypes.byref(geom)), "n3dt_render_train_saved_bytes")
    wbytes = _bytes_or_raise(lib().n3dt_render_train_workspace_bytes(ctypes.byref(geom)), "n3dt_render_train_workspace_bytes")
    saved = torch.empty(sbytes, dtype=torch.uint8, device=dev)
    ws = WORKSPACE.get("train", wbytes, dev)
    check(lib().n3dt_render_train_fwd(
        ctypes.byref(geom), precision, _ptr(packed), ctypes.byref(params), _ptr(xy), _ptr(R), _ptr(T), _ptr(Kinv), _ptr(shape), _ptr(appea),
        _ptr(audio), _ptr(t_rand), _ptr(bg_featmap), _ptr(ray_bias), _ptr(out["fg_feat"]), _ptr(out["bg_alpha"]), None, _ptr(out["merge_feat"]),
        _ptr(saved), sbytes, _ptr(ws), wbytes, _stream()), "n3dt_render_train_fwd")
    return out, saved


def render_bwd(geom, params, grads, shape, appea, audio, bg_featmap, d_merge, saved, cam=None, precision=0, d_bg=None, frozen=False,
               cam_grads=None):
    dev = d_merge.device
    B, Nr, C = geom.batch, geom.n_rays, geom.feat_nc
    if frozen:
        assert grads is None
        d_bg = None
    elif d_bg is None:
        d_bg = torch.zeros(C, Nr, dtype=torch.float32, device=dev)
    S_, A_, U_ = geom.shape_dim, geom.appea_dim, geom.audio_dim
    codes = torch.empty(B * (S_ + A_ + U_), dtype=torch.float32, device=dev)
    d_shape = codes[:B * S_].view(B, S_)
    d_appea = codes[B * S_:B * (S_ + A_)].view(B, A_)
    d_audio = codes[B * (S_ + A_):].view(B, U_) if U_ > 0 else None
    d_R = d_T = d_Kinv = d_xy = None
    cam_ptrs = [None] * 5
    if cam is not None:
        want = ("R", "T") if cam_grads is None else tuple(cam_grads)
        assert set(want) <= {"R", "T", "Kinv", "xy"}
        if "R" in want:
            d_R = torch.empty(B, 3, 3, dtype=torch.float32, device=dev)
        if "T" in want:
            d_T = torch.empty(B, 3, dtype=torch.float32, device=dev)
        if "Kinv" in want:
            d_Kinv = torch.zeros(B, 3, 3, dtype=torch.float32, device=dev)
        if "xy" in want:
            d_xy = torch.empty(B, 2, Nr, dtype=torch.float32, device=dev)
        cam_ptrs = [_ptr(t) for t in cam]
    d_ray = torch.empty(B, Nr, 192, dtype=torch.float32, device=dev) if geom.vd_dim > 0 else None
    wbytes = lib().n3dt_render_train_workspace_bytes(ctypes.byref(geom))
    ws = WORKSPACE.get("train", wbytes, dev)
    head = (ctypes.byref(geom), precision, ctypes.byref(params), None if grads is None else ctypes.byref(grads), _ptr(shape), _ptr(appea),
            _ptr(audio), _ptr(bg_featmap),
            _ptr(d_merge), None, None, _ptr(saved), saved.numel(), _ptr(d_bg), _ptr(d_shape), _ptr(d_appea), _ptr(d_audio), _ptr(d_ray),
            *cam_ptrs, _ptr(d_R), _ptr(d_T))
    if cam_grads is None:
        check(lib().n3dt_render_bwd(*head, _ptr(ws), wbytes, _stream()), "n3dt_render_bwd")
    else:
        check(lib().n3dt_render_bwd_cam(*head, _ptr(d_Kinv), _ptr(d_xy), _ptr(ws), wbytes, _stream()), "n3dt_render_bwd_cam")
    res = (d_bg, d_shape, d_appea, d_audio, d_R, d_T) + ((d_ray,) if d_ray is not None else ())
    return res if cam_grads is None else res + (d_Kinv, d_xy)


def neural_render_train_fwd(geom, nb, rparams, featmap, precision=0):
    dev = featmap.device
    P = geom.featmap_size << geom.n_blocks
    img = torch.empty(nb, 3, P, P, dtype=torch.float32, device=dev)
    sbytes = _bytes_or_raise(lib().n3dt_neural_render_train_saved_bytes(ctypes.byref(geom), nb), "n3dt_neural_render_train_saved_bytes")
    wbytes = _bytes_or_raise(lib().n3dt_neural_render_train_workspace_bytes(ctypes.byref(geom), nb),
                             "n3dt_neural_render_train_workspace_bytes")
    saved = torch.empty(sbytes, dtype=torch.uint8, device=dev)
    ws = WORKSPACE.get("nr_train", wbytes, dev)
    check(lib().n3dt_neural_render_train_fwd(ctypes.byref(geom), nb, precision, ctypes.byref(rparams), _ptr(featmap), _ptr(img), _ptr(saved), sbytes,
                                             _ptr(ws), wbytes, _stream()), "n3dt_neural_render_train_fwd")
    return img, saved


def neural_render_bwd(geom, nb, rparams, rgrads, featmap, d_img, saved, precision=0):
    dev = featmap.device
    d_feat = torch.empty_like(featmap)
    wbytes = lib().n3dt_neural_render_train_workspace_bytes(ctypes.byref(geom), nb)
    ws = WORKSPACE.get("nr_train", wbytes, dev)
    check(lib().n3dt_neural_render_bwd(ctypes.byref(geom), nb, precision, ctypes.byref(rparams), None if rgrads is None else ctypes.byref(rgrads),
                                       _ptr(featmap), _ptr(d_img),
                                       _ptr(saved), saved.numel(), _ptr(d_feat), _ptr(ws), wbytes, _stream()), "n3dt_neural_render_bwd")
    return d_feat
```

Before: 2130 frames/s.

## Precompute per-ray direction table in fold kernel; use 2D grid block indexing

Result: no change. 2139 frames/s, median of 6 (+0.4%).

```diff
diff --git a/include/n3dt.h b/include/n3dt.h
--- a/include/n3dt.h
+++ b/include/n3dt.h
@@ -114,6 +114,8 @@
                    const float* zvals, float* feat, float* bg_alpha, float* depth, float* weight, void* stream);
 int n3dt_x16_pack_probe(int precision, int form, size_t n, const float* in, uint16_t* out, void* stream);
 int n3dt_x16_pe_probe(int precision, int form, size_t n, const float* points, uint16_t* out, void* stream);
+int n3dt_x16_head_probe(const N3dtGeom* g, const float* xy, const float* R, const float* T, const float* Kinv, const float* t_rand,
+                        float* out, void* workspace, void* stream);
 
 size_t n3dt_neural_render_workspace_bytes(const N3dtGeom* g, int nb);
 int n3dt_neural_render_fwd(const N3dtGeom* g, int nb, int precision, const N3dtRenderParams* p, const float* featmap,
diff --git a/nerf-3dtalker-code_amd/csrc/n3dt_api.hip b/nerf-3dtalker-code_amd/csrc/n3dt_api.hip
--- a/nerf-3dtalker-code_amd/csrc/n3dt_api.hip
+++ b/nerf-3dtalker-code_amd/csrc/n3dt_api.hip
@@ -38,8 +38,12 @@
 void n3dt_launch_fine_sample(const N3dtGeom*, int, const float*, const float*, const float*, const float*, float*, hipStream_t);
 void n3dt_launch_nerf_fwd_f32(const N3dtGeom*, const N3dtMlpParams*, const void*, const float*, const float*, const float*,
                               const float*, const float*, const float*, float*, float*, hipStream_t);
-void n3dt_launch_nerf_fwd_x16(const N3dtGeom*, int, const void*, const float*, const float*, const float*, const float*,
+void n3dt_launch_nerf_fwd_x16(const N3dtGeom*, int, const void*, const float*, const float*, const float*, const float*, const float*,
                               const float*, const float*, float*, float*, hipStream_t);
+void n3dt_launch_fold_rays(const N3dtGeom*, const N3dtMlpParams*, const float*, const float*, const float*, float*, int, const float*,
+                           const float*, const float*, float*, hipStream_t);
+void n3dt_launch_ray_table(const N3dtGeom*, const float*, const float*, const float*, float*, hipStream_t);
+void n3dt_launch_x16_head_probe(const N3dtGeom*, const float*, const float*, const float*, float*, hipStream_t);
 void n3dt_launch_nerf_fwd_x16s(const N3dtGeom*, const void*, const float*, const float*, const float*, const float*, const float*,
                                const float*, float*, float*, hipStream_t);
 size_t n3dt_nr_workspace_floats(const N3dtGeom*, int);
@@ -145,7 +149,7 @@
 static inline size_t align256(size_t b) { return (b + 255) & ~(size_t)255; }
 
 struct RenderCarve {
-    size_t fold, part, wlocal, bghwc, total;
+    size_t fold, raytab, part, wlocal, bghwc, total;
     int bpr, bs;
 };
 
@@ -155,7 +159,8 @@
     c.bpr = (g->n_samples + c.bs - 1) / c.bs;
     const size_t blocks = (size_t)g->batch * g->n_rays * c.bpr;
     c.fold = 0;
-    c.part = align256(n3dt_fold_region_floats(g->batch, g->n_rays, g->vd_dim) * sizeof(float));
+    c.raytab = align256(n3dt_fold_region_floats(g->batch, g->n_rays, g->vd_dim) * sizeof(float));
+    c.part = c.raytab + align256((size_t)g->batch * g->n_rays * 4 * sizeof(float));
     c.wlocal = c.part + align256(blocks * (192 + 4) * sizeof(float));
     c.bghwc = c.wlocal + align256(blocks * c.bs * sizeof(float));
     c.total = c.bghwc + align256((size_t)g->n_rays * g->feat_nc * sizeof(float));
@@ -257,12 +262,16 @@
     if (g->z_planes_given && !t_rand) return fail(N3DT_EINVAL, "n3dt_render_fwd: z_planes_given but no planes passed as t_rand");
     const RenderCarve c = render_carve(g, precision);
     if (workspace_bytes < c.total) return fail(N3DT_EWORKSPACE, "n3dt_render_fwd: workspace too small");
+    const bool x16 = precision == N3DT_BF16 || precision == N3DT_F16;
+    if (x16 && (size_t)g->n_rays * c.bpr >= ((size_t)1 << 31)) return fail(N3DT_EINVAL, "n3dt_render_fwd: 2^31 or more sample blocks per frame");
     hipStream_t s = (hipStream_t)stream;
     unsigned char* ws = (unsigned char*)workspace;
     float* fold = (float*)(ws + c.fold);
     float* part = (float*)(ws + c.part);
     float* wlocal = (float*)(ws + c.wlocal);
-    n3dt_launch_fold(g, p, shape, appea, audio, fold, precision != N3DT_F32, s);
+    float* raytab = (float*)(ws + c.raytab);
+    if (x16) n3dt_launch_fold_rays(g, p, shape, appea, audio, fold, 1, xy, R, Kinv, raytab, s);
+    else n3dt_launch_fold(g, p, shape, appea, audio, fold, precision != N3DT_F32, s);
     if (ray_bias) n3dt_launch_rayfold(g, fold, ray_bias, s);
     const int span = n3dt_prof_span_begin(s);
     if (precision == N3DT_F32)
@@ -270,7 +279,7 @@
     else if (precision == N3DT_BF16X3)
         n3dt_launch_nerf_fwd_x16s(g, packed_mlp, fold, xy, R, T, Kinv, t_rand, part, weight ? wlocal : nullptr, s);
     else
-        n3dt_launch_nerf_fwd_x16(g, precision, packed_mlp, fold, xy, R, T, Kinv, t_rand, part, weight ? wlocal : nullptr, s);
+        n3dt_launch_nerf_fwd_x16(g, precision, packed_mlp, fold, raytab, xy, R, T, Kinv, t_rand, part, weight ? wlocal : nullptr, s);
     n3dt_prof_span_end(span, s);
     const float* tail = (const float*)((const unsigned char*)packed_mlp + n3dt_packed_tail_offset(precision));
     const float* bghwc = bg_featmap;
@@ -385,6 +394,19 @@
     if (!points || !out) return fail(N3DT_EINVAL, "n3dt_x16_pe_probe: NULL argument");
     n3dt_launch_x16_pe_probe(precision, form, n, points, out, (hipStream_t)stream);
     return check_hip("n3dt_x16_pe_probe");
+}
+
+extern "C" int n3dt_x16_head_probe(const N3dtGeom* g, const float* xy, const float* R, const float* T, const float* Kinv,
+                                   const float* t_rand, float* out, void* workspace, void* stream) {
+    int rc = check_geom(g, N3DT_BF16);
+    if (rc) return rc;
+    if (!xy || !R || !T || !Kinv || !out || !workspace) return fail(N3DT_EINVAL, "n3dt_x16_head_probe: NULL argument");
+    if (g->z_planes_given && !t_rand) return fail(N3DT_EINVAL, "n3dt_x16_head_probe: z_planes_given but no planes passed as t_rand");
+    if ((size_t)g->n_rays * ((g->n_samples + 31) / 32) >= ((size_t)1 << 31))
+        return fail(N3DT_EINVAL, "n3dt_x16_head_probe: 2^31 or more sample blocks per frame");
+    n3dt_launch_ray_table(g, xy, R, Kinv, (float*)workspace, (hipStream_t)stream);
+    n3dt_launch_x16_head_probe(g, (const float*)workspace, T, t_rand, out, (hipStream_t)stream);
+    return check_hip("n3dt_x16_head_probe");
 }
 
 extern "C" int n3dt_fine_sample(const N3dtGeom* g, int n_fine, const float* weight, const float* T, const float* t_rand, const float* u,
diff --git a/nerf-3dtalker-code_amd/csrc/n3dt_device.h b/nerf-3dtalker-code_amd/csrc/n3dt_device.h
--- a/nerf-3dtalker-code_amd/csrc/n3dt_device.h
+++ b/nerf-3dtalker-code_amd/csrc/n3dt_device.h
@@ -95,6 +95,66 @@
     }
 }
 
+#define N3DT_RAYTAB_STRIDE 4
+__device__ __forceinline__ void n3dt_ray_table_entry(const N3dtGeom& g, const float* __restrict__ xy, const float* __restrict__ R,
+                                                     const float* __restrict__ Kinv, int b, int ray, float* __restrict__ raytab) {
+    float x = xy[(int64_t)b * g.xy_stride_b + 0 * g.xy_stride_c + (int64_t)ray * g.xy_stride_r];
+    float y = xy[(int64_t)b * g.xy_stride_b + 1 * g.xy_stride_c + (int64_t)ray * g.xy_stride_r];
+    float d[3], l;
+    n3dt_ray_setup(R + b * 9, Kinv + b * 9, x, y, d, l);
+    *reinterpret_cast<f32x4*>(raytab + ((size_t)b * g.n_rays + ray) * N3DT_RAYTAB_STRIDE) = f32x4{d[0] * l, d[1] * l, d[2] * l, l};
+}
+
+__device__ __forceinline__ void n3dt_sample_point_tab(const N3dtGeom& g, const float* __restrict__ raytab, const float* __restrict__ T,
+                                                      const float* __restrict__ t_rand, int b, int ray, int s, float p[3],
+                                                      float& dist, float& zval) {
+    const float* Tb = T + b * 3;
+    const float* rt = raytab + ((size_t)b * g.n_rays + ray) * N3DT_RAYTAB_STRIDE;
+    const float dl[3] = {rt[0], rt[1], rt[2]};
+    const float l = rt[3];
+    float rz1 = Tb[2] - g.world_z1, rz2 = Tb[2] - g.world_z2;
+    const int Ns = g.n_samples;
+    if (s < Ns) {
+        const float* tr = t_rand ? t_rand + ((int64_t)b * g.n_rays + ray) * (Ns + 1) : nullptr;
+        float z_lo, z_hi;
+        if (g.z_planes_given) {
+            z_lo = tr[s];
+            z_hi = tr[s + 1];
+        } else {
+            z_lo = n3dt_edge_z(rz1, rz2, s, Ns, tr);
+            z_hi = n3dt_edge_z(rz1, rz2, s + 1, Ns, tr);
+        }
+        dist = (z_hi - z_lo) * l;
+        zval = z_lo;
+#pragma unroll
+        for (int i = 0; i < 3; ++i) p[i] = Tb[i] + dl[i] * z_lo;
+    } else {
+        dist = 0.0f;
+        zval = 0.0f;
+        p[0] = p[1] = p[2] = 0.0f;
+    }
+}
+
+struct N3dtBlockIndex {
+    unsigned blk, ray, sb;
+    bool live;
+};
+__device__ __forceinline__ N3dtBlockIndex n3dt_block_index(const unsigned wg, const int waves, const int wave, const unsigned bpf,
+                                                           const unsigned bpr, const int bpr_sh) {
+    N3dtBlockIndex v;
+    v.blk = wg * waves + wave;
+    v.live = v.blk < bpf;
+    if (!v.live) v.blk = bpf - 1;
+    if (bpr_sh >= 0) {
+        v.ray = v.blk >> bpr_sh;
+        v.sb = v.blk & (bpr - 1);
+    } else {
+        v.ray = v.blk / bpr;
+        v.sb = v.blk - v.ray * bpr;
+    }
+    return v;
+}
+
 __device__ __forceinline__ float n3dt_pe_row_accurate(const float p[3], int row) {
     if (row < 3) return row == 0 ? p[0] : (row == 1 ? p[1] : p[2]);
     if (row >= N3DT_PE_DIM) return 0.0f;
diff --git a/nerf-3dtalker-code_amd/csrc/nerf_aux.hip b/nerf-3dtalker-code_amd/csrc/nerf_aux.hip
--- a/nerf-3dtalker-code_amd/csrc/nerf_aux.hip
+++ b/nerf-3dtalker-code_amd/csrc/nerf_aux.hip
@@ -154,10 +154,20 @@
 }
 
 #define FOLD_ROWGROUPS 24
+struct FoldRayTable {
+    N3dtGeom g;
+    const float *xy, *R, *Kinv;
+    float* raytab;
+};
 __global__ __launch_bounds__(256) void fold_latents_kernel(N3dtMlpParams p, int S, int A, int U, int merged, const float* __restrict__ shape,
                                                            const float* __restrict__ appea, const float* __restrict__ audio,
-                                                           float* __restrict__ fold) {
+                                                           float* __restrict__ fold, FoldRayTable rt) {
     const int b = blockIdx.x, stage = blockIdx.y;
+    if (stage >= N3DT_NSTAGE) {
+        const long ray = ((long)(stage - N3DT_NSTAGE) * FOLD_ROWGROUPS + blockIdx.z) * 256 + threadIdx.x;
+        if (ray < rt.g.n_rays) n3dt_ray_table_entry(rt.g, rt.xy, rt.R, rt.Kinv, b, (int)ray, rt.raytab);
+        return;
+    }
     const int lane = threadIdx.x & 63, wave = threadIdx.x >> 6;
     __shared__ float code[512 + N3DT_HID];
     const int in0 = N3DT_PE_DIM + S + U, in5 = N3DT_PE_DIM + S + N3DT_HID, inr = N3DT_HID + A;
@@ -218,7 +228,31 @@
 extern "C" void n3dt_launch_fold(const N3dtGeom* g, const N3dtMlpParams* p, const float* shape, const float* appea,
                                  const float* audio, float* fold, int merged_rgb, hipStream_t stream) {
     hipLaunchKernelGGL(fold_latents_kernel, dim3(g->batch, N3DT_NSTAGE, FOLD_ROWGROUPS), dim3(256), 0, stream, *p, g->shape_dim,
-                       g->appea_dim, g->audio_dim, merged_rgb, shape, appea, audio, fold);
+                       g->appea_dim, g->audio_dim, merged_rgb, shape, appea, audio, fold, FoldRayTable{*g, nullptr, nullptr, nullptr, nullptr});
+}
+
+extern "C" void n3dt_launch_fold_rays(const N3dtGeom* g, const N3dtMlpParams* p, const float* shape, const float* appea,
+                                      const float* audio, float* fold, int merged_rgb, const float* xy, const float* R,
+                                      const float* Kinv, float* raytab, hipStream_t stream) {
+    const int ray_rows = (int)(((long)g->n_rays + 256 * FOLD_ROWGROUPS - 1) / (256 * FOLD_ROWGROUPS));
+    hipLaunchKernelGGL(fold_latents_kernel, dim3(g->batch, N3DT_NSTAGE + ray_rows, FOLD_ROWGROUPS), dim3(256), 0, stream, *p, g->shape_dim,
+                       g->appea_dim, g->audio_dim, merged_rgb, shape, appea, audio, fold, FoldRayTable{*g, xy, R, Kinv, raytab});
+}
+
+__global__ __launch_bounds__(256) void ray_table_kernel(FoldRayTable rt) {
+    const long ray = (long)blockIdx.x * 256 + threadIdx.x;
+    if (ray < rt.g.n_rays) n3dt_ray_table_entry(rt.g, rt.xy, rt.R, rt.Kinv, (int)blockIdx.y, (int)ray, rt.raytab);
+}
+extern "C" void n3dt_launch_ray_table(const N3dtGeom* g, const float* xy, const float* R, const float* Kinv, float* raytab,
+                                      hipStream_t stream) {
+    for (int f0 = 0; f0 < g->batch; f0 += 65535) {
+        const int frames = g->batch - f0 < 65535 ? g->batch - f0 : 65535;
+        N3dtGeom gs = *g;
+        gs.batch = frames;
+        hipLaunchKernelGGL(ray_table_kernel, dim3((unsigned)((g->n_rays + 255) / 256), frames), dim3(256), 0, stream,
+                           FoldRayTable{gs, xy + (int64_t)f0 * g->xy_stride_b, R + (size_t)f0 * 9, Kinv + (size_t)f0 * 9,
+                                        raytab + (size_t)f0 * g->n_rays * N3DT_RAYTAB_STRIDE});
+    }
 }
 
 __global__ __launch_bounds__(256) void rayfold_kernel(int n_rays, long total, const float* __restrict__ fold, const float* __restrict__ ray_bias,
diff --git a/nerf-3dtalker-code_amd/csrc/nerf_fwd_x16.hip b/nerf-3dtalker-code_amd/csrc/nerf_fwd_x16.hip
--- a/nerf-3dtalker-code_amd/csrc/nerf_fwd_x16.hip
+++ b/nerf-3dtalker-code_amd/csrc/nerf_fwd_x16.hip
@@ -190,12 +190,19 @@
     unsigned* gates;
 };
 
+struct X16Head {
+    unsigned bpf;
+    int bpr_sh;
+    int frame0;
+};
+
 template <int PREC, int WAVES, bool SAVE = false>
 __device__ __forceinline__ void nerf_fwd_x16_body(
     const N3dtGeom& g, const unsigned char* __restrict__ packed, const float* __restrict__ fold, const float* __restrict__ xy,
     const float* __restrict__ R, const float* __restrict__ T, const float* __restrict__ Kinv, const float* __restrict__ t_rand,
     float* __restrict__ part, float* __restrict__ wlocal, int bpr, long total_blocks, unsigned char* lds, const int wave,
-    const X16TrainSave tsv = X16TrainSave{nullptr, nullptr, nullptr, nullptr}) {
+    const X16TrainSave tsv = X16TrainSave{nullptr, nullptr, nullptr, nullptr}, const X16Head hd = X16Head{0u, 0, 0},
+    const float* __restrict__ raytab = nullptr) {
     typedef typename X16<PREC>::frag frag;
     const int lane = threadIdx.x & 63;
     const int c = lane & 31, h = lane >> 5;
@@ -216,19 +223,34 @@
     ws.prologue_issue();
     unsigned char* pe_lds = lds + X16_NBUF * X16_CH * X16_PIECE + (size_t)wave * 4 * X16_PIECE + lane * 16;
 
-    long blk = (long)blockIdx.x * WAVES + wave;
-    const bool live = __builtin_amdgcn_readfirstlane((int)(blk < total_blocks)) != 0;
-    if (!live) blk = total_blocks - 1;
+    long blk;
+    bool live;
+    int sb, ray, frame;
+    long ray0;
+    if constexpr (SAVE) {
+        blk = (long)blockIdx.x * WAVES + wave;
+        live = __builtin_amdgcn_readfirstlane((int)(blk < total_blocks)) != 0;
+        if (!live) blk = total_blocks - 1;
+        sb = (int)(blk % bpr);
+        ray0 = blk / bpr;
+        ray = (int)(ray0 % g.n_rays);
+        frame = (int)(ray0 / g.n_rays);
+    } else {
+        const N3dtBlockIndex bi = n3dt_block_index(blockIdx.x, WAVES, wave, hd.bpf, (unsigned)bpr, hd.bpr_sh);
+        live = __builtin_amdgcn_readfirstlane((int)bi.live) != 0;
+        sb = (int)bi.sb;
+        ray = (int)bi.ray;
+        frame = hd.frame0 + (int)blockIdx.y;
+        blk = (long)frame * hd.bpf + bi.blk;
+        ray0 = (long)frame * g.n_rays + ray;
+    }
     float* const po = part + (size_t)blk * N3DT_PART_STRIDE;
     float dist, zval;
     frag pe[4];
-    const int sb = (int)(blk % bpr);
-    const long ray0 = blk / bpr;
-    const int ray = (int)(ray0 % g.n_rays);
-    const int frame = (int)(ray0 / g.n_rays);
     {
         float p[3];
-        n3dt_sample_point(g, xy, R, T, Kinv, t_rand, frame, ray, sb * X16_BS + c, p, dist, zval);
+        if constexpr (SAVE) n3dt_sample_point(g, xy, R, T, Kinv, t_rand, frame, ray, sb * X16_BS + c, p, dist, zval);
+        else n3dt_sample_point_tab(g, raytab, T, t_rand, frame, ray, sb * X16_BS + c, p, dist, zval);
         pe_encode<PREC>(p, h, pe_lds, pe);
     }
     const float* fb = fold + (size_t)__builtin_amdgcn_readfirstlane(frame) * N3DT_FOLD_STRIDE;
@@ -339,10 +361,11 @@
 __global__ __launch_bounds__(WAVES * 64, 1) void nerf_fwd_x16_kernel(
     N3dtGeom g, const unsigned char* __restrict__ packed, const float* __restrict__ fold, const float* __restrict__ xy,
     const float* __restrict__ R, const float* __restrict__ T, const float* __restrict__ Kinv, const float* __restrict__ t_rand,
-    float* __restrict__ part, float* __restrict__ wlocal, int bpr, long total_blocks) {
+    float* __restrict__ part, float* __restrict__ wlocal, int bpr, X16Head hd, const float* __restrict__ raytab) {
     extern __shared__ __attribute__((aligned(16))) unsigned char lds[];
     const int wave = __builtin_amdgcn_readfirstlane(threadIdx.x >> 6);
-    nerf_fwd_x16_body<PREC, WAVES>(g, packed, fold, xy, R, T, Kinv, t_rand, part, wlocal, bpr, total_blocks, lds, wave);
+    nerf_fwd_x16_body<PREC, WAVES>(g, packed, fold, xy, R, T, Kinv, t_rand, part, wlocal, bpr, 0L, lds, wave,
+                                   X16TrainSave{nullptr, nullptr, nullptr, nullptr}, hd, raytab);
 }
 
 template <int WAVES>
@@ -375,22 +398,29 @@
 }
 
 template <int PREC>
-static void launch_x16(const N3dtGeom* g, const void* packed, const float* fold, const float* xy, const float* R, const float* T,
-                       const float* Kinv, const float* t_rand, float* part, float* wlocal, hipStream_t stream) {
+static void launch_x16(const N3dtGeom* g, const void* packed, const float* fold, const float* raytab, const float* xy, const float* R,
+                       const float* T, const float* Kinv, const float* t_rand, float* part, float* wlocal, hipStream_t stream) {
     constexpr int WAVES = 8;
     const int bpr = (g->n_samples + X16_BS - 1) / X16_BS;
-    const long total = (long)g->batch * g->n_rays * bpr;
-    const int grid = (int)((total + WAVES - 1) / WAVES);
+    X16Head hd;
+    hd.bpf = (unsigned)g->n_rays * (unsigned)bpr;
+    hd.bpr_sh = (bpr & (bpr - 1)) == 0 ? __builtin_ctz((unsigned)bpr) : -1;
+    const unsigned grid_x = (hd.bpf + WAVES - 1) / WAVES;
+    constexpr int MAX_Y = 65535;
     const size_t lds_bytes = X16_NBUF * X16_CH * X16_PIECE + (size_t)WAVES * 4 * X16_PIECE + (size_t)WAVES * 2 * X16_BIAS_SLOT;
     auto kern = nerf_fwd_x16_kernel<PREC, WAVES>;
     (void)hipFuncSetAttribute(reinterpret_cast<const void*>(kern), hipFuncAttributeMaxDynamicSharedMemorySize, (int)lds_bytes);
-    hipLaunchKernelGGL(kern, dim3(grid), dim3(WAVES * 64), lds_bytes, stream, *g, reinterpret_cast<const unsigned char*>(packed),
-                       fold, xy, R, T, Kinv, t_rand, part, wlocal, bpr, total);
-}
-
-extern "C" void n3dt_launch_nerf_fwd_x16(const N3dtGeom* g, int precision, const void* packed, const float* fold, const float* xy,
-                                         const float* R, const float* T, const float* Kinv, const float* t_rand, float* part,
-                                         float* wlocal, hipStream_t stream) {
-    if (precision == N3DT_BF16) launch_x16<N3DT_BF16>(g, packed, fold, xy, R, T, Kinv, t_rand, part, wlocal, stream);
-    else launch_x16<N3DT_F16>(g, packed, fold, xy, R, T, Kinv, t_rand, part, wlocal, stream);
-}
+    for (int f0 = 0; f0 < g->batch; f0 += MAX_Y) {
+        hd.frame0 = f0;
+        const int frames = g->batch - f0 < MAX_Y ? g->batch - f0 : MAX_Y;
+        hipLaunchKernelGGL(kern, dim3(grid_x, frames), dim3(WAVES * 64), lds_bytes, stream, *g, reinterpret_cast<const unsigned char*>(packed),
+                           fold, xy, R, T, Kinv, t_rand, part, wlocal, bpr, hd, raytab);
+    }
+}
+
+extern "C" void n3dt_launch_nerf_fwd_x16(const N3dtGeom* g, int precision, const void* packed, const float* fold, const float* raytab,
+                                         const float* xy, const float* R, const float* T, const float* Kinv, const float* t_rand,
+                                         float* part, float* wlocal, hipStream_t stream) {
+    if (precision == N3DT_BF16) launch_x16<N3DT_BF16>(g, packed, fold, raytab, xy, R, T, Kinv, t_rand, part, wlocal, stream);
+    else launch_x16<N3DT_F16>(g, packed, fold, raytab, xy, R, T, Kinv, t_rand, part, wlocal, stream);
+}
diff --git a/nerf-3dtalker-code_amd/csrc/seams.hip b/nerf-3dtalker-code_amd/csrc/seams.hip
--- a/nerf-3dtalker-code_amd/csrc/seams.hip
+++ b/nerf-3dtalker-code_amd/csrc/seams.hip
@@ -298,6 +298,36 @@
     }
 }
 
+__global__ void __launch_bounds__(512) x16_head_probe_kernel(N3dtGeom g, const float* __restrict__ raytab, const float* __restrict__ T,
+                                                             const float* __restrict__ t_rand, float* __restrict__ out, int bpr,
+                                                             unsigned bpf, int bpr_sh, int frame0) {
+    const int wave = __builtin_amdgcn_readfirstlane(threadIdx.x >> 6);
+    const int lane = threadIdx.x & 63, c = lane & 31, h = lane >> 5;
+    const N3dtBlockIndex bi = n3dt_block_index(blockIdx.x, 8, wave, bpf, (unsigned)bpr, bpr_sh);
+    const int frame = frame0 + (int)blockIdx.y, ray = (int)bi.ray, s = (int)bi.sb * X16_BS + c;
+    float p[3], dist, zval;
+    n3dt_sample_point_tab(g, raytab, T, t_rand, frame, ray, s, p, dist, zval);
+    if (!bi.live || h != 0 || s >= g.n_samples) return;
+    const size_t M = (size_t)g.n_rays * g.n_samples, m = (size_t)ray * g.n_samples + s, o = (size_t)frame * 5 * M + m;
+    out[o] = p[0];
+    out[o + M] = p[1];
+    out[o + 2 * M] = p[2];
+    out[o + 3 * M] = dist;
+    out[o + 4 * M] = zval;
+}
+
+extern "C" void n3dt_launch_x16_head_probe(const N3dtGeom* g, const float* raytab, const float* T, const float* t_rand, float* out,
+                                           hipStream_t s) {
+    const int bpr = (g->n_samples + X16_BS - 1) / X16_BS;
+    const unsigned bpf = (unsigned)g->n_rays * (unsigned)bpr;
+    const int bpr_sh = (bpr & (bpr - 1)) == 0 ? __builtin_ctz((unsigned)bpr) : -1;
+    for (int f0 = 0; f0 < g->batch; f0 += 65535) {
+        const int frames = g->batch - f0 < 65535 ? g->batch - f0 : 65535;
+        hipLaunchKernelGGL(x16_head_probe_kernel, dim3((bpf + 7) / 8, frames), dim3(512), 0, s, *g, raytab, T, t_rand, out, bpr, bpf, bpr_sh,
+                           f0);
+    }
+}
+
 extern "C" void n3dt_launch_x16_pack_probe(int precision, int form, size_t n, const float* in, unsigned short* out, hipStream_t s) {
     const dim3 grid((unsigned)(n / 512)), block(64);
     if (precision == N3DT_BF16) {
diff --git a/nerf-3dtalker-code_amd/n3dt/_lib.py b/nerf-3dtalker-code_amd/n3dt/_lib.py
--- a/nerf-3dtalker-code_amd/n3dt/_lib.py
+++ b/nerf-3dtalker-code_amd/n3dt/_lib.py
@@ -106,7 +106,7 @@
     "n3dt_a2s_saved_bytes", "n3dt_a2s_workspace_bytes", "n3dt_a2s_fwd", "n3dt_a2s_bwd",
     "n3dt_flat_adam_record_bytes", "n3dt_flat_adam_step",
     "n3dt_render_fwd16", "n3dt_neural_render_fwd16_reuse", "n3dt_feat_to_rgb0",
-    "n3dt_x16_pack_probe", "n3dt_x16_pe_probe",
+    "n3dt_x16_pack_probe", "n3dt_x16_pe_probe", "n3dt_x16_head_probe",
     "n3dt_eval_metrics_workspace_bytes", "n3dt_eval_metrics",
     "n3dt_lpips_packed_bytes", "n3dt_lpips_pack", "n3dt_lpips_workspace_bytes", "n3dt_lpips",
     "n3dt_mel_workspace_bytes", "n3dt_mel_spectrogram", "n3dt_mel_windows",
@@ -215,6 +215,8 @@
     L.n3dt_x16_pack_probe.argtypes = [ci, ci, sz, vp, vp, vp]
     L.n3dt_x16_pe_probe.restype = ci
     L.n3dt_x16_pe_probe.argtypes = [ci, ci, sz, vp, vp, vp]
+    L.n3dt_x16_head_probe.restype = ci
+    L.n3dt_x16_head_probe.argtypes = [ctypes.POINTER(Geom)] + [vp] * 8
     L.n3dt_stage_inputs.restype = ci
     L.n3dt_stage_inputs.argtypes = [ctypes.POINTER(Stage), vp]
     L.n3dt_graph_begin.restype = ci
diff --git a/nerf-3dtalker-code_amd/n3dt/ops.py b/nerf-3dtalker-code_amd/n3dt/ops.py
--- a/nerf-3dtalker-code_amd/n3dt/ops.py
+++ b/nerf-3dtalker-code_amd/n3dt/ops.py
@@ -195,6 +195,15 @@
     out = torch.empty((n // 32, 4, 64, 8), dtype=torch.bfloat16 if prec == _lib.BF16 else torch.float16, device=points.device)
     check(lib().n3dt_x16_pe_probe(prec, int(form), n, _ptr(points), _ptr(out), _stream()), "n3dt_x16_pe_probe")
     return out
+
+
+def x16_head_probe(geom, xy, R, T, Kinv, t_rand=None):
+    B, Nr, Ns, dev = geom.batch, geom.n_rays, geom.n_samples, xy.device
+    out = torch.empty(B, 5, Nr, Ns, dtype=torch.float32, device=dev)
+    table = torch.empty(B * Nr * 4, dtype=torch.float32, device=dev)
+    check(lib().n3dt_x16_head_probe(ctypes.byref(geom), _ptr(xy), _ptr(R), _ptr(T), _ptr(Kinv), _ptr(t_rand), _ptr(out), _ptr(table),
+                                    _stream()), "n3dt_x16_head_probe")
+    return {"pts": out[:, 0:3], "z_dists": out[:, 3:4], "zvals": out[:, 4:5]}
 
 
 def ray_vd_bias(geom, w_rgb1, xy, R, Kinv, out=None):
```
